# wildsonbbl/gnnepcsaft

Hardware: AMD Instinct MI355X
Metric: molecular graphs/sec (fwd+bwd) (higher is better)
Workload: dtype f32; 1 GPU; BASELINE configs[1]: PNA hidden=128 L=6 towers=1 pre=2 post=4, 4096 graphs/GPU (81920 atoms, 163840 directed bonds), fwd+loss+bwd incl. CSR packing; graphs_per_gpu=4096, parallelism=dp1, hip_graph=False, launch=auto, grad_allreduce_bytes=0, grad_exchange=none (1 rank)

## Files before the change

gnnepcsaft_amd/_lib.py:

```python
from __future__ import annotations

import ctypes as C
from pathlib import Path
from typing import Dict, Optional

import torch

_LIB_PATH = Path(__file__).resolve().parent / "libgnnepcsaft_hip.so"

ABI_VERSION = 6
GNX_OK, GNX_E_INVALID, GNX_E_HIP, GNX_E_RANGE, GNX_E_WORKSPACE = 0, -1, -2, -3, -4
OPT_GEMM_SPLIT, OPT_WGRAD_WGS, OPT_EMBED_BWD_MFMA, OPT_STD_BWD_CENTERED, OPT_GEMM_PIPE, OPT_WGRAD_PIPE, OPT_GEMM_AS, \
    OPT_GEMM_WS_FAST, OPT_GEMM_TILE_ROWS, OPT_GEMM_MID = range(10)
GEMM_RELU, GEMM_ACCUMULATE, GEMM_B_TRANS, GEMM_SPLIT_ONLY, GEMM_PRESPLIT = 1, 2, 4, 8, 16
POOL_ADD, POOL_MEAN, POOL_MAX = 0, 1, 2
K_NONE, K_PNA_AGG_FWD, K_PNA_AGG_BWD, K_GEMM_WS, K_GEMM_WGRAD, K_GINE_AGG_FWD, K_GINE_AGG_BWD, K_EDGE_COMBINE_FWD, \
    K_EDGE_COMBINE_BWD, K_BN_FWD, K_BN_BWD, K_GEMM_TILED, K_GEMM_SMALL, K_GEMM_WGRAD_BATCHED, K_KEY_SEGMENT_SUM, \
    K_EMBED, K_PNA_EDGE_FWD, K_PNA_EDGE_BWD, K_ATTN_FWD, K_ATTN_BWD, K_PCSAFT_RHO, K_PCSAFT_VP = range(22)
K_COUNT = 22
KERNEL_GROUPS = {K_PNA_AGG_FWD: "pna_aggregate_fwd", K_PNA_AGG_BWD: "pna_aggregate_bwd", K_GEMM_WS: "gemm_weights_stationary",
                 K_GEMM_WGRAD: "weight_gradient", K_GINE_AGG_FWD: "gine_aggregate_fwd", K_GINE_AGG_BWD: "gine_aggregate_bwd",
                 K_EDGE_COMBINE_FWD: "edge_combine_fwd", K_EDGE_COMBINE_BWD: "edge_combine_bwd", K_BN_FWD: "batchnorm_fwd",
                 K_BN_BWD: "batchnorm_bwd", K_GEMM_TILED: "gemm_tiled", K_GEMM_SMALL: "gemm_small",
                 K_GEMM_WGRAD_BATCHED: "weight_gradient_batched", K_KEY_SEGMENT_SUM: "key_segment_sum", K_EMBED: "embedding",
                 K_PNA_EDGE_FWD: "pna_edge_fused_fwd", K_PNA_EDGE_BWD: "pna_edge_fused_bwd",
                 K_ATTN_FWD: "transformer_attn_fwd", K_ATTN_BWD: "transformer_attn_bwd",
                 K_PCSAFT_RHO: "pcsaft_density", K_PCSAFT_VP: "pcsaft_vapor_pressure"}


class GnxError(RuntimeError):
    def __init__(self, status: int, msg: str):
        super().__init__(f"gnx status {status}: {msg}")
        self.status = status


class GemmSeg(C.Structure):
    _fields_ = [("a", C.c_void_p), ("lda", C.c_int64), ("rowscale", C.c_void_p), ("b", C.c_void_p),
                ("ldb", C.c_int64), ("k", C.c_int32), ("_pad", C.c_int32)]


class WgradProb(C.Structure):
    _fields_ = [("dC", C.c_void_p), ("lddc", C.c_int64), ("A", C.c_void_p), ("lda", C.c_int64),
                ("rowscale", C.c_void_p), ("dW", C.c_void_p), ("lddw", C.c_int64), ("dbias", C.c_void_p),
                ("M", C.c_int64), ("N", C.c_int32), ("K", C.c_int32)]


_vp, _i32, _i64, _f32, _sz = C.c_void_p, C.c_int32, C.c_int64, C.c_float, C.c_size_t

PNA_MAX_LAYERS, PNA_MAX_TOWERS = 8, 8
PNA_BWD_DEFER_SMALL, PNA_BWD_LAST_OF_PASS = 1, 2


class PnaFwdArgs(C.Structure):
    _fields_ = [("N", _i64), ("E", _i64), ("T", _i32), ("F", _i32), ("pre_layers", _i32), ("post_layers", _i32),
                ("D", _i32), ("merged", _i32),
                ("rowptr", _vp), ("src", _vp), ("dst", _vp), ("code", _vp), ("dperm", _vp), ("tiles", _vp), ("ntiles", _vp),
                ("max_tiles", _i64), ("x", _vp), ("Te", _vp), ("weff", _vp * PNA_MAX_TOWERS), ("Wm", _vp), ("bm", _vp),
                ("params", C.POINTER(_vp)), ("P", _vp), ("Q", _vp), ("A", _vp), ("hs", _vp * PNA_MAX_LAYERS),
                ("zs", _vp * PNA_MAX_LAYERS), ("ws", _vp), ("ws_bytes", _sz), ("out", _vp), ("etile_info", _vp),
                ("etile_w", _i32), ("tile_rows", _i32)]


class PnaBwdArgs(C.Structure):
    _fields_ = [("N", _i64), ("E", _i64), ("T", _i32), ("F", _i32), ("pre_layers", _i32), ("post_layers", _i32),
                ("R", _i32), ("D", _i32), ("avg_deg_log", _f32), ("merged", _i32), ("acc_first", _i32),
                ("use_side_streams", _i32), ("n_h", _i32), ("n_z", _i32),
                ("rowptr", _vp), ("colptr", _vp), ("cpos", _vp), ("code", _vp), ("code_pos", _vp), ("dperm", _vp),
                ("tiles", _vp), ("ntiles", _vp), ("chunks", _vp), ("nchunks", _vp),
                ("max_tiles", _i64), ("max_chunks", _i64),
                ("x", _vp), ("BE", _vp), ("EE", _vp), ("A", _vp),
                ("hs", _vp * PNA_MAX_LAYERS), ("zs", _vp * PNA_MAX_LAYERS), ("weff", _vp * PNA_MAX_TOWERS), ("Wm", _vp),
                ("params", C.POINTER(_vp)), ("grads", C.POINTER(_vp)), ("dout", _vp),
                ("gbuf", _vp * PNA_MAX_LAYERS), ("dA", _vp), ("gebuf", _vp * PNA_MAX_LAYERS), ("dP", _vp), ("dQ", _vp),
                ("dTe", _vp), ("dEE", _vp), ("dWm", _vp), ("dbm", _vp), ("dWeff", _vp), ("ws", _vp), ("ws_bytes", _sz),
                ("acc_buf", _vp), ("dx", _vp), ("flags", _i32), ("etile_w", _i32), ("etile_info", _vp)]


class PnaFinishArgs(C.Structure):
    _fields_ = [("L", _i32), ("T", _i32), ("F", _i32), ("pre_layers", _i32), ("post_layers", _i32), ("R", _i32), ("D", _i32),
                ("merged", _i32), ("use_side_streams", _i32), ("_pad", _i32),
                ("BE", _vp), ("acc_buf", _vp), ("ones", _vp), ("avg_deg_log", C.POINTER(_f32)),
                ("params", C.POINTER(_vp)), ("grads", C.POINTER(_vp)), ("EE", C.POINTER(_vp)), ("dTe", C.POINTER(_vp)),
                ("dEE", C.POINTER(_vp)), ("dWm", C.POINTER(_vp)), ("dbm", C.POINTER(_vp)), ("dWeff", C.POINTER(_vp))]


class SmallProb(C.Structure):
    _fields_ = [("A", _vp), ("lda", _i64), ("B", _vp), ("ldb", _i64), ("bias", _vp), ("C", _vp), ("ldc", _i64),
                ("M", _i32), ("N", _i32), ("K", _i32), ("flags", _i32)]


SB_A_TRANS, SB_B_TRANS, SB_ACCUMULATE, SB_ATOMIC, SB_RELU = 1, 2, 4, 8, 16

SIGNATURES = {
    "gnx_create": (_i32, [C.POINTER(_vp), _i32]),
    "gnx_destroy": (_i32, [_vp]),
    "gnx_set_stream": (_i32, [_vp, _vp]),
    "gnx_last_error": (C.c_char_p, []),
    "gnx_abi_version": (_i32, []),
    "gnx_set_option": (_i32, [_vp, _i32, _i32]),
    "gnx_get_option": (_i32, [_vp, _i32, C.POINTER(_i32)]),
    "gnx_prof_begin": (_i32, [_vp, C.c_uint32]),
    "gnx_prof_read": (_i32, [_vp, _i32, C.POINTER(_i64), C.POINTER(C.c_double), C.POINTER(C.c_double),
                             C.POINTER(C.c_double), C.POINTER(C.c_double)]),
    "gnx_prof_end": (_i32, [_vp]),
    "gnx_pack_csr_workspace_bytes": (_sz, [_i64, _i64]),
    "gnx_pack_csr": (_i32, [_vp, _vp, _i64, _i64, _vp, _vp, _vp, _vp, _vp, _vp, _vp, _sz]),
    "gnx_feature_code": (_i32, [_vp, _vp, _i64, _i32, C.POINTER(_i32), _vp, _vp, _vp, _sz]),
    "gnx_graph_ptr": (_i32, [_vp, _vp, _i64, _i64, _vp, _vp, _sz]),
    "gnx_degree_scalers": (_i32, [_vp, _vp, _i64, _f32, _vp, _vp]),
    "gnx_embed_sum_fwd": (_i32, [_vp, _vp, _i64, _i32, C.POINTER(_i32), _vp, _i32, _vp]),
    "gnx_table_scatter_workspace_bytes": (_sz, [_i64, _i32, _i32]),
    "gnx_embed_sum_bwd": (_i32, [_vp, _vp, _i64, _i32, C.POINTER(_i32), _i32, _vp, _i32, _vp, _vp, _sz]),
    "gnx_check_range": (_i32, [_vp]),
    "gnx_gemm_workspace_bytes": (_sz, [_vp, _i32, C.POINTER(GemmSeg), C.POINTER(_i64), _i32, _i64, _i32, _vp, _i32,
                                       _i32]),
    "gnx_gemm": (_i32, [_vp, _i32, C.POINTER(GemmSeg), _i64, _i32, _vp, _vp, _i64, _vp, _i64, _i32, _vp, _sz]),
    "gnx_gemm_wgrad": (_i32, [_vp, _vp, _i64, _vp, _i64, _vp, _i64, _i32, _i32, _vp, _i64, _vp]),
    "gnx_gemm_wgrad_batched": (_i32, [_vp, _i32, C.POINTER(WgradProb)]),
    "gnx_degree_max": (_i32, [_vp, _vp, _i64, C.POINTER(_i32)]),
    "gnx_degree_classes_workspace_bytes": (_sz, [_i64, _i32]),
    "gnx_degree_classes": (_i32, [_vp, _vp, _i64, _i32, _vp, _vp, _vp, _sz]),
    "gnx_class_tiles": (_i32, [_vp, _vp, _i32, _i32, _vp, _vp]),
    "gnx_gemm_grouped": (_i32, [_vp, _i32, C.POINTER(GemmSeg), C.POINTER(_i64), _i32, _i64, _i32, _vp, _vp, _i64, _vp,
                                _i64, _i32, _vp, _vp, _vp, _i64, _vp, _sz]),
    "gnx_gemm_tile_rows": (_i32, [_vp, _i64, _i32]),
    "gnx_gemm_grouped_rows": (_i32, [_vp, _i32, C.POINTER(GemmSeg), C.POINTER(_i64), _i32, _i64, _i32, _vp, _vp, _i64, _vp,
                                     _i64, _i32, _vp, _vp, _vp, _i64, _vp, _sz, _i32]),
    "gnx_gemm_wgrad_grouped": (_i32, [_vp, _vp, _i64, _vp, _i64, _i64, _i32, _i32, _vp, _i64, _i64, _vp, _vp, _vp,
                                      _i64]),
    "gnx_pna_weff": (_i32, [_vp, _vp, _i64, _i32, _i32, _f32, _vp]),
    "gnx_pna_weff_bwd": (_i32, [_vp, _vp, _i32, _i32, _f32, _vp, _i64]),
    "gnx_group_by_small_key": (_i32, [_vp, _vp, _i64, _i32, _vp, _vp, _vp, _sz]),
    "gnx_key_segment_sum": (_i32, [_vp, _vp, _vp, _vp, _i64, _i32, _vp]),
    "gnx_edge_combine_fwd": (_i32, [_vp, _vp, _vp, _vp, _vp, _vp, _vp, _i64, _i32, _i32, _vp]),
    "gnx_edge_combine_bwd": (_i32, [_vp, _vp, _vp, _vp, _vp, _vp, _i64, _i64, _i32, _i32, _vp, _vp, _vp, _vp, _sz]),
    "gnx_pna_aggregate_fwd": (_i32, [_vp, _vp, _vp, _i64, _i64, _i32, _i32, _vp]),
    "gnx_pna_aggregate_bwd": (_i32, [_vp, _vp, _vp, _vp, _vp, _i64, _i64, _i32, _i32, _vp]),
    "gnx_edge_tiles_count": (_i32, [_i64, _i32]),
    "gnx_edge_tiles": (_i32, [_vp, _vp, _i64, _i64, _i32, _vp]),
    "gnx_pna_edge_fwd": (_i32, [_vp, _vp, _vp, _vp, _vp, _vp, _vp, _vp, _vp, _i32, _i64, _i64, _i32, _i32, C.POINTER(_vp),
                                C.POINTER(_vp), _vp, _vp, _vp]),
    "gnx_pna_edge_bwd": (_i32, [_vp, _vp, _vp, _vp, _vp, _vp, _i32, _i64, _i64, _i32, _i32, _i32, C.POINTER(_vp), _vp, _vp,
                                _vp]),
    "gnx_gine_aggregate_fwd": (_i32, [_vp, _vp, _vp, _vp, _vp, _vp, _i64, _i64, _i32, _f32, _vp]),
    "gnx_gine_aggregate_bwd": (_i32, [_vp, _vp, _vp, _vp, _vp, _vp, _vp, _vp, _vp, _vp, _i64, _i64, _i32, _i32, _f32,
                                      _vp, _vp]),
    "gnx_gine_dle": (_i32, [_vp, _vp, _vp, _vp, _vp, _vp, _vp, _vp, _i64, _i32, _i32, _vp]),
    "gnx_transformer_attn_fwd": (_i32, [_vp, _vp, _vp, _vp, _vp, _vp, _i64, _i64, _i32, _i32, _f32, C.c_uint64,
                                        C.c_uint64, _vp, _vp, _vp]),
    "gnx_transformer_attn_bwd": (_i32, [_vp, _vp, _vp, _vp, _vp, _vp, _vp, _vp, _vp, _vp, _vp, _vp, _i64, _i64, _i32,
                                        _i32, _i32, _f32, C.c_uint64, C.c_uint64, _vp, _vp, _vp]),
    "gnx_transformer_attn_dle": (_i32, [_vp, _vp, _vp, _vp, _vp, _vp, _vp, _i64, _i32, _i32, _i32, _vp]),
    "gnx_pcsaft_density": (_i32, [_vp, _vp, _i64, _vp, _vp, _vp, _i64, _vp, _vp]),
    "gnx_pcsaft_vapor_pressure": (_i32, [_vp, _vp, _i64, _vp, _vp, _i64, _vp, _vp, _vp, _vp]),
    "gnx_segment_pool_fwd": (_i32, [_vp, _vp, _vp, _i64, _i32, _i32, _vp]),
    "gnx_segment_pool_bwd": (_i32, [_vp, _vp, _vp, _vp, _vp, _i64, _i32, _i32, _vp]),
    "gnx_batchnorm_workspace_bytes": (_sz, [_i64, _i32]),
    "gnx_batchnorm_fwd": (_i32, [_vp, _vp, _i64, _i32, _vp, _vp, _vp, _vp, _vp, _f32, _f32, _i32, _i32, _vp, _vp, _vp,
                                 _vp, _sz]),
    "gnx_batchnorm_bwd": (_i32, [_vp, _vp, _vp, _vp, _i64, _i32, _vp, _vp, _vp, _i32, _vp, _vp, _vp, _vp, _sz]),
    "gnx_dropout": (_i32, [_vp, _vp, _i64, _f32, C.c_uint64, C.c_uint64, _vp]),
    "gnx_huber_ape": (_i32, [_vp, _vp, _vp, _i64, _f32, _vp, _vp]),
    "gnx_adamw_amsgrad": (_i32, [_vp, _vp, _vp, _vp, _vp, _vp, _i64, _f32, _f32, _f32, _f32, _f32, _i64]),
    "gnx_sgd": (_i32, [_vp, _vp, _vp, _i64, _f32]),
    "gnx_pna_weight_only": (_i32, [_vp, _vp, _i32, _i32, _i32, _i32, _i32, _i32, _f32, C.POINTER(_vp), _i32, _vp, _vp,
                                   C.POINTER(_vp), _vp, _vp]),
    "gnx_pna_conv_fwd": (_i32, [_vp, C.POINTER(PnaFwdArgs)]),
    "gnx_pna_weight_only_all": (_i32, [_vp, _i32, _vp, _i32, _i32, _i32, _i32, _i32, _i32, C.POINTER(_f32), C.POINTER(_vp),
                                       _i32, C.POINTER(_vp), C.POINTER(_vp), C.POINTER(_vp), C.POINTER(_vp), C.POINTER(_vp)]),
    "gnx_pna_stack_finish": (_i32, [_vp, C.POINTER(PnaFinishArgs)]),
    "gnx_gemm_small_batched": (_i32, [_vp, _i32, C.POINTER(SmallProb)]),
    "gnx_pna_weff_batched": (_i32, [_vp, _i32, C.POINTER(_vp), _i64, _i32, _i32, C.POINTER(_f32), C.POINTER(_vp)]),
    "gnx_pna_weff_bwd_batched": (_i32, [_vp, _i32, C.POINTER(_vp), _i32, _i32, C.POINTER(_f32), C.POINTER(_vp), _i64]),
    "gnx_pna_conv_bwd_workspace_bytes": (_sz, [_i32, _i32, _i32]),
    "gnx_pna_conv_bwd": (_i32, [_vp, C.POINTER(PnaBwdArgs)]),
    "gnx_fill": (_i32, [_vp, _vp, _i64, _f32]),
    "gnx_scale": (_i32, [_vp, _vp, _i64, _f32]),
    "gnx_axpy": (_i32, [_vp, _vp, _vp, _i64, _f32]),
    "gnx_side_stream": (_i32, [_vp, C.POINTER(_vp)]),
    "gnx_side_begin": (_i32, [_vp]),
    "gnx_side_end": (_i32, [_vp]),
    "gnx_side_join": (_i32, [_vp]),
    "gnx_side_stream_n": (_i32, [_vp, _i32, C.POINTER(_vp)]),
    "gnx_side_begin_n": (_i32, [_vp, _i32]),
    "gnx_side_join_n": (_i32, [_vp, _i32]),
    "gnx_clip_rows": (_i32, [_vp, _vp, _i64, _i32, _vp, _vp, _vp]),
}

_lib: Optional[C.CDLL] = None
_handles: Dict[int, int] = {}


def lib_path() -> Path:
    return _LIB_PATH


def load() -> C.CDLL:
    global _lib
    if _lib is not None:
        return _lib
    if not _LIB_PATH.exists():
        raise ImportError(f"{_LIB_PATH} is missing: build it with `python -m gnnepcsaft_amd.build` "
                          "(hipcc --offload-arch=gfx950). There is no CPU fallback.")
    lib = C.CDLL(str(_LIB_PATH))
    for name, (res, args) in SIGNATURES.items():
        fn = getattr(lib, name)
        fn.restype = res
        fn.argtypes = args
    if lib.gnx_abi_version() != ABI_VERSION:
        raise ImportError(f"ABI version mismatch: library {lib.gnx_abi_version()} != binding {ABI_VERSION}")
    _lib = lib
    return lib


def last_error() -> str:
    return load().gnx_last_error().decode(errors="replace")


def check(status: int) -> None:
    if status != GNX_OK:
        raise GnxError(status, last_error())


_bound_stream: dict = {}
try:
    _raw_stream = torch._C._cuda_getCurrentRawStream
except AttributeError:
    def _raw_stream(idx: int) -> int:
        return torch.cuda.current_stream(idx).cuda_stream


def handle(device: torch.device) -> int:
    if device.type != "cuda":
        raise GnxError(GNX_E_INVALID, f"gnnepcsaft_amd kernels need a HIP device tensor, got {device}; there is no CPU "
                                      "fallback")
    idx = device.index if device.index is not None else torch.cuda.current_device()
    lib = load()
    h = _handles.get(idx)
    if h is None:
        out = _vp()
        check(lib.gnx_create(C.byref(out), idx))
        h = out.value
        _handles[idx] = h
    stream = _raw_stream(idx)
    if _bound_stream.get(idx) != stream:
        check(lib.gnx_set_stream(h, stream))
        _bound_stream[idx] = stream
    return h
```

gnnepcsaft_amd/csrc/gnx_norm.hip:

```cpp
#include "gnx_common.hpp"

#define BN_ROWS_PER_BLOCK 256

extern "C" size_t gnx_batchnorm_workspace_bytes(int64_t M, int32_t H) {
  if (M < 0) M = 0;
  size_t chunks = (size_t)gnx_cdiv(M > 0 ? M : 1, BN_ROWS_PER_BLOCK);
  return sizeof(float) * ((size_t)4 * H + chunks * 2 * (size_t)H) + 256;
}

__global__ void __launch_bounds__(256) k_bn_partial(const float* __restrict__ x, int64_t M, int H,
                                                    float* __restrict__ part) {
  __shared__ float s1[4][64], s2[4][64];
  const int cx = threadIdx.x & 63, ry = threadIdx.x >> 6;
  const int col = blockIdx.y * 64 + cx;
  int64_t r0 = (int64_t)blockIdx.x * BN_ROWS_PER_BLOCK;
  int64_t r1 = r0 + BN_ROWS_PER_BLOCK;
  if (r1 > M) r1 = M;
  float a1 = 0.f, a2 = 0.f;
  if (col < H) {
    const float k = x[col];
    for (int64_t r = r0 + ry; r < r1; r += 4) {
      float v = x[r * H + col] - k;
      a1 += v;
      a2 += v * v;
    }
  }
  s1[ry][cx] = a1;
  s2[ry][cx] = a2;
  __syncthreads();
  if (ry == 0 && col < H) {
    float t1 = (s1[0][cx] + s1[1][cx]) + (s1[2][cx] + s1[3][cx]);
    float t2 = (s2[0][cx] + s2[1][cx]) + (s2[2][cx] + s2[3][cx]);
    part[((int64_t)blockIdx.x * 2 + 0) * H + col] = t1;
    part[((int64_t)blockIdx.x * 2 + 1) * H + col] = t2;
  }
}


__global__ void __launch_bounds__(256) k_bn_partial_v4(const float* __restrict__ x, int64_t M, int H,
                                                       float* __restrict__ part) {
  __shared__ f32x4 s1[8][32], s2[8][32];
  const int cq = threadIdx.x & 31, ry = threadIdx.x >> 5;
  const int col = blockIdx.y * 128 + cq * 4;
  int64_t r0 = (int64_t)blockIdx.x * BN_ROWS_PER_BLOCK;
  int64_t r1 = r0 + BN_ROWS_PER_BLOCK;
  if (r1 > M) r1 = M;
  f32x4 a1 = {0.f, 0.f, 0.f, 0.f}, a2 = {0.f, 0.f, 0.f, 0.f};
  if (col < H) {
    const f32x4 k = *reinterpret_cast<const f32x4*>(x + col);
    int64_t r = r0 + ry;
    for (; r + 24 < r1; r += 32) {
      f32x4 v0 = *reinterpret_cast<const f32x4*>(x + r * H + col);
      f32x4 v1 = *reinterpret_cast<const f32x4*>(x + (r + 8) * H + col);
      f32x4 v2 = *reinterpret_cast<const f32x4*>(x + (r + 16) * H + col);
      f32x4 v3 = *reinterpret_cast<const f32x4*>(x + (r + 24) * H + col);
      v0 -= k;
      a1 += v0;
      a2 += v0 * v0;
      v1 -= k;
      a1 += v1;
      a2 += v1 * v1;
      v2 -= k;
      a1 += v2;
      a2 += v2 * v2;
      v3 -= k;
      a1 += v3;
      a2 += v3 * v3;
    }
    for (; r < r1; r += 8) {
      f32x4 v = *reinterpret_cast<const f32x4*>(x + r * H + col);
      v -= k;
      a1 += v;
      a2 += v * v;
    }
  }
  s1[ry][cq] = a1;
  s2[ry][cq] = a2;
  __syncthreads();
  if (ry == 0 && col < H) {
    f32x4 t1 = s1[0][cq], t2 = s2[0][cq];
#pragma unroll
    for (int l = 1; l < 8; ++l) {
      t1 += s1[l][cq];
      t2 += s2[l][cq];
    }
    *reinterpret_cast<f32x4*>(part + ((int64_t)blockIdx.x * 2 + 0) * H + col) = t1;
    *reinterpret_cast<f32x4*>(part + ((int64_t)blockIdx.x * 2 + 1) * H + col) = t2;
  }
}

__global__ void __launch_bounds__(256) k_bn_bwd_partial_v4(const float* __restrict__ dy, const float* __restrict__ x,
                                                           const float* __restrict__ y, int64_t M, int H,
                                                           const float* __restrict__ mean,
                                                           const float* __restrict__ rstd, int relu,
                                                           float* __restrict__ part) {
  __shared__ f32x4 s1[8][32], s2[8][32];
  const int cq = threadIdx.x & 31, ry = threadIdx.x >> 5;
  const int col = blockIdx.y * 128 + cq * 4;
  int64_t r0 = (int64_t)blockIdx.x * BN_ROWS_PER_BLOCK;
  int64_t r1 = r0 + BN_ROWS_PER_BLOCK;
  if (r1 > M) r1 = M;
  f32x4 a1 = {0.f, 0.f, 0.f, 0.f}, a2 = {0.f, 0.f, 0.f, 0.f};
  if (col < H) {
    const f32x4 mu = *reinterpret_cast<const f32x4*>(mean + col);
    const f32x4 rs = *reinterpret_cast<const f32x4*>(rstd + col);
    auto row = [&](int64_t r, f32x4& g, f32x4& xv, f32x4& yv) {
      g = *reinterpret_cast<const f32x4*>(dy + r * H + col);
      xv = *reinterpret_cast<const f32x4*>(x + r * H + col);
      yv = *reinterpret_cast<const f32x4*>((relu ? y : x) + r * H + col);
    };
    auto fold = [&](f32x4 g, const f32x4& xv, const f32x4& yv) {
      if (relu) {
        g.x = yv.x > 0.f ? g.x : 0.f;
        g.y = yv.y > 0.f ? g.y : 0.f;
        g.z = yv.z > 0.f ? g.z : 0.f;
        g.w = yv.w > 0.f ? g.w : 0.f;
      }
      a1 += g;
      a2 += g * ((xv - mu) * rs);
    };
    int64_t r = r0 + ry;
    for (; r + 8 < r1; r += 16) {
      f32x4 g0, x0, y0, g1, x1, y1;
      row(r, g0, x0, y0);
      row(r + 8, g1, x1, y1);
      fold(g0, x0, y0);
      fold(g1, x1, y1);
    }
    for (; r < r1; r += 8) {
      f32x4 g, xv, yv;
      row(r, g, xv, yv);
      fold(g, xv, yv);
    }
  }
  s1[ry][cq] = a1;
  s2[ry][cq] = a2;
  __syncthreads();
  if (ry == 0 && col < H) {
    f32x4 t1 = s1[0][cq], t2 = s2[0][cq];
#pragma unroll
    for (int l = 1; l < 8; ++l) {
      t1 += s1[l][cq];
      t2 += s2[l][cq];
    }
    *reinterpret_cast<f32x4*>(part + ((int64_t)blockIdx.x * 2 + 0) * H + col) = t1;
    *reinterpret_cast<f32x4*>(part + ((int64_t)blockIdx.x * 2 + 1) * H + col) = t2;
  }
}

template <int VEC>
__global__ void __launch_bounds__(256) k_bn_bwd_apply_v(const float* __restrict__ dy, const float* __restrict__ x,
                                                        const float* __restrict__ y, int64_t total, int H,
                                                        const float* __restrict__ mean, const float* __restrict__ rstd,
                                                        const float* __restrict__ coef, int relu,
                                                        float* __restrict__ dx) {
  int64_t i = ((int64_t)blockIdx.x * blockDim.x + threadIdx.x) * 4;
  const int64_t stride = (int64_t)gridDim.x * blockDim.x * 4;
  for (; i < total; i += stride) {
    const int c = (int)(i % H);
    f32x4 g = *reinterpret_cast<const f32x4*>(dy + i);
    const f32x4 xv = *reinterpret_cast<const f32x4*>(x + i);
    if (relu) {
      const f32x4 yv = *reinterpret_cast<const f32x4*>(y + i);
      g.x = yv.x > 0.f ? g.x : 0.f;
      g.y = yv.y > 0.f ? g.y : 0.f;
      g.z = yv.z > 0.f ? g.z : 0.f;
      g.w = yv.w > 0.f ? g.w : 0.f;
    }
    const f32x4 mu = *reinterpret_cast<const f32x4*>(mean + c), rs = *reinterpret_cast<const f32x4*>(rstd + c);
    const f32x4 k0 = *reinterpret_cast<const f32x4*>(coef + c), k1 = *reinterpret_cast<const f32x4*>(coef + H + c),
                k2 = *reinterpret_cast<const f32x4*>(coef + 2 * H + c);
    const f32x4 xh = (xv - mu) * rs;
    *reinterpret_cast<f32x4*>(dx + i) = k0 * (g - k1 - xh * k2);
  }
}

__device__ __forceinline__ void bn_fold(const float* __restrict__ part, int64_t chunks, int H, int c, float& t1,
                                        float& t2) {
  __shared__ float f1[16][17], f2[16][17];
  const int cx = threadIdx.x & 15, ly = threadIdx.x >> 4;
  float a1 = 0.f, a2 = 0.f;
  if (c < H) {
    int64_t b = ly;
    for (; b + 48 < chunks; b += 64) {
      const float p0 = part[(b * 2 + 0) * H + c], q0 = part[(b * 2 + 1) * H + c];
      const float p1 = part[((b + 16) * 2 + 0) * H + c], q1 = part[((b + 16) * 2 + 1) * H + c];
      const float p2 = part[((b + 32) * 2 + 0) * H + c], q2 = part[((b + 32) * 2 + 1) * H + c];
      const float p3 = part[((b + 48) * 2 + 0) * H + c], q3 = part[((b + 48) * 2 + 1) * H + c];
      a1 += p0;
      a2 += q0;
      a1 += p1;
      a2 += q1;
      a1 += p2;
      a2 += q2;
      a1 += p3;
      a2 += q3;
    }
    for (; b < chunks; b += 16) {
      a1 += part[(b * 2 + 0) * H + c];
      a2 += part[(b * 2 + 1) * H + c];
    }
  }
  f1[ly][cx] = a1;
  f2[ly][cx] = a2;
  __syncthreads();
  t1 = 0.f;
  t2 = 0.f;
  if (ly == 0) {
#pragma unroll
    for (int l = 0; l < 16; ++l) {
      t1 += f1[l][cx];
      t2 += f2[l][cx];
    }
  }
}

__global__ void k_bn_finalize(const float* __restrict__ x, const float* __restrict__ part, int64_t chunks, int64_t M,
                              int H, const float* __restrict__ gamma, const float* __restrict__ beta,
                              float* __restrict__ running_mean, float* __restrict__ running_var, float momentum,
                              float eps, int training, float* __restrict__ save_mean, float* __restrict__ save_rstd,
                              float* __restrict__ ab, int64_t* __restrict__ num_batches_tracked) {
  const int c = blockIdx.x * 16 + (threadIdx.x & 15);
  if (training && num_batches_tracked != nullptr && blockIdx.x == 0 && threadIdx.x == 0) num_batches_tracked[0] += 1;
  float t1 = 0.f, t2 = 0.f;
  if (training) bn_fold(part, chunks, H, c, t1, t2);
  if (c >= H || (threadIdx.x >> 4) != 0) return;
  float mean, var;
  if (training) {
    const float inv = 1.0f / (float)M;
    const float d = t1 * inv;
    mean = x[c] + d;
    var = fmaxf(t2 * inv - d * d, 0.f);
    if (running_mean) running_mean[c] = (1.f - momentum) * running_mean[c] + momentum * mean;
    if (running_var) {
      float unb = (M > 1) ? var * ((float)M / (float)(M - 1)) : var;
      running_var[c] = (1.f - momentum) * running_var[c] + momentum * unb;
    }
  } else {
    mean = running_mean[c];
    var = running_var[c];
  }
  float rstd = 1.0f / sqrtf(var + eps);
  if (save_mean) save_mean[c] = mean;
  if (save_rstd) save_rstd[c] = rstd;
  float a = rstd * (gamma ? gamma[c] : 1.f);
  ab[c] = a;
  ab[H + c] = (beta ? beta[c] : 0.f) - mean * a;
}

template <int VEC>
__global__ void __launch_bounds__(256) k_bn_apply(const float* __restrict__ x, int64_t total, int H,
                                                  const float* __restrict__ ab, int relu, float* __restrict__ y) {
  int64_t i = ((int64_t)blockIdx.x * blockDim.x + threadIdx.x) * VEC;
  int64_t stride = (int64_t)gridDim.x * blockDim.x * VEC;
  for (; i < total; i += stride) {
    int c = (int)(i % H);
    if constexpr (VEC == 4) {
      f32x4 v = *reinterpret_cast<const f32x4*>(x + i);
      f32x4 a = *reinterpret_cast<const f32x4*>(ab + c);
      f32x4 b = *reinterpret_cast<const f32x4*>(ab + H + c);
      f32x4 o = {v.x * a.x + b.x, v.y * a.y + b.y, v.z * a.z + b.z, v.w * a.w + b.w};
      if (relu) {
        o.x = fmaxf(o.x, 0.f);
        o.y = fmaxf(o.y, 0.f);
        o.z = fmaxf(o.z, 0.f);
        o.w = fmaxf(o.w, 0.f);
      }
      *reinterpret_cast<f32x4*>(y + i) = o;
    } else {
      float o = x[i] * ab[c] + ab[H + c];
      y[i] = relu ? fmaxf(o, 0.f) : o;
    }
  }
}

extern "C" int32_t gnx_batchnorm_fwd(gnx_handle* h, const float* x, int64_t M, int32_t H, const float* gamma,
                                     const float* beta, float* running_mean, float* running_var,
                                     int64_t* num_batches_tracked, float momentum, float eps, int32_t training,
                                     int32_t relu, float* y, float* save_mean, float* save_rstd, void* ws,
                                     size_t ws_bytes) {
  GNX_CHECK_ARG(h && H > 0 && M >= 0, "gnx_batchnorm_fwd: bad argument");
  if (M == 0) return GNX_OK;
  GNX_CHECK_ARG(x && y && ws, "gnx_batchnorm_fwd: NULL argument");
  GNX_CHECK_ARG(training || (running_mean && running_var), "gnx_batchnorm_fwd: eval mode needs running stats");
  if (ws_bytes < gnx_batchnorm_workspace_bytes(M, H)) {
    gnx_set_error("gnx_batchnorm_fwd: workspace %zu < %zu", ws_bytes, gnx_batchnorm_workspace_bytes(M, H));
    return GNX_E_WORKSPACE;
  }
  float* ab = reinterpret_cast<float*>(ws);
  float* part = ab + 4 * (size_t)H;
  int64_t chunks = gnx_cdiv(M, BN_ROWS_PER_BLOCK);
  gnx_prof_scope prof(h, GNX_K_BN_FWD, (training ? 12.0 : 8.0) * M * H);
  if (training) {
    if (H % 4 == 0)
      hipLaunchKernelGGL(k_bn_partial_v4, dim3((unsigned)chunks, (unsigned)gnx_cdiv(H, 128)), dim3(256), 0, h->stream, x,
                         M, (int)H, part);
    else
      hipLaunchKernelGGL(k_bn_partial, dim3((unsigned)chunks, (unsigned)gnx_cdiv(H, 64)), dim3(256), 0, h->stream, x, M,
                         (int)H, part);
    GNX_LAUNCH_CHECK();
  }
  hipLaunchKernelGGL(k_bn_finalize, dim3((unsigned)gnx_cdiv(H, 16)), dim3(256), 0, h->stream, x, part, chunks, M, (int)H,
                     gamma, beta, running_mean, running_var, momentum, eps, (int)training, save_mean, save_rstd, ab,
                     num_batches_tracked);
  GNX_LAUNCH_CHECK();
  int64_t total = M * H;
  if (H % 4 == 0) {
    int64_t blocks = gnx_cdiv(total / 4, 256);
    if (blocks > 4096) blocks = 4096;
    hipLaunchKernelGGL(k_bn_apply<4>, dim3((unsigned)blocks), dim3(256), 0, h->stream, x, total, (int)H, ab, (int)relu, y);
  } else {
    int64_t blocks = gnx_cdiv(total, 256);
    if (blocks > 4096) blocks = 4096;
    hipLaunchKernelGGL(k_bn_apply<1>, dim3((unsigned)blocks), dim3(256), 0, h->stream, x, total, (int)H, ab, (int)relu, y);
  }
  GNX_LAUNCH_CHECK();
  return GNX_OK;
}

__global__ void __launch_bounds__(256) k_bn_bwd_partial(const float* __restrict__ dy, const float* __restrict__ x,
                                                        const float* __restrict__ y, int64_t M, int H,
                                                        const float* __restrict__ mean, const float* __restrict__ rstd,
                                                        int relu, float* __restrict__ part) {
  __shared__ float s1[4][64], s2[4][64];
  const int cx = threadIdx.x & 63, ry = threadIdx.x >> 6;
  const int col = blockIdx.y * 64 + cx;
  int64_t r0 = (int64_t)blockIdx.x * BN_ROWS_PER_BLOCK;
  int64_t r1 = r0 + BN_ROWS_PER_BLOCK;
  if (r1 > M) r1 = M;
  float a1 = 0.f, a2 = 0.f;
  if (col < H) {
    const float mu = mean[col], rs = rstd[col];
    for (int64_t r = r0 + ry; r < r1; r += 4) {
      float g = dy[r * H + col];
      if (relu && !(y[r * H + col] > 0.f)) g = 0.f;
      a1 += g;
      a2 += g * ((x[r * H + col] - mu) * rs);
    }
  }
  s1[ry][cx] = a1;
  s2[ry][cx] = a2;
  __syncthreads();
  if (ry == 0 && col < H) {
    part[((int64_t)blockIdx.x * 2 + 0) * H + col] = (s1[0][cx] + s1[1][cx]) + (s1[2][cx] + s1[3][cx]);
    part[((int64_t)blockIdx.x * 2 + 1) * H + col] = (s2[0][cx] + s2[1][cx]) + (s2[2][cx] + s2[3][cx]);
  }
}

__global__ void k_bn_bwd_finalize(const float* __restrict__ part, int64_t chunks, int64_t M, int H,
                                  const float* __restrict__ gamma, const float* __restrict__ rstd,
                                  float* __restrict__ dgamma, float* __restrict__ dbeta, float* __restrict__ coef) {
  const int c = blockIdx.x * 16 + (threadIdx.x & 15);
  float t1 = 0.f, t2 = 0.f;
  bn_fold(part, chunks, H, c, t1, t2);
  if (c >= H || (threadIdx.x >> 4) != 0) return;
  if (dbeta) dbeta[c] += t1;
  if (dgamma) dgamma[c] += t2;
  const float inv = 1.0f / (float)M;
  coef[c] = (gamma ? gamma[c] : 1.f) * rstd[c];
  coef[H + c] = t1 * inv;
  coef[2 * H + c] = t2 * inv;
}

__global__ void __launch_bounds__(256) k_bn_bwd_apply(const float* __restrict__ dy, const float* __restrict__ x,
                                                      const float* __restrict__ y, int64_t total, int H,
                                                      const float* __restrict__ mean, const float* __restrict__ rstd,
                                                      const float* __restrict__ coef, int relu, float* __restrict__ dx) {
  int64_t i = (int64_t)blockIdx.x * blockDim.x + threadIdx.x;
  int64_t stride = (int64_t)gridDim.x * blockDim.x;
  for (; i < total; i += stride) {
    int c = (int)(i % H);
    float g = dy[i];
    if (relu && !(y[i] > 0.f)) g = 0.f;
    float xh = (x[i] - mean[c]) * rstd[c];
    dx[i] = coef[c] * (g - coef[H + c] - xh * coef[2 * H + c]);
  }
}

extern "C" int32_t gnx_batchnorm_bwd(gnx_handle* h, const float* dy, const float* x, const float* y, int64_t M,
                                     int32_t H, const float* gamma, const float* save_mean, const float* save_rstd,
                                     int32_t relu, float* dx, float* dgamma, float* dbeta, void* ws, size_t ws_bytes) {
  GNX_CHECK_ARG(h && H > 0 && M >= 0, "gnx_batchnorm_bwd: bad argument");
  if (M == 0) return GNX_OK;
  GNX_CHECK_ARG(dy && x && save_mean && save_rstd && dx && ws && (!relu || y), "gnx_batchnorm_bwd: NULL argument");
  if (ws_bytes < gnx_batchnorm_workspace_bytes(M, H)) {
    gnx_set_error("gnx_batchnorm_bwd: workspace %zu < %zu", ws_bytes, gnx_batchnorm_workspace_bytes(M, H));
    return GNX_E_WORKSPACE;
  }
  float* coef = reinterpret_cast<float*>(ws);
  float* part = coef + 4 * (size_t)H;
  int64_t chunks = gnx_cdiv(M, BN_ROWS_PER_BLOCK);
  gnx_prof_scope prof(h, GNX_K_BN_BWD, 28.0 * M * H);
  if (H % 4 == 0)
    hipLaunchKernelGGL(k_bn_bwd_partial_v4, dim3((unsigned)chunks, (unsigned)gnx_cdiv(H, 128)), dim3(256), 0, h->stream,
                       dy, x, y, M, (int)H, save_mean, save_rstd, (int)relu, part);
  else
    hipLaunchKernelGGL(k_bn_bwd_partial, dim3((unsigned)chunks, (unsigned)gnx_cdiv(H, 64)), dim3(256), 0, h->stream, dy,
                       x, y, M, (int)H, save_mean, save_rstd, (int)relu, part);
  GNX_LAUNCH_CHECK();
  hipLaunchKernelGGL(k_bn_bwd_finalize, dim3((unsigned)gnx_cdiv(H, 16)), dim3(256), 0, h->stream, part, chunks, M, (int)H,
                     gamma, save_rstd, dgamma, dbeta, coef);
  GNX_LAUNCH_CHECK();
  int64_t total = M * H;
  if (H % 4 == 0) {
    int64_t blocks = gnx_cdiv(total / 4, 256);
    if (blocks > 4096) blocks = 4096;
    hipLaunchKernelGGL(k_bn_bwd_apply_v<4>, dim3((unsigned)blocks), dim3(256), 0, h->stream, dy, x, y, total, (int)H,
                       save_mean, save_rstd, coef, (int)relu, dx);
  } else {
    int64_t blocks = gnx_cdiv(total, 256);
    if (blocks > 8192) blocks = 8192;
    hipLaunchKernelGGL(k_bn_bwd_apply, dim3((unsigned)blocks), dim3(256), 0, h->stream, dy, x, y, total, (int)H,
                       save_mean, save_rstd, coef, (int)relu, dx);
  }
  GNX_LAUNCH_CHECK();
  return GNX_OK;
}

#define LOSS_MAX_BLOCKS 64

__global__ void __launch_bounds__(256) k_huber_partial(const float* __restrict__ pred, const float* __restrict__ tgt,
                                                       int64_t count, float delta, float* __restrict__ part,
                                                       float* __restrict__ dpred) {
  __shared__ float sh[256], sm[256];
  float ah = 0.f, am = 0.f;
  const float inv = 1.0f / (float)count;
  int64_t i = (int64_t)blockIdx.x * blockDim.x + threadIdx.x;
  int64_t stride = (int64_t)gridDim.x * blockDim.x;
  for (; i < count; i += stride) {
    float p = pred[i], t = tgt[i];
    float a = (p - t) / t;
    float aa = fabsf(a);
    ah += (aa <= delta) ? 0.5f * a * a : delta * (aa - 0.5f * delta);
    am += fabsf(p - t) / fmaxf(fabsf(t), 1.17e-06f);
    if (dpred) {
      float da = (aa <= delta) ? a : (a > 0.f ? delta : -delta);
      dpred[i] = da * inv / t;
    }
  }
  sh[threadIdx.x] = ah;
  sm[threadIdx.x] = am;
  __syncthreads();
  for (int off = 128; off > 0; off >>= 1) {
    if (threadIdx.x < off) {
      sh[threadIdx.x] += sh[threadIdx.x + off];
      sm[threadIdx.x] += sm[threadIdx.x + off];
    }
    __syncthreads();
  }
  if (threadIdx.x == 0) {
    part[blockIdx.x * 2] = sh[0];
    part[blockIdx.x * 2 + 1] = sm[0];
  }
}

__global__ void k_huber_final(const float* __restrict__ part, int blocks, int64_t count, float* __restrict__ out2) {
  if (threadIdx.x == 0 && blockIdx.x == 0) {
    float h = 0.f, m = 0.f;
    for (int b = 0; b < blocks; ++b) {
      h += part[b * 2];
      m += part[b * 2 + 1];
    }
    out2[0] = h / (float)count;
    out2[1] = m / (float)count;
  }
}

extern "C" int32_t gnx_huber_ape(gnx_handle* h, const float* pred, const float* target, int64_t count, float delta,
                                 float* out2, float* dpred) {
  GNX_CHECK_ARG(h && pred && target && out2 && count > 0, "gnx_huber_ape: bad argument");
  int blocks = (int)(gnx_cdiv(count, 256) < LOSS_MAX_BLOCKS ? gnx_cdiv(count, 256) : LOSS_MAX_BLOCKS);
  hipLaunchKernelGGL(k_huber_partial, dim3(blocks), dim3(256), 0, h->stream, pred, target, count, delta, h->d_scratch,
                     dpred);
  GNX_LAUNCH_CHECK();
  hipLaunchKernelGGL(k_huber_final, dim3(1), dim3(64), 0, h->stream, h->d_scratch, blocks, count, out2);
  GNX_LAUNCH_CHECK();
  return GNX_OK;
}
```

gnnepcsaft_amd/csrc/gnx_pack.hip:

```cpp
#include "gnx_common.hpp"

#define SCAN_ITEMS 4
#define SCAN_BLOCK 256
#define SCAN_TILE (SCAN_ITEMS * SCAN_BLOCK)

__global__ void __launch_bounds__(SCAN_BLOCK) k_scan_tile(const int* __restrict__ in, int* __restrict__ out,
                                                          int* __restrict__ sums, int64_t n) {
  __shared__ int s[SCAN_BLOCK];
  int64_t base = (int64_t)blockIdx.x * SCAN_TILE + (int64_t)threadIdx.x * SCAN_ITEMS;
  int v[SCAN_ITEMS];
  int t = 0;
#pragma unroll
  for (int i = 0; i < SCAN_ITEMS; ++i) {
    v[i] = (base + i < n) ? in[base + i] : 0;
    t += v[i];
  }
  s[threadIdx.x] = t;
  __syncthreads();
  for (int off = 1; off < SCAN_BLOCK; off <<= 1) {
    int add = (threadIdx.x >= off) ? s[threadIdx.x - off] : 0;
    __syncthreads();
    s[threadIdx.x] += add;
    __syncthreads();
  }
  int excl = s[threadIdx.x] - t;
#pragma unroll
  for (int i = 0; i < SCAN_ITEMS; ++i) {
    if (base + i < n) out[base + i] = excl;
    excl += v[i];
  }
  if (threadIdx.x == SCAN_BLOCK - 1) sums[blockIdx.x] = s[SCAN_BLOCK - 1];
}

__global__ void k_scan_add(int* __restrict__ out, const int* __restrict__ offs, int64_t n) {
  int64_t i = (int64_t)blockIdx.x * SCAN_TILE + threadIdx.x;
  int o = offs[blockIdx.x];
  for (int k = 0; k < SCAN_ITEMS; ++k, i += SCAN_BLOCK)
    if (i < n) out[i] += o;
}

__global__ void k_set_total(int* __restrict__ out, const int* __restrict__ in, int64_t n) {
  if (threadIdx.x == 0 && blockIdx.x == 0) out[n] = (n > 0) ? out[n - 1] + in[n - 1] : 0;
}

static int32_t exclusive_scan(gnx_handle* h, const int* in, int* out, int64_t n, int* ws, bool write_total) {
  if (n > 0) {
    int64_t blocks = gnx_cdiv(n, SCAN_TILE);
    hipLaunchKernelGGL(k_scan_tile, dim3((unsigned)blocks), dim3(SCAN_BLOCK), 0, h->stream, in, out, ws, n);
    GNX_LAUNCH_CHECK();
    if (blocks > 1) {
      int* sums_scanned = ws + blocks + 1;
      int32_t st = exclusive_scan(h, ws, sums_scanned, blocks, sums_scanned + blocks + 1, false);
      if (st != GNX_OK) return st;
      hipLaunchKernelGGL(k_scan_add, dim3((unsigned)blocks), dim3(SCAN_BLOCK), 0, h->stream, out, sums_scanned, n);
      GNX_LAUNCH_CHECK();
    }
  }
  if (write_total) {
    hipLaunchKernelGGL(k_set_total, dim3(1), dim3(64), 0, h->stream, out, in, n);
    GNX_LAUNCH_CHECK();
  }
  return GNX_OK;
}

static size_t scan_ws_ints_total(int64_t n) {
  size_t tot = 0;
  int64_t m = n;
  while (m > 1) {
    int64_t b = gnx_cdiv(m, SCAN_TILE);
    tot += 2 * ((size_t)b + 1);
    m = b;
  }
  return tot + 16;
}

__global__ void k_convert_edges(const int64_t* __restrict__ ei, int64_t E, int64_t N, int* __restrict__ src0,
                                int* __restrict__ dst0, int* __restrict__ flag) {
  int64_t e = (int64_t)blockIdx.x * blockDim.x + threadIdx.x;
  if (e >= E) return;
  int64_t s = ei[e], d = ei[E + e];
  bool bad = (s < 0) | (s >= N) | (d < 0) | (d >= N);
  if (bad) {
    atomicOr(flag, 1);
    s = 0;
    d = 0;
  }
  src0[e] = (int)s;
  dst0[e] = (int)d;
}

__global__ void k_count_keys(const int* __restrict__ key, int64_t E, int* __restrict__ counts) {
  int64_t e = (int64_t)blockIdx.x * blockDim.x + threadIdx.x;
  if (e < E) atomicAdd(&counts[key[e]], 1);
}

__global__ void k_fill_groups(const int* __restrict__ key, int64_t E, const int* __restrict__ ptr,
                              int* __restrict__ cursor, int* __restrict__ items) {
  int64_t e = (int64_t)blockIdx.x * blockDim.x + threadIdx.x;
  if (e >= E) return;
  int k = key[e];
  int pos = ptr[k] + atomicAdd(&cursor[k], 1);
  items[pos] = (int)e;
}

__global__ void k_sort_groups(const int* __restrict__ ptr, int64_t N, int* __restrict__ items) {
  int64_t i = (int64_t)blockIdx.x * blockDim.x + threadIdx.x;
  if (i >= N) return;
  int b = ptr[i], e = ptr[i + 1];
  for (int a = b + 1; a < e; ++a) {
    int v = items[a];
    int c = a - 1;
    while (c >= b && items[c] > v) {
      items[c + 1] = items[c];
      --c;
    }
    items[c + 1] = v;
  }
}

__global__ void k_gather_endpoints(const int* __restrict__ perm, const int* __restrict__ src0,
                                   const int* __restrict__ dst0, int64_t E, int* __restrict__ src,
                                   int* __restrict__ dst) {
  int64_t p = (int64_t)blockIdx.x * blockDim.x + threadIdx.x;
  if (p >= E) return;
  int e = perm[p];
  src[p] = src0[e];
  dst[p] = dst0[e];
}

static int32_t group_by_key(gnx_handle* h, const int* key, int64_t E, int64_t N, int* ptr, int* items, int* cursor,
                            int* scan_ws) {
  gnx_zero_ints(h, cursor, N > 0 ? N : 1);
  if (E > 0) {
    hipLaunchKernelGGL(k_count_keys, dim3((unsigned)gnx_cdiv(E, 256)), dim3(256), 0, h->stream, key, E, cursor);
    GNX_LAUNCH_CHECK();
  }
  int32_t st = exclusive_scan(h, cursor, ptr, N, scan_ws, true);
  if (st != GNX_OK) return st;
  gnx_zero_ints(h, cursor, N > 0 ? N : 1);
  if (E > 0) {
    hipLaunchKernelGGL(k_fill_groups, dim3((unsigned)gnx_cdiv(E, 256)), dim3(256), 0, h->stream, key, E, ptr, cursor,
                       items);
    GNX_LAUNCH_CHECK();
    hipLaunchKernelGGL(k_sort_groups, dim3((unsigned)gnx_cdiv(N, 256)), dim3(256), 0, h->stream, ptr, N, items);
    GNX_LAUNCH_CHECK();
  }
  return GNX_OK;
}

extern "C" size_t gnx_pack_csr_workspace_bytes(int64_t N, int64_t E) {
  if (N < 0) N = 0;
  if (E < 0) E = 0;
  size_t ints = 2 * (size_t)E + (size_t)N + 1 + scan_ws_ints_total(N) + 64;
  return ints * sizeof(int);
}

extern "C" int32_t gnx_pack_csr(gnx_handle* h, const int64_t* edge_index, int64_t E, int64_t N, int32_t* rowptr,
                                int32_t* perm, int32_t* src, int32_t* dst, int32_t* colptr, int32_t* cpos, void* ws,
                                size_t ws_bytes) {
  GNX_CHECK_ARG(h != nullptr, "gnx_pack_csr: handle is NULL");
  GNX_CHECK_ARG(N >= 0 && E >= 0 && N < (1ll << 31) - 1 && E < (1ll << 31) - 1, "gnx_pack_csr: N=%lld E=%lld out of int32 range",
                (long long)N, (long long)E);
  GNX_CHECK_ARG(rowptr && colptr, "gnx_pack_csr: rowptr/colptr NULL");
  GNX_CHECK_ARG(E == 0 || (edge_index && perm && src && dst && cpos), "gnx_pack_csr: NULL edge array with E>0");
  if (ws_bytes < gnx_pack_csr_workspace_bytes(N, E) || (!ws && ws_bytes)) {
    gnx_set_error("gnx_pack_csr: workspace %zu < %zu", ws_bytes, gnx_pack_csr_workspace_bytes(N, E));
    return GNX_E_WORKSPACE;
  }
  GNX_CHECK_ARG(ws != nullptr, "gnx_pack_csr: workspace is NULL");
  int* w = reinterpret_cast<int*>(ws);
  int* src0 = w;
  int* dst0 = src0 + E;
  int* cursor = dst0 + E;
  int* scan_ws = cursor + N + 1;
  if (E > 0) {
    hipLaunchKernelGGL(k_convert_edges, dim3((unsigned)gnx_cdiv(E, 256)), dim3(256), 0, h->stream, edge_index, E, N,
                       src0, dst0, h->d_flag);
    GNX_LAUNCH_CHECK();
  }
  int32_t st = group_by_key(h, dst0, E, N, rowptr, perm, cursor, scan_ws);
  if (st != GNX_OK) return st;
  if (E > 0) {
    hipLaunchKernelGGL(k_gather_endpoints, dim3((unsigned)gnx_cdiv(E, 256)), dim3(256), 0, h->stream, perm, src0,
                       dst0, E, src, dst);
    GNX_LAUNCH_CHECK();
  }
  return group_by_key(h, src, E, N, colptr, cpos, cursor, scan_ws);
}

struct dims_t {
  int d[16];
};

__global__ void k_feature_code(const int64_t* __restrict__ feat, int64_t rows, int K, dims_t dims,
                               const int* __restrict__ perm, int* __restrict__ code, int* __restrict__ flag) {
  int64_t p = (int64_t)blockIdx.x * blockDim.x + threadIdx.x;
  if (p >= rows) return;
  int64_t r = perm ? perm[p] : p;
  int c = 0;
  bool bad = false;
  for (int k = 0; k < K; ++k) {
    int64_t f = feat[r * K + k];
    if (f < 0 || f >= dims.d[k]) {
      bad = true;
      f = 0;
    }
    c = c * dims.d[k] + (int)f;
  }
  if (bad) atomicOr(flag, 2);
  code[p] = c;
}

extern "C" int32_t gnx_feature_code(gnx_handle* h, const int64_t* feat, int64_t rows, int32_t K, const int32_t* dims,
                                    const int32_t* perm, int32_t* code, void* ws, size_t ws_bytes) {
  (void)ws;
  (void)ws_bytes;
  GNX_CHECK_ARG(h && dims && K > 0 && K <= 16 && rows >= 0, "gnx_feature_code: bad argument");
  GNX_CHECK_ARG(rows == 0 || (feat && code), "gnx_feature_code: NULL array with rows>0");
  dims_t d;
  int64_t prod = 1;
  for (int k = 0; k < 16; ++k) d.d[k] = (k < K) ? dims[k] : 1;
  for (int k = 0; k < K; ++k) {
    GNX_CHECK_ARG(dims[k] > 0, "gnx_feature_code: dims[%d] <= 0", k);
    prod *= dims[k];
  }
  GNX_CHECK_ARG(prod < (1ll << 31), "gnx_feature_code: code space overflows int32");
  if (rows > 0) {
    hipLaunchKernelGGL(k_feature_code, dim3((unsigned)gnx_cdiv(rows, 256)), dim3(256), 0, h->stream, feat, rows, (int)K,
                       d, perm, code, h->d_flag);
    GNX_LAUNCH_CHECK();
  }
  return GNX_OK;
}

__global__ void k_graph_ptr(const int64_t* __restrict__ batch, int64_t N, int64_t B, int* __restrict__ ptr,
                            int* __restrict__ flag) {
  int64_t n = (int64_t)blockIdx.x * blockDim.x + threadIdx.x;
  if (n > N) return;
  int64_t prev = (n == 0) ? -1 : batch[n - 1];
  int64_t cur = (n == N) ? B : batch[n];
  if (n < N && (cur < 0 || cur >= B)) {
    atomicOr(flag, 4);
    return;
  }
  if (cur < prev) {
    atomicOr(flag, 8);
    return;
  }
  for (int64_t g = prev + 1; g <= cur; ++g) ptr[g] = (int)n;
}

extern "C" int32_t gnx_graph_ptr(gnx_handle* h, const int64_t* batch, int64_t N, int64_t B, int32_t* graph_ptr,
                                 void* ws, size_t ws_bytes) {
  (void)ws;
  (void)ws_bytes;
  GNX_CHECK_ARG(h && graph_ptr && N >= 0 && B >= 0 && (batch || N == 0), "gnx_graph_ptr: bad argument");
  hipLaunchKernelGGL(k_graph_ptr, dim3((unsigned)gnx_cdiv(N + 1, 256)), dim3(256), 0, h->stream, batch, N, B,
                     graph_ptr, h->d_flag);
  GNX_LAUNCH_CHECK();
  return GNX_OK;
}

__global__ void k_degree_scalers(const int* __restrict__ rowptr, int64_t N, float avg_log, float* __restrict__ amp,
                                 float* __restrict__ att) {
  int64_t n = (int64_t)blockIdx.x * blockDim.x + threadIdx.x;
  if (n >= N) return;
  float d = (float)(rowptr[n + 1] - rowptr[n]);
  amp[n] = logf(d + 1.0f) / avg_log;
  att[n] = avg_log / logf(fmaxf(d, 1.0f) + 1.0f);
}

extern "C" int32_t gnx_degree_scalers(gnx_handle* h, const int32_t* rowptr, int64_t N, float avg_deg_log, float* amp,
                                      float* att) {
  GNX_CHECK_ARG(h && N >= 0 && (N == 0 || (rowptr && amp && att)), "gnx_degree_scalers: bad argument");
  if (N == 0) return GNX_OK;
  hipLaunchKernelGGL(k_degree_scalers, dim3((unsigned)gnx_cdiv(N, 256)), dim3(256), 0, h->stream, rowptr, N,
                     avg_deg_log, amp, att);
  GNX_LAUNCH_CHECK();
  return GNX_OK;
}

struct weff_batch_args {
  const float* W[GNX_SMALL_BATCH];
  float* out[GNX_SMALL_BATCH];
  float avg_log[GNX_SMALL_BATCH];
  int64_t ldw;
  int F, D;
};

__global__ void k_pna_weff_batched(weff_batch_args a) {
  const int b = blockIdx.y;
  const int F = a.F;
  int64_t i = (int64_t)blockIdx.x * blockDim.x + threadIdx.x;
  int64_t per = (int64_t)F * 4 * F;
  if (i >= per * a.D) return;
  int d = (int)(i / per);
  int o = (int)((i % per) / (4 * F)), j = (int)(i % (4 * F));
  float dd = (float)d;
  float amp = logf(dd + 1.0f) / a.avg_log[b];
  float att = a.avg_log[b] / logf(fmaxf(dd, 1.0f) + 1.0f);
  const float* w = a.W[b] + (int64_t)o * a.ldw;
  a.out[b][i] = w[F + j] + amp * w[5 * F + j] + att * w[9 * F + j];
}

struct weff_bwd_batch_args {
  const float* dWeff[GNX_SMALL_BATCH];
  float* dW[GNX_SMALL_BATCH];
  float avg_log[GNX_SMALL_BATCH];
  int64_t lddw;
  int F, D;
};

__global__ void k_pna_weff_bwd_batched(weff_bwd_batch_args a) {
  const int b = blockIdx.y;
  const int F = a.F;
  int64_t i = (int64_t)blockIdx.x * blockDim.x + threadIdx.x;
  int64_t per = (int64_t)F * 4 * F;
  if (i >= per) return;
  int o = (int)(i / (4 * F)), j = (int)(i % (4 * F));
  float s1 = 0.f, s2 = 0.f, s3 = 0.f;
  const float avg_log = a.avg_log[b];
  const float* dWeff = a.dWeff[b];
  for (int d = 0; d < a.D; ++d) {
    float dd = (float)d;
    float amp = logf(dd + 1.0f) / avg_log;
    float att = avg_log / logf(fmaxf(dd, 1.0f) + 1.0f);
    float v = dWeff[(int64_t)d * per + i];
    s1 += v;
    s2 += amp * v;
    s3 += att * v;
  }
  float* w = a.dW[b] + (int64_t)o * a.lddw;
  w[F + j] += s1;
  w[5 * F + j] += s2;
  w[9 * F + j] += s3;
}

extern "C" int32_t gnx_pna_weff_bwd_batched(gnx_handle* h, int32_t n, const float* const* dWeff, int32_t F, int32_t D,
                                            const float* avg_deg_log, float* const* dW, int64_t lddw) {
  GNX_CHECK_ARG(h && dWeff && dW && avg_deg_log && n >= 0 && F > 0 && D > 0 && lddw >= 13 * F,
                "gnx_pna_weff_bwd_batched: bad argument");
  const int64_t cnt = (int64_t)F * 4 * F;
  for (int32_t i0 = 0; i0 < n; i0 += GNX_SMALL_BATCH) {
    weff_bwd_batch_args a;
    const int m = n - i0 < GNX_SMALL_BATCH ? n - i0 : GNX_SMALL_BATCH;
    for (int i = 0; i < GNX_SMALL_BATCH; ++i) {
      const int k = i < m ? i0 + i : i0;
      a.dWeff[i] = dWeff[k];
      a.dW[i] = dW[k];
      a.avg_log[i] = avg_deg_log[k];
      GNX_CHECK_ARG(a.dWeff[i] && a.dW[i], "gnx_pna_weff_bwd_batched: NULL pointer at %d", k);
    }
    a.lddw = lddw;
    a.F = F;
    a.D = D;
    hipLaunchKernelGGL(k_pna_weff_bwd_batched, dim3((unsigned)gnx_cdiv(cnt, 256), (unsigned)m), dim3(256), 0, h->stream, a);
    GNX_LAUNCH_CHECK();
  }
  return GNX_OK;
}

extern "C" int32_t gnx_pna_weff_batched(gnx_handle* h, int32_t n, const float* const* W, int64_t ldw, int32_t F, int32_t D,
                                        const float* avg_deg_log, float* const* Weff) {
  GNX_CHECK_ARG(h && W && Weff && avg_deg_log && n >= 0 && F > 0 && D > 0 && ldw >= 13 * F, "gnx_pna_weff_batched: bad argument");
  const int64_t cnt = (int64_t)F * 4 * F * D;
  for (int32_t i0 = 0; i0 < n; i0 += GNX_SMALL_BATCH) {
    weff_batch_args a;
    const int m = n - i0 < GNX_SMALL_BATCH ? n - i0 : GNX_SMALL_BATCH;
    for (int i = 0; i < GNX_SMALL_BATCH; ++i) {
      const int k = i < m ? i0 + i : i0;
      a.W[i] = W[k];
      a.out[i] = Weff[k];
      a.avg_log[i] = avg_deg_log[k];
      GNX_CHECK_ARG(a.W[i] && a.out[i], "gnx_pna_weff_batched: NULL pointer at %d", k);
    }
    a.ldw = ldw;
    a.F = F;
    a.D = D;
    hipLaunchKernelGGL(k_pna_weff_batched, dim3((unsigned)gnx_cdiv(cnt, 256), (unsigned)m), dim3(256), 0, h->stream, a);
    GNX_LAUNCH_CHECK();
  }
  return GNX_OK;
}

extern "C" int32_t gnx_pna_weff(gnx_handle* h, const float* W, int64_t ldw, int32_t F, int32_t D, float avg_deg_log,
                                float* Weff) {
  GNX_CHECK_ARG(h && W && Weff && F > 0 && D > 0 && ldw >= 13 * F, "gnx_pna_weff: bad argument");
  return gnx_pna_weff_batched(h, 1, &W, ldw, F, D, &avg_deg_log, &Weff);
}

extern "C" int32_t gnx_pna_weff_bwd(gnx_handle* h, const float* dWeff, int32_t F, int32_t D, float avg_deg_log,
                                    float* dW, int64_t lddw) {
  GNX_CHECK_ARG(h && dWeff && dW && F > 0 && D > 0 && lddw >= 13 * F, "gnx_pna_weff_bwd: bad argument");
  return gnx_pna_weff_bwd_batched(h, 1, &dWeff, F, D, &avg_deg_log, &dW, lddw);
}

__global__ void k_degree_max(const int* __restrict__ rowptr, int64_t N, int* __restrict__ out) {
  int64_t n = (int64_t)blockIdx.x * blockDim.x + threadIdx.x;
  int d = (n < N) ? rowptr[n + 1] - rowptr[n] : 0;
  for (int off = 32; off > 0; off >>= 1) d = max(d, __shfl_xor(d, off));
  if ((threadIdx.x & 63) == 0) atomicMax(out, d);
}

extern "C" int32_t gnx_degree_max(gnx_handle* h, const int32_t* rowptr, int64_t N, int32_t* max_degree_host) {
  GNX_CHECK_ARG(h && max_degree_host && N >= 0 && (N == 0 || rowptr), "gnx_degree_max: bad argument");
  int* d_out = h->d_flag + 8;
  gnx_zero_ints(h, d_out, 1);
  if (N > 0) {
    hipLaunchKernelGGL(k_degree_max, dim3((unsigned)gnx_cdiv(N, 256)), dim3(256), 0, h->stream, rowptr, N, d_out);
    GNX_LAUNCH_CHECK();
  }
  int v = 0;
  GNX_HIP(hipMemcpyAsync(&v, d_out, sizeof(int), hipMemcpyDeviceToHost, h->stream));
  GNX_HIP(hipStreamSynchronize(h->stream));
  *max_degree_host = v;
  return GNX_OK;
}

#define DC_BLOCK 256
#define DC_MAX_CLASSES 64

__global__ void __launch_bounds__(DC_BLOCK) k_dc_hist(const int* __restrict__ rowptr, const int* __restrict__ keys,
                                                       int64_t N, int D, int nblocks, int* __restrict__ blockhist,
                                                       int* __restrict__ flag) {
  __shared__ int hist[DC_MAX_CLASSES];
  if (threadIdx.x < DC_MAX_CLASSES) hist[threadIdx.x] = 0;
  __syncthreads();
  int64_t n = (int64_t)blockIdx.x * DC_BLOCK + threadIdx.x;
  if (n < N) {
    int d = keys ? keys[n] : rowptr[n + 1] - rowptr[n];
    if (d < 0) d = 0;
    if (d >= D) {
      atomicOr(flag, 32);
      d = D - 1;
    }
    atomicAdd(&hist[d], 1);
  }
  __syncthreads();
  if (threadIdx.x < D) blockhist[threadIdx.x * nblocks + blockIdx.x] = hist[threadIdx.x];
}

__global__ void __launch_bounds__(DC_BLOCK) k_dc_fill(const int* __restrict__ rowptr, const int* __restrict__ keys,
                                                       int64_t N, int D, int nblocks,
                                                       const int* __restrict__ blockoff, int* __restrict__ dperm,
                                                       int* __restrict__ cls_ptr) {
  __shared__ int degs[DC_BLOCK];
  int64_t n = (int64_t)blockIdx.x * DC_BLOCK + threadIdx.x;
  int d = -1;
  if (n < N) {
    d = keys ? keys[n] : rowptr[n + 1] - rowptr[n];
    if (d < 0) d = 0;
    if (d >= D) d = D - 1;
  }
  degs[threadIdx.x] = d;
  __syncthreads();
  if (n < N) {
    int rank = 0;
    for (int t = 0; t < (int)threadIdx.x; ++t) rank += (degs[t] == d) ? 1 : 0;
    dperm[blockoff[d * nblocks + blockIdx.x] + rank] = (int)n;
  }
  if (blockIdx.x == 0 && (int)threadIdx.x <= D)
    cls_ptr[threadIdx.x] = ((int)threadIdx.x == D) ? (int)N : blockoff[threadIdx.x * nblocks];
}

extern "C" size_t gnx_degree_classes_workspace_bytes(int64_t N, int32_t D) {
  if (N < 0) N = 0;
  int64_t nblocks = gnx_cdiv(N > 0 ? N : 1, DC_BLOCK);
  size_t ints = 2 * (size_t)(D * nblocks + 1) + scan_ws_ints_total(D * nblocks) + 64;
  return ints * sizeof(int);
}

extern "C" int32_t gnx_degree_classes(gnx_handle* h, const int32_t* rowptr, int64_t N, int32_t D, int32_t* dperm,
                                      int32_t* cls_ptr, void* ws, size_t ws_bytes) {
  GNX_CHECK_ARG(h && rowptr && cls_ptr && N >= 0 && D >= 1 && D <= DC_MAX_CLASSES && (N == 0 || dperm),
                "gnx_degree_classes: bad argument (D must be in [1,%d])", DC_MAX_CLASSES);
  if (ws_bytes < gnx_degree_classes_workspace_bytes(N, D) || !ws) {
    gnx_set_error("gnx_degree_classes: workspace %zu < %zu", ws_bytes, gnx_degree_classes_workspace_bytes(N, D));
    return GNX_E_WORKSPACE;
  }
  int nblocks = (int)gnx_cdiv(N > 0 ? N : 1, DC_BLOCK);
  int* blockhist = reinterpret_cast<int*>(ws);
  int* blockoff = blockhist + (size_t)D * nblocks + 1;
  int* scan_ws = blockoff + (size_t)D * nblocks + 1;
  hipLaunchKernelGGL(k_dc_hist, dim3(nblocks), dim3(DC_BLOCK), 0, h->stream, rowptr, (const int*)nullptr, N, (int)D,
                     nblocks, blockhist, h->d_flag);
  GNX_LAUNCH_CHECK();
  int32_t st = exclusive_scan(h, blockhist, blockoff, (int64_t)D * nblocks, scan_ws, false);
  if (st != GNX_OK) return st;
  hipLaunchKernelGGL(k_dc_fill, dim3(nblocks), dim3(DC_BLOCK), 0, h->stream, rowptr, (const int*)nullptr, N, (int)D,
                     nblocks, blockoff, dperm, cls_ptr);
// ... 55 lines not shown
```

gnnepcsaft_amd/functional.py:

```python
from __future__ import annotations

from typing import Optional, Sequence

import torch

from . import ops
from .ops import GraphPack


_GRAD_IN_PLACE = False
_USE_DEGREE_CLASSES = True
_NATIVE_LAYER_BWD = True
_FUSED_EDGE = True
_BATCH_WEIGHT_ONLY = True


def set_grad_in_place(enabled: bool) -> None:
    global _GRAD_IN_PLACE
    _GRAD_IN_PLACE = bool(enabled)


def grad_in_place_enabled() -> bool:
    return _GRAD_IN_PLACE


def set_degree_classes(enabled: bool) -> None:
    global _USE_DEGREE_CLASSES
    _USE_DEGREE_CLASSES = bool(enabled)


def degree_classes_enabled() -> bool:
    return _USE_DEGREE_CLASSES


def set_native_layer_backward(enabled: bool) -> None:
    global _NATIVE_LAYER_BWD
    _NATIVE_LAYER_BWD = bool(enabled)


def set_fused_edge(enabled: bool) -> None:
    global _FUSED_EDGE
    _FUSED_EDGE = bool(enabled)


def set_batch_weight_only(enabled: bool) -> None:
    global _BATCH_WEIGHT_ONLY
    _BATCH_WEIGHT_ONLY = bool(enabled)


def batch_weight_only_enabled() -> bool:
    return _BATCH_WEIGHT_ONLY


def grad_sinks(params: Sequence[torch.Tensor]) -> tuple:
    if not _GRAD_IN_PLACE:
        return tuple(None for _ in params)
    out = []
    for p in params:
        g = p.grad
        ok = g is not None and g.dtype == torch.float32 and g.is_contiguous() and g.shape == p.shape and \
            g.device == p.device
        out.append(g if ok else None)
    return tuple(out)


def _tower_slices(T: int, F: int):
    return [None] if T == 1 else [slice(t * F, (t + 1) * F) for t in range(T)]


def _cols(t: torch.Tensor, sl_t):
    return t if sl_t is None else t[:, sl_t]


def _empty(rows: int, cols: int, like: torch.Tensor) -> torch.Tensor:
    return torch.empty(rows, cols, dtype=torch.float32, device=like.device)


def _zeros_like(t: torch.Tensor) -> torch.Tensor:
    return ops.zeros(*t.shape, device=t.device)


def adjacent_rows(tensors: Sequence[torch.Tensor]) -> Optional[torch.Tensor]:
    t0 = tensors[0]
    if t0.dim() != 2 or t0.dtype is not torch.float32 or not t0.is_contiguous():
        return None
    H = t0.size(1)
    ptr, rows = t0.data_ptr(), 0
    for t in tensors:
        if t.dim() != 2 or t.size(1) != H or t.dtype is not torch.float32 or not t.is_contiguous() or \
                t.device != t0.device or t.data_ptr() != ptr + rows * H * 4:
            return None
        rows += t.size(0)
    if t0.untyped_storage().nbytes() - t0.storage_offset() * 4 < rows * H * 4:
        return None
    return torch.as_strided(t0.detach(), (rows, H), (H, 1))


class EmbedSumFn(torch.autograd.Function):

    @staticmethod
    def forward(ctx, idx, offsets, *weights):
        table = adjacent_rows(weights)
        if table is None:
            table = torch.cat([w.detach() for w in weights], dim=0)
        ctx.save_for_backward(idx)
        ctx.offsets = tuple(offsets)
        ctx.sinks = grad_sinks(weights)
        return ops.embed_sum_fwd(idx, table, offsets)

    @staticmethod
    def backward(ctx, dout):
        (idx,) = ctx.saved_tensors
        sinks, offs = ctx.sinks, ctx.offsets
        if all(g is not None for g in sinks):
            gtable = adjacent_rows(sinks)
            if gtable is not None:
                ops.embed_sum_bwd(idx, offs, dout.contiguous(), out=gtable)
                return (None, None) + (None,) * len(sinks)
        dtable = ops.embed_sum_bwd(idx, offs, dout.contiguous())
        return (None, None) + tuple(dtable[offs[k]:offs[k + 1]] for k in range(len(sinks)))


class DropoutFn(torch.autograd.Function):

    @staticmethod
    def forward(ctx, x, p, seed, offset):
        ctx.key = (float(p), int(seed), int(offset))
        return ops.dropout(x, p, seed, offset)

    @staticmethod
    def backward(ctx, dy):
        p, seed, offset = ctx.key
        return ops.dropout(dy, p, seed, offset), None, None, None


class LinearFn(torch.autograd.Function):

    @staticmethod
    def forward(ctx, x, weight, bias):
        x = x.contiguous()
        ctx.save_for_backward(x, weight)
        ctx.has_bias = bias is not None
        ctx.sinks = grad_sinks([weight] + ([bias] if bias is not None else []))
        y = _empty(x.size(0), weight.size(0), x)
        return ops.gemm([(x, None, weight)], y, bias=bias)

    @staticmethod
    def backward(ctx, dy):
        x, weight = ctx.saved_tensors
        dy = dy.contiguous()
        sw = ctx.sinks[0]
        sb = ctx.sinks[1] if ctx.has_bias else None
        dw = sw if sw is not None else _zeros_like(weight)
        db = None
        if ctx.has_bias:
            db = sb if sb is not None else ops.zeros(weight.size(0), device=dy.device)
        ops.gemm_wgrad(dy, x, dw, dbias=db)
        dx = None
        if ctx.needs_input_grad[0]:
            dx = ops.gemm([(dy, None, weight)], _empty(x.size(0), x.size(1), x), b_trans=False)
        ops.finish_backward(dy.device, sw is not None and (sb is not None or not ctx.has_bias), ctx.sinks)
        return dx, (None if sw is not None else dw), (None if (sb is not None or not ctx.has_bias) else db)


class BatchNormFn(torch.autograd.Function):

    @staticmethod
    def forward(ctx, x, gamma, beta, running_mean, running_var, momentum, eps, training, relu, nbt=None):
        x = x.contiguous()
        y, mean, rstd = ops.batchnorm_fwd(x, gamma, beta, running_mean, running_var, momentum, eps, training, relu,
                                          num_batches_tracked=nbt)
        ctx.save_for_backward(x, y, gamma, mean, rstd)
        ctx.relu, ctx.training = relu, training
        ctx.sinks = grad_sinks([gamma, beta])
        return y

    @staticmethod
    def backward(ctx, dy):
        x, y, gamma, mean, rstd = ctx.saved_tensors
        if not ctx.training:
            raise NotImplementedError("BatchNorm backward in eval mode is not on the reference's training path")
        sg, sb = ctx.sinks
        dx, dgamma, dbeta = ops.batchnorm_bwd(dy.contiguous(), x, y, gamma, mean, rstd, ctx.relu, dgamma=sg, dbeta=sb)
        return dx, (None if sg is not None else dgamma), (None if sb is not None else dbeta), None, None, None, None, \
            None, None, None


class SegmentPoolFn(torch.autograd.Function):

    @staticmethod
    def forward(ctx, x, ptr, B, mode):
        x = x.contiguous()
        out = ops.segment_pool_fwd(x, ptr, B, mode)
        ctx.save_for_backward(x, out, ptr)
        ctx.B, ctx.mode = B, mode
        return out

    @staticmethod
    def backward(ctx, dout):
        x, out, ptr = ctx.saved_tensors
        return ops.segment_pool_bwd(dout.contiguous(), x, out, ptr, ctx.B, ctx.mode), None, None, None


class HuberAPEFn(torch.autograd.Function):

    @staticmethod
    def forward(ctx, pred, target, delta):
        out2, dpred = ops.huber_ape(pred, target, delta, need_grad=True)
        ctx.save_for_backward(dpred)
        ctx.mark_non_differentiable(out2)
        return out2[0], out2

    @staticmethod
    def backward(ctx, dloss, _):
        (dpred,) = ctx.saved_tensors
        return dpred * dloss, None, None


def _pna_weight_only(BE, T, F, pre_layers, post_layers, avg_deg_log, params, D):
    R, H = BE.size(0), T * F
    merged = post_layers > 1
    if _NATIVE_LAYER_BWD and BE.is_cuda and T <= 8:
        import ctypes as C
        from . import _lib
        EE, Te = _empty(R, F, BE), _empty(R, H, BE)
        weffs = [torch.empty(D, F, 4 * F, dtype=torch.float32, device=BE.device) for _ in range(T)] if D > 0 else []
        Wm = _empty(H, H, BE) if merged else None
        bm = torch.empty(H, dtype=torch.float32, device=BE.device) if merged else None
        n = len(params)
        parr = (C.c_void_p * n)(*[p.data_ptr() for p in params])
        warr = (C.c_void_p * max(T, 1))(*[w.data_ptr() for w in weffs]) if weffs else None
        ops.check(_lib.load().gnx_pna_weight_only(
            _lib.handle(BE.device), BE.data_ptr(), R, T, F, pre_layers, post_layers, D, float(avg_deg_log),
            C.cast(parr, C.POINTER(C.c_void_p)), int(merged), EE.data_ptr(), Te.data_ptr(),
            None if warr is None else C.cast(warr, C.POINTER(C.c_void_p)), None if Wm is None else Wm.data_ptr(),
            None if bm is None else bm.data_ptr()))
        return EE, Te, weffs, Wm, bm
    enc_w, enc_b, lin_w, lin_b = params[:4]
    per = 2 * (pre_layers + post_layers)
    sl = _tower_slices(T, F)
    EE = ops.gemm([(BE, None, enc_w)], _empty(R, F, BE), bias=enc_b)
    Te = _empty(R, H, BE)
    weffs, last = [], []
    for t in range(T):
        W0, b0 = params[4 + t * per], params[4 + t * per + 1]
        ops.gemm([(EE, None, W0[:, 2 * F:3 * F])], _cols(Te, sl[t]), bias=b0)
        Wp = params[4 + t * per + 2 * pre_layers]
        if D > 0:
            weffs.append(ops.pna_weff(Wp, F, D, avg_deg_log))
        k = 4 + t * per + 2 * (pre_layers + post_layers - 1)
        last.append((params[k], params[k + 1]))
    Wm = bm = None
    if merged:
        Wm, bm = _merge_last_post_with_lin(lin_w, lin_b, last, sl, BE)
    return EE, Te, weffs, Wm, bm


class BondGradAccumulator:

    def __init__(self, R: int, H: int, device, depth: int):
        self.buf = torch.empty(R, H, dtype=torch.float32, device=device)
        self.depth = depth
        self.encoder = None
        self.defer = False
        self.slab = None
        self.deferred = []

    def layer_slab(self, layer_index: int, R: int, H: int, F: int, T: int, D: int, device):
        per = R * H + R * F + H * H + H + T * D * F * 4 * F
        if self.slab is None:
            self.slab = ops.zeros(R * H + self.depth * per, device=device)
            self.buf = self.slab[:R * H].view(R, H)
        o = R * H + layer_index * per
        out = []
        for n in (R * H, R * F, H * H, H, T * D * F * 4 * F):
            out.append(self.slab[o:o + n])
            o += n
        return out

    def finish_deferred(self, device) -> None:
        if not self.deferred:
            return
        import ctypes as C
        from . import _lib
        d0 = self.deferred[0]
        L = len(self.deferred)
        T, F, pre, post, R, D, merged = d0["T"], d0["F"], d0["pre"], d0["post"], d0["R"], d0["D"], d0["merged"]
        np_ = 4 + T * 2 * (pre + post)
        a = _lib.PnaFinishArgs()
        a.L, a.T, a.F, a.pre_layers, a.post_layers, a.R, a.D, a.merged = L, T, F, pre, post, R, D, int(merged)
        a.use_side_streams = int(ops.wgrad_stream_enabled())
        ones = ops.ones_vector(device, max(R, 1))
        a.BE, a.acc_buf, a.ones = d0["BE"].data_ptr(), self.buf.data_ptr(), ones.data_ptr()
        avg = (C.c_float * L)(*[d["avg"] for d in self.deferred])
        vp = C.c_void_p
        params = (vp * (L * np_))(*[p.data_ptr() for d in self.deferred for p in d["params"]])
        grads = (vp * (L * np_))(*[g.data_ptr() for d in self.deferred for g in d["sinks"]])
        EE = (vp * L)(*[d["EE"].data_ptr() for d in self.deferred])
        dTe = (vp * L)(*[d["dTe"].data_ptr() for d in self.deferred])
        dEE = (vp * L)(*[d["dEE"].data_ptr() for d in self.deferred])
        dWm = (vp * L)(*[d["dWm"].data_ptr() for d in self.deferred])
        dbm = (vp * L)(*[d["dbm"].data_ptr() for d in self.deferred])
        per_w = D * F * 4 * F
        dWeff = (vp * (L * T))(*[d["dWeff"].data_ptr() + 4 * t * per_w for d in self.deferred for t in range(T)])
        a.avg_deg_log = C.cast(avg, C.POINTER(C.c_float))
        for name, arr in (("params", params), ("grads", grads), ("EE", EE), ("dTe", dTe), ("dEE", dEE), ("dWm", dWm),
                          ("dbm", dbm), ("dWeff", dWeff)):
            setattr(a, name, C.cast(arr, C.POINTER(vp)))
        ops.check(_lib.load().gnx_pna_stack_finish(_lib.handle(device), C.byref(a)))
        ops.keep_until_join(device, [self.slab, ones] + [t for d in self.deferred for t in (d["BE"], d["EE"], *d["params"], *d["sinks"])])
        self.deferred = []

    def first_in_backward(self, layer_index: int) -> bool:
        return layer_index == self.depth - 1

    def handoff(self, device) -> Optional[torch.Tensor]:
        if self.encoder is not None:
            idx, offs, weights = self.encoder
            sinks = grad_sinks(weights)
            gtable = adjacent_rows(sinks) if all(g is not None for g in sinks) else None
            if gtable is not None:
                buf = self.buf
                ops.run_on_second_side_stream(buf, [buf, idx, gtable], lambda: ops.embed_sum_bwd(idx, offs, buf, out=gtable))
                return None
        ops.join_side_stream(device, 1)
        return self.buf


class WeightOnlyAhead:

    def __init__(self, BE, T, F, pre_layers, post_layers, avg_deg_log, params, D):
        self.device = BE.device
        box = []
        ops.run_after_wgrads(BE, (), lambda: box.append(_pna_weight_only(BE, T, F, pre_layers, post_layers, avg_deg_log,
                                                                        params, D)))
        self.value = box[0]

    def wait(self):
        ops.join_side_stream(self.device)
        return self.value


class WeightOnlyAll:

    def __init__(self, BE, T, F, pre_layers, post_layers, layers, D):
        import ctypes as C
        from . import _lib
        self.device = BE.device
        L, R, H = len(layers), BE.size(0), T * F
        merged = post_layers > 1
        f32 = dict(dtype=torch.float32, device=BE.device)
        EE = torch.empty(L, R, F, **f32)
        Te = torch.empty(L, R, H, **f32)
        weff = torch.empty(L, T, D, F, 4 * F, **f32) if D > 0 else None
        Wm = torch.empty(L, H, H, **f32) if merged else None
        bm = torch.empty(L, H, **f32) if merged else None
        vp = C.c_void_p
        np_ = len(layers[0][1])
        avg = (C.c_float * L)(*[float(a_) for a_, _ in layers])
        params = (vp * (L * np_))(*[p.data_ptr() for _, ps in layers for p in ps])
        ptrs = lambda t_, n: (vp * n)(*[t_[i].data_ptr() for i in range(n)]) if t_ is not None else None
        a_EE, a_Te, a_Wm, a_bm = ptrs(EE, L), ptrs(Te, L), ptrs(Wm, L), ptrs(bm, L)
        a_weff = (vp * (L * T))(*[weff[l, t].data_ptr() for l in range(L) for t in range(T)]) if weff is not None else None
        cast = lambda arr: None if arr is None else C.cast(arr, C.POINTER(vp))

        def launch():
            ops.check(_lib.load().gnx_pna_weight_only_all(
                _lib.handle(BE.device), L, BE.data_ptr(), R, T, F, pre_layers, post_layers, D,
                C.cast(avg, C.POINTER(C.c_float)), cast(params), int(merged), cast(a_EE), cast(a_Te), cast(a_weff),
                cast(a_Wm), cast(a_bm)))

        keep = [BE, EE, Te, weff, Wm, bm] + [p for _, ps in layers for p in ps]
        ops.run_after_wgrads(BE, keep, launch)
        self.values = [(EE[l], Te[l], [weff[l, t] for t in range(T)] if weff is not None else [],
                        Wm[l] if merged else None, bm[l] if merged else None) for l in range(L)]
        self._joined = False

    def get(self, l: int):
        if not self._joined:
            ops.join_side_stream(self.device)
            self._joined = True
        return self.values[l]


def _merge_last_post_with_lin(lin_w, lin_b, last, sl, like):
    H = lin_w.size(0)
    Wm, bm = _empty(H, H, like), _empty(1, H, like)
    for t, (Wt, _) in enumerate(last):
        ops.gemm([(_cols(lin_w, sl[t]), None, Wt)], _cols(Wm, sl[t]), b_trans=False)
    for t, (_, bt) in enumerate(last):
        ops.gemm([(bt.view(1, -1), None, _cols(lin_w, sl[t]))], bm, bias=lin_b if t == 0 else None, accumulate=t > 0)
    return Wm, bm.view(-1)


def _unmerge_last_post_and_lin(dWm, dbm, lin_w, d_lin_w, d_lin_b, last, last_bias, sl):
    row, col = dbm.view(1, -1), dbm.view(-1, 1)
    for t, (Wt, dWt, dbt) in enumerate(last):
        bt = last_bias[t]
        ops.gemm([(_cols(dWm, sl[t]), None, Wt)], _cols(d_lin_w, sl[t]), accumulate=True)
        ops.gemm([(col, None, bt.view(-1, 1))], _cols(d_lin_w, sl[t]), accumulate=True)
        ops.gemm_wgrad_inline(_cols(lin_w, sl[t]), _cols(dWm, sl[t]), dWt)
        ops.gemm([(row, None, _cols(lin_w, sl[t]))], dbt.view(1, -1), b_trans=False, accumulate=True)
    ops.axpy_(d_lin_b, dbm)


def _pna_forward_native(ctx, x, BE, pack, cfg, params, dc, prep):
    import ctypes as C
    from . import _lib
    T, F, pre_layers, post_layers, avg_deg_log = cfg[:5]
    EE, Te, weffs, Wm, bm = prep
    N, H = x.shape
    E, D = pack.E, dc.D
    dev = x.device
    merged = Wm is not None
    n_z = post_layers - 1 if merged else post_layers
    f32 = dict(dtype=torch.float32, device=dev)
    PQ = torch.empty(2, N, H, **f32)
    hs_all = torch.empty(pre_layers, max(E, 1), H, **f32)
    zs_all = torch.empty(max(n_z, 1), N, H, **f32)
    A = torch.empty(N, T * 4 * F, **f32)
    out = torch.empty(N, H, **f32)
    lib = _lib.load()
    ws_bytes = lib.gnx_pna_conv_bwd_workspace_bytes(T, F, D)
    ws = torch.empty(ws_bytes, dtype=torch.uint8, device=dev)
    a = _lib.PnaFwdArgs()
    a.N, a.E, a.T, a.F, a.pre_layers, a.post_layers, a.D, a.merged = N, E, T, F, pre_layers, post_layers, D, int(merged)
    a.rowptr, a.src, a.dst, a.code = pack.rowptr.data_ptr(), pack.src.data_ptr(), pack.dst.data_ptr(), pack.code.data_ptr()
    a.dperm, a.tiles, a.ntiles, a.max_tiles = dc.dperm.data_ptr(), dc.tiles_p.data_ptr(), dc.ntiles_p.data_ptr(), dc.max_tiles_p
    a.tile_rows = dc.tile_rows_p
    a.x, a.Te = x.data_ptr(), Te.data_ptr()
    for i, w in enumerate(weffs):
        a.weff[i] = w.data_ptr()
    a.Wm, a.bm = (Wm.data_ptr(), bm.data_ptr()) if merged else (None, None)
    n = len(params)
    parr = (C.c_void_p * n)(*[p.data_ptr() for p in params])
    a.params = C.cast(parr, C.POINTER(C.c_void_p))
    a.P, a.Q, a.A = PQ[0].data_ptr(), PQ[1].data_ptr(), A.data_ptr()
    hs = [hs_all[i][:E] if E != hs_all.size(1) else hs_all[i] for i in range(pre_layers)]
    zs = [zs_all[i] for i in range(n_z)]
    for i, t_ in enumerate(hs):
        a.hs[i] = t_.data_ptr()
    for i, t_ in enumerate(zs):
        a.zs[i] = t_.data_ptr()
    a.ws, a.ws_bytes, a.out = ws.data_ptr(), ws_bytes, out.data_ptr()
    etiles = pack.edge_tiles(D - 1) if (_FUSED_EDGE and pre_layers == 2) else None
    a.etile_info, a.etile_w = (etiles[0].data_ptr(), etiles[1]) if etiles is not None else (None, 0)
    ops.check(lib.gnx_pna_conv_fwd(_lib.handle(dev), C.byref(a)))
    amp, att = pack.degree_scalers(avg_deg_log)
    ctx.pack, ctx.cfg = pack, cfg[:5]
    ctx.n_h, ctx.n_z = len(hs), len(zs)
    ctx.sinks = grad_sinks(params)
    ctx.dc, ctx.weffs, ctx.Wm = dc, weffs, Wm
    ctx.save_for_backward(x, BE, EE, A, amp, att, *hs, *zs, *params)
    return out


def _pna_backward_native(ctx, dout, x, BE, EE, A, hs, zs, params, sinks, code_pos):
    import ctypes as C
    from . import _lib
    T, F, pre_layers, post_layers, avg_deg_log = ctx.cfg
    pack, dc, acc = ctx.pack, ctx.dc, ctx.bond_acc
    N, H = x.shape
    E, R, D = pack.E, BE.size(0), dc.D
    dev = x.device
    dout = dout.contiguous()
    merged = ctx.Wm is not None
    n_g = post_layers - 1 if merged else post_layers
    f32 = dict(dtype=torch.float32, device=dev)
    gbuf = torch.empty(max(n_g, 1), N, H, **f32)
    gebuf = torch.empty(pre_layers, max(E, 1), H, **f32)
    dA = torch.empty(N, T * 4 * F, **f32)
    pq = torch.empty(2, N, H, **f32)
    defer = _BATCH_WEIGHT_ONLY and acc is not None and not ops.wgrad_done_hook_set() and \
        (acc.slab is not None or acc.first_in_backward(ctx.layer_index))
    if defer:
        dTe_t, dEE_t, dWm_t, dbm_t, dWeff_t = acc.layer_slab(ctx.layer_index, R, H, F, T, D, dev)
        small = None
    else:
        small = torch.empty(R * H + R * F + H * H + H + T * D * F * 4 * F, **f32)
    dx = torch.empty(N, H, **f32)
    lib = _lib.load()
    ws_bytes = lib.gnx_pna_conv_bwd_workspace_bytes(T, F, D)
    ws = torch.empty(ws_bytes, dtype=torch.uint8, device=dev)
    a = _lib.PnaBwdArgs()
    a.N, a.E, a.T, a.F, a.pre_layers, a.post_layers, a.R, a.D = N, E, T, F, pre_layers, post_layers, R, D
    a.avg_deg_log, a.merged = float(avg_deg_log), int(merged)
# ... 375 lines not shown
```

gnnepcsaft_amd/ops.py:

```python
from __future__ import annotations

import ctypes as C
import threading
from typing import List, Optional, Sequence, Tuple

import torch

from . import _lib
from ._lib import GemmSeg, check, handle

_I32 = C.c_int32


def _f32(t: torch.Tensor, name: str) -> torch.Tensor:
    if t.dtype != torch.float32:
        raise _lib.GnxError(_lib.GNX_E_INVALID, f"{name}: expected float32, got {t.dtype}")
    return t


def _mat(t: torch.Tensor, name: str) -> Tuple[int, int]:
    if t.dtype is not torch.float32:
        raise _lib.GnxError(_lib.GNX_E_INVALID, f"{name}: expected float32, got {t.dtype}")
    shape, strides = t.shape, t.stride()
    if len(shape) != 2 or (shape[1] > 1 and strides[1] != 1):
        raise _lib.GnxError(_lib.GNX_E_INVALID, f"{name}: need a 2-D view with unit column stride, got "
                                                f"shape {tuple(shape)} strides {strides}")
    ld = strides[0]
    return t.data_ptr(), (ld if ld > shape[1] else shape[1])


def _ptr(t: Optional[torch.Tensor]) -> Optional[int]:
    return None if t is None else t.data_ptr()


def _carr(vals: Sequence[int]):
    return (_I32 * len(vals))(*vals)


def zeros(*shape: int, device: torch.device) -> torch.Tensor:
    t = torch.empty(*shape, dtype=torch.float32, device=device)
    return zero_(t)


_ONES: dict = {}


def ones_vector(device: torch.device, n: int) -> torch.Tensor:
    key = device.index if device.index is not None else torch.cuda.current_device()
    t = _ONES.get(key)
    if t is None or t.numel() < n:
        t = torch.empty(max(n, 256), dtype=torch.float32, device=device)
        check(_lib.load().gnx_fill(handle(device), t.data_ptr(), t.numel(), 1.0))
        _ONES[key] = t
    return t


def zero_(t: torch.Tensor) -> torch.Tensor:
    if t.is_cuda and t.dtype is torch.float32 and t.is_contiguous():
        if t.numel():
            check(_lib.load().gnx_fill(handle(t.device), t.data_ptr(), t.numel(), 0.0))
        return t
    return t.zero_()


class GraphPack:

    __slots__ = ("N", "E", "B", "rowptr", "perm", "src", "dst", "colptr", "cpos", "code", "graph_ptr", "device",
                 "_scalers", "has_batch", "_classes", "_code_index", "max_degree_hint", "_edge_tiles")

    EDGE_TILE_ROWS = 64
    EDGE_TILE_MAX_DEG = 16

    def edge_tiles(self, max_degree: int) -> Optional[Tuple[torch.Tensor, int]]:
        if max_degree > GraphPack.EDGE_TILE_MAX_DEG or self.E == 0 or self.N == 0:
            return None
        w = GraphPack.EDGE_TILE_ROWS + 1 - max(int(max_degree), 1)
        hit = self._edge_tiles
        if hit is None or hit[1] != w:
            lib = _lib.load()
            count = lib.gnx_edge_tiles_count(self.E, w)
            info = torch.empty(2 * (count + 1), dtype=torch.int32, device=self.device)
            check(lib.gnx_edge_tiles(handle(self.device), self.rowptr.data_ptr(), self.N, self.E, w, info.data_ptr()))
            hit = self._edge_tiles = (info, w)
        return hit

    def code_index(self, R: int) -> Optional[torch.Tensor]:
        if R > 64:
            return None
        if self._code_index is None or self._code_index[0] != R:
            lib, h = _lib.load(), handle(self.device)
            pos = torch.empty(max(self.E, 1), dtype=torch.int32, device=self.device)
            ptr = torch.empty(R + 1, dtype=torch.int32, device=self.device)
            nbytes = lib.gnx_degree_classes_workspace_bytes(self.E, R)
            ws = torch.empty(nbytes, dtype=torch.uint8, device=self.device)
            check(lib.gnx_group_by_small_key(h, self.code.data_ptr(), self.E, R, pos.data_ptr(), ptr.data_ptr(),
                                             ws.data_ptr(), nbytes))
            self._code_index = (R, pos, ptr)
        return self._code_index[1]

    def degree_classes(self, max_degree_hint: Optional[int] = None) -> Optional["DegreeClasses"]:
        if self._classes is None:
            self._classes = DegreeClasses.build(self, max_degree_hint)
        return self._classes if self._classes.D <= DegreeClasses.MAX_D else None

    def degree_scalers(self, avg_deg_log: float) -> Tuple[torch.Tensor, torch.Tensor]:
        key = float(avg_deg_log)
        hit = self._scalers.get(key)
        if hit is None:
            amp = torch.empty(self.N, dtype=torch.float32, device=self.device)
            att = torch.empty(self.N, dtype=torch.float32, device=self.device)
            check(_lib.load().gnx_degree_scalers(handle(self.device), self.rowptr.data_ptr(), self.N, key,
                                                 amp.data_ptr(), att.data_ptr()))
            hit = (amp, att)
            self._scalers[key] = hit
        return hit


class DegreeClasses:
    MAX_D = 64
    GEMM_ROWS = 128
    WGRAD_ROWS = 1024

    __slots__ = ("D", "dperm", "cls_ptr", "tiles", "ntiles", "max_tiles", "chunks", "nchunks", "max_chunks",
                 "tiles_p", "ntiles_p", "max_tiles_p", "tile_rows_p")

    @staticmethod
    def build(g: "GraphPack", max_degree_hint: Optional[int] = None) -> "DegreeClasses":
        lib, h = _lib.load(), handle(g.device)
        dc = DegreeClasses()
        if max_degree_hint is None:
            mx = _I32(0)
            check(lib.gnx_degree_max(h, g.rowptr.data_ptr(), g.N, C.byref(mx)))
            dc.D = int(mx.value) + 1
        else:
            dc.D = int(max_degree_hint) + 1
        if dc.D > DegreeClasses.MAX_D:
            return dc
        i32 = dict(dtype=torch.int32, device=g.device)
        dc.dperm = torch.empty(max(g.N, 1), **i32)
        dc.cls_ptr = torch.empty(dc.D + 1, **i32)
        nbytes = lib.gnx_degree_classes_workspace_bytes(g.N, dc.D)
        ws = torch.empty(nbytes, dtype=torch.uint8, device=g.device)
        check(lib.gnx_degree_classes(h, g.rowptr.data_ptr(), g.N, dc.D, dc.dperm.data_ptr(), dc.cls_ptr.data_ptr(),
                                     ws.data_ptr(), nbytes))
        dc.max_tiles = g.N // DegreeClasses.GEMM_ROWS + dc.D
        dc.max_chunks = g.N // DegreeClasses.WGRAD_ROWS + dc.D
        dc.tiles = torch.empty(3 * dc.max_tiles, **i32)
        dc.chunks = torch.empty(3 * dc.max_chunks, **i32)
        dc.ntiles = torch.empty(1, **i32)
        dc.nchunks = torch.empty(1, **i32)
        check(lib.gnx_class_tiles(h, dc.cls_ptr.data_ptr(), dc.D, DegreeClasses.GEMM_ROWS, dc.tiles.data_ptr(),
                                  dc.ntiles.data_ptr()))
        check(lib.gnx_class_tiles(h, dc.cls_ptr.data_ptr(), dc.D, DegreeClasses.WGRAD_ROWS, dc.chunks.data_ptr(),
                                  dc.nchunks.data_ptr()))
        dc.tile_rows_p = int(lib.gnx_gemm_tile_rows(h, g.N, 128))
        if dc.tile_rows_p == DegreeClasses.GEMM_ROWS:
            dc.tiles_p, dc.ntiles_p, dc.max_tiles_p = dc.tiles, dc.ntiles, dc.max_tiles
        else:
            dc.max_tiles_p = g.N // dc.tile_rows_p + dc.D
            dc.tiles_p = torch.empty(3 * dc.max_tiles_p, **i32)
            dc.ntiles_p = torch.empty(1, **i32)
            check(lib.gnx_class_tiles(h, dc.cls_ptr.data_ptr(), dc.D, dc.tile_rows_p, dc.tiles_p.data_ptr(),
                                      dc.ntiles_p.data_ptr()))
        return dc


def set_option(device: torch.device, opt: int, value: int) -> int:
    lib, h = _lib.load(), handle(device)
    old = _I32(0)
    check(lib.gnx_get_option(h, opt, C.byref(old)))
    check(lib.gnx_set_option(h, opt, int(value)))
    return int(old.value)


def check_range(device: torch.device) -> None:
    check(_lib.load().gnx_check_range(handle(device)))


def pack_graph(edge_index: torch.Tensor, edge_attr: Optional[torch.Tensor], batch: Optional[torch.Tensor],
               num_nodes: int, num_graphs: Optional[int] = None, bond_dims: Sequence[int] = (5, 6, 2),
               validate: bool = True) -> GraphPack:
    dev = edge_index.device
    lib, h = _lib.load(), handle(dev)
    if edge_index.dtype != torch.int64 or edge_index.dim() != 2 or edge_index.size(0) != 2:
        raise _lib.GnxError(_lib.GNX_E_INVALID, f"edge_index must be int64[2,E], got {edge_index.dtype} "
                                                f"{tuple(edge_index.shape)}")
    edge_index = edge_index.contiguous()
    N, E = int(num_nodes), int(edge_index.size(1))
    i32 = dict(dtype=torch.int32, device=dev)
    g = GraphPack()
    g.N, g.E, g.device, g._scalers, g._classes, g._code_index = N, E, dev, {}, None, None
    g._edge_tiles = None
    g.max_degree_hint = None
    g.rowptr = torch.empty(N + 1, **i32)
    g.colptr = torch.empty(N + 1, **i32)
    g.perm = torch.empty(E, **i32)
    g.src = torch.empty(E, **i32)
    g.dst = torch.empty(E, **i32)
    g.cpos = torch.empty(E, **i32)
    ws_bytes = lib.gnx_pack_csr_workspace_bytes(N, E)
    ws = torch.empty(ws_bytes, dtype=torch.uint8, device=dev)
    check(lib.gnx_pack_csr(h, edge_index.data_ptr(), E, N, g.rowptr.data_ptr(), g.perm.data_ptr(), g.src.data_ptr(),
                           g.dst.data_ptr(), g.colptr.data_ptr(), g.cpos.data_ptr(), ws.data_ptr(), ws_bytes))
    g.code = torch.empty(E, **i32)
    if edge_attr is not None:
        if edge_attr.dtype != torch.int64 or edge_attr.dim() != 2 or edge_attr.size(0) != E or \
                edge_attr.size(1) != len(bond_dims):
            raise _lib.GnxError(_lib.GNX_E_INVALID, f"edge_attr must be int64[E,{len(bond_dims)}], got "
                                                    f"{edge_attr.dtype} {tuple(edge_attr.shape)}")
        edge_attr = edge_attr.contiguous()
        check(lib.gnx_feature_code(h, edge_attr.data_ptr(), E, len(bond_dims), _carr(list(bond_dims)),
                                   g.perm.data_ptr(), g.code.data_ptr(), None, 0))
    else:
        g.code.zero_()
    if batch is not None:
        if batch.dtype != torch.int64 or batch.dim() != 1 or batch.size(0) != N:
            raise _lib.GnxError(_lib.GNX_E_INVALID, f"batch must be int64[N], got {batch.dtype} {tuple(batch.shape)}")
        if num_graphs is None:
            num_graphs = int(batch.max()) + 1 if N > 0 else 0
        g.B = int(num_graphs)
        g.has_batch = True
        g.graph_ptr = torch.empty(g.B + 1, **i32)
        check(lib.gnx_graph_ptr(h, batch.contiguous().data_ptr(), N, g.B, g.graph_ptr.data_ptr(), None, 0))
    else:
        g.B = 1
        g.has_batch = False
        g.graph_ptr = torch.arange(2, **i32) * N
    if validate:
        check_range(dev)
    return g


def embed_sum_fwd(idx: torch.Tensor, table: torch.Tensor, offsets: Sequence[int]) -> torch.Tensor:
    K = len(offsets) - 1
    if idx.dtype != torch.int64 or idx.dim() != 2 or idx.size(1) != K:
        raise _lib.GnxError(_lib.GNX_E_INVALID, f"embedding index must be int64[N,{K}], got {idx.dtype} "
                                                f"{tuple(idx.shape)}")
    idx = idx.contiguous()
    table = _f32(table, "table").contiguous()
    N, H = idx.size(0), table.size(1)
    out = torch.empty(N, H, dtype=torch.float32, device=table.device)
    check(_lib.load().gnx_embed_sum_fwd(handle(table.device), idx.data_ptr(), N, K, _carr(list(offsets)),
                                        table.data_ptr(), H, out.data_ptr()))
    return out


def embed_sum_bwd(idx: torch.Tensor, offsets: Sequence[int], dout: torch.Tensor,
                  out: Optional[torch.Tensor] = None) -> torch.Tensor:
    K, R = len(offsets) - 1, offsets[-1]
    dout = _f32(dout, "dout").contiguous()
    idx = idx.contiguous()
    H = dout.size(1)
    if out is not None:
        if out.shape != (R, H) or not out.is_contiguous() or out.dtype is not torch.float32:
            raise _lib.GnxError(_lib.GNX_E_INVALID, f"embed_sum_bwd: out must be contiguous fp32 [{R},{H}]")
        dtable = out
    else:
        dtable = zeros(R, H, device=dout.device)
    lib = _lib.load()
    nbytes = lib.gnx_table_scatter_workspace_bytes(idx.size(0), R, H)
    ws = torch.empty(max(nbytes, 1), dtype=torch.uint8, device=dout.device)
    check(lib.gnx_embed_sum_bwd(handle(dout.device), idx.data_ptr(), idx.size(0), K, _carr(list(offsets)), R,
                                dout.data_ptr(), H, dtable.data_ptr(), ws.data_ptr(), nbytes))
    return dtable


Seg = Tuple[torch.Tensor, Optional[torch.Tensor], torch.Tensor]


class _SegArrays(threading.local):

    def __init__(self):
        self.by_len = {n: (GemmSeg * n)() for n in range(1, 5)}


_SEG_ARRAYS = _SegArrays()


def gemm(segs: Sequence[Seg], out: torch.Tensor, *, bias: Optional[torch.Tensor] = None,
         mask: Optional[torch.Tensor] = None, relu: bool = False, accumulate: bool = False,
         b_trans: bool = True) -> torch.Tensor:
    M, N = out.shape
    if M == 0:
        return out
    cptr, ldc = _mat(out, "out")
    arr = _SEG_ARRAYS.by_len[len(segs)]
    for i, (a, rs, b) in enumerate(segs):
        ap, lda = _mat(a, "A")
        bp, ldb = _mat(b, "B")
        (am, k), (b0, b1) = a.shape, b.shape
        if am != M or (b_trans and (b0 != N or b1 != k)) or (not b_trans and (b0 != k or b1 != N)):
            raise _lib.GnxError(_lib.GNX_E_INVALID, f"gemm segment {i}: A {tuple(a.shape)} B {tuple(b.shape)} "
                                                    f"out {tuple(out.shape)} b_trans={b_trans}")
        e = arr[i]
        e.a, e.lda, e.rowscale = ap, lda, (None if rs is None else rs.data_ptr())
        e.b, e.ldb, e.k = bp, ldb, k
    flags = (_lib.GEMM_RELU if relu else 0) | (_lib.GEMM_ACCUMULATE if accumulate else 0) | \
            (_lib.GEMM_B_TRANS if b_trans else 0)
    mp, ldm = (None, 0) if mask is None else _mat(mask, "mask")
    lib, h = _lib.load(), handle(out.device)
    nbytes = lib.gnx_gemm_workspace_bytes(h, len(segs), arr, None, 1, M, N, mp, flags, 0) if M >= 4096 else 0
    ws = torch.empty(nbytes, dtype=torch.uint8, device=out.device) if nbytes else None
    check(lib.gnx_gemm(h, len(segs), arr, M, N, _ptr(bias), mp, ldm, cptr, ldc, flags, _ptr(ws), nbytes))
    return out


GSeg = Tuple[torch.Tensor, Optional[torch.Tensor], torch.Tensor, int]
# ... 235 lines not shown

def pna_conv_bwd(args: "_lib.PnaBwdArgs", device: torch.device) -> None:
    check(_lib.load().gnx_pna_conv_bwd(handle(device), C.byref(args)))


def run_on_second_side_stream(ref: torch.Tensor, tensors, fn) -> None:
    _run_on_side(ref, tensors, fn, which=1)


def gemm_wgrad_inline(dC: torch.Tensor, A: torch.Tensor, dW: torch.Tensor, dbias: Optional[torch.Tensor] = None) -> None:
    _gemm_wgrad_launch(dC, A, dW, None, dbias)


def axpy_(y: torch.Tensor, x: torch.Tensor, alpha: float = 1.0) -> torch.Tensor:
    if y.numel() != x.numel() or not (y.is_contiguous() and x.is_contiguous()):
        raise _lib.GnxError(_lib.GNX_E_INVALID, "axpy_: need contiguous tensors of equal size")
    check(_lib.load().gnx_axpy(handle(y.device), _f32(y, "y").data_ptr(), _f32(x, "x").data_ptr(), y.numel(),
                               float(alpha)))
    return y


def gemm_wgrad(dC: torch.Tensor, A: torch.Tensor, dW: torch.Tensor, *, rowscale: Optional[torch.Tensor] = None,
               dbias: Optional[torch.Tensor] = None) -> None:
    if dC.size(0) == 0:
        return
    _run_on_side(dC, (dC, A, rowscale, dW, dbias), lambda: _gemm_wgrad_launch(dC, A, dW, rowscale, dbias))


def pna_post0_wgrad_classes(g: torch.Tensor, A: torch.Tensor, dc: "DegreeClasses", F: int, avg_deg_log: float,
                            dW: torch.Tensor) -> None:
    if g.size(0) == 0:
        return
    dWeff = zeros(dc.D, F, 4 * F, device=g.device)

    def run():
        gemm_wgrad_grouped(g, A, dWeff, dc)
        pna_weff_bwd(dWeff, F, dc.D, avg_deg_log, dW)

    _run_on_side(g, (g, A, dWeff, dW), run)


def _gemm_wgrad_launch(dC, A, dW, rowscale, dbias) -> None:
    M, N = dC.shape
    xp, ldx = _mat(dC, "dC")
    ap, lda = _mat(A, "A")
    wp, ldw = _mat(dW, "dW")
    K = A.size(1)
    if A.size(0) != M or dW.size(0) != N or dW.size(1) != K:
        raise _lib.GnxError(_lib.GNX_E_INVALID, f"wgrad shapes dC {tuple(dC.shape)} A {tuple(A.shape)} "
                                                f"dW {tuple(dW.shape)}")
    check(_lib.load().gnx_gemm_wgrad(handle(dW.device), xp, ldx, ap, lda, _ptr(rowscale), M, N, K, wp, ldw,
                                     _ptr(dbias)))


def edge_combine_fwd(P: torch.Tensor, Q: torch.Tensor, Te: torch.Tensor, g: GraphPack, relu: bool) -> torch.Tensor:
    H = P.size(1)
    h1 = torch.empty(g.E, H, dtype=torch.float32, device=P.device)
    check(_lib.load().gnx_edge_combine_fwd(handle(P.device), P.data_ptr(), Q.data_ptr(), Te.data_ptr(),
                                           g.src.data_ptr(), g.dst.data_ptr(), g.code.data_ptr(), g.E, H, int(relu),
                                           h1.data_ptr()))
    return h1


def edge_combine_bwd_pq(gr: torch.Tensor, g: GraphPack) -> Tuple[torch.Tensor, torch.Tensor]:
    H = gr.size(1)
    dP = torch.empty(g.N, H, dtype=torch.float32, device=gr.device)
    dQ = torch.empty(g.N, H, dtype=torch.float32, device=gr.device)
    check(_lib.load().gnx_edge_combine_bwd(handle(gr.device), gr.data_ptr(), g.rowptr.data_ptr(), g.colptr.data_ptr(),
                                           g.cpos.data_ptr(), g.code.data_ptr(), g.N, g.E, H, 0, dP.data_ptr(),
                                           dQ.data_ptr(), None, None, 0))
    return dP, dQ


def bond_table_grad(gr: torch.Tensor, g: GraphPack, R: int, pos: Optional[torch.Tensor]) -> torch.Tensor:
    H = gr.size(1)
    dTe = zeros(R, H, device=gr.device)
    lib = _lib.load()
    if g.E == 0:
        return dTe
    if pos is not None:
        check(lib.gnx_key_segment_sum(handle(gr.device), gr.data_ptr(), pos.data_ptr(), g.code.data_ptr(), g.E, H,
                                      dTe.data_ptr()))
        return dTe
    nbytes = lib.gnx_table_scatter_workspace_bytes(g.E, R, H)
    ws = torch.empty(max(nbytes, 1), dtype=torch.uint8, device=gr.device)
    tmp = torch.empty(2, g.N, H, dtype=torch.float32, device=gr.device)
    check(lib.gnx_edge_combine_bwd(handle(gr.device), gr.data_ptr(), g.rowptr.data_ptr(), g.colptr.data_ptr(),
                                   g.cpos.data_ptr(), g.code.data_ptr(), g.N, g.E, H, R, tmp[0].data_ptr(),
                                   tmp[1].data_ptr(), dTe.data_ptr(), ws.data_ptr(), nbytes))
    return dTe


def bond_code_index(g: GraphPack, R: int, H: int) -> Optional[torch.Tensor]:
    return g.code_index(R) if ((H % 4 == 0 and H <= 1024) or H <= 256) and g.E > 0 else None


def edge_combine_bwd(gr: torch.Tensor, g: GraphPack, R: int) -> Tuple[torch.Tensor, torch.Tensor, torch.Tensor]:
    dP, dQ = edge_combine_bwd_pq(gr, g)
    return dP, dQ, bond_table_grad(gr, g, R, bond_code_index(g, R, gr.size(1)))


def pna_edge_fwd(P: torch.Tensor, Q: torch.Tensor, Te: torch.Tensor, g: GraphPack, T: int, F: int,
                 weights: Sequence[torch.Tensor], biases: Sequence[torch.Tensor], max_degree: int,
                 keep: bool = True) -> Tuple[Optional[torch.Tensor], Optional[torch.Tensor], torch.Tensor]:
    H = T * F
    tiles = g.edge_tiles(max_degree)
    if tiles is None and g.E > 0:
        raise _lib.GnxError(_lib.GNX_E_INVALID, f"pna_edge_fwd: in-degree bound {max_degree} too large for edge tiles")
    dev = P.device
    h1 = torch.empty(g.E, H, dtype=torch.float32, device=dev) if keep else None
    m = torch.empty(g.E, H, dtype=torch.float32, device=dev) if keep else None
    A = torch.empty(g.N, T * 4 * F, dtype=torch.float32, device=dev)
    warr = (C.c_void_p * T)(*[_f32(w, "W1").data_ptr() for w in weights])
    barr = (C.c_void_p * T)(*[_f32(b, "b1").data_ptr() for b in biases])
    for w in weights:
        if tuple(w.shape) != (F, F) or not w.is_contiguous():
            raise _lib.GnxError(_lib.GNX_E_INVALID, f"pna_edge_fwd: pre-layer 1 weight must be contiguous [{F},{F}]")
    info, w_ = tiles if tiles is not None else (None, 1)
    check(_lib.load().gnx_pna_edge_fwd(handle(dev), P.data_ptr(), Q.data_ptr(), Te.data_ptr(), g.src.data_ptr(),
                                       g.dst.data_ptr(), g.code.data_ptr(), g.rowptr.data_ptr(), _ptr(info), w_, g.N, g.E,
                                       T, F, C.cast(warr, C.POINTER(C.c_void_p)), C.cast(barr, C.POINTER(C.c_void_p)),
                                       _ptr(h1), _ptr(m), A.data_ptr()))
    return h1, m, A


def pna_edge_bwd(ge: torch.Tensor, h1: torch.Tensor, g: GraphPack, T: int, F: int, R: int,
                 weights: Sequence[torch.Tensor], max_degree: int) -> Tuple[torch.Tensor, torch.Tensor, torch.Tensor]:
    H = T * F
    tiles = g.edge_tiles(max_degree)
    if tiles is None and g.E > 0:
        raise _lib.GnxError(_lib.GNX_E_INVALID, f"pna_edge_bwd: in-degree bound {max_degree} too large for edge tiles")
    dev = ge.device
    gh1 = torch.empty(g.E, H, dtype=torch.float32, device=dev)
    dP = torch.empty(g.N, H, dtype=torch.float32, device=dev)
    dTe = zeros(R, H, device=dev)
    warr = (C.c_void_p * T)(*[_f32(w, "W1").data_ptr() for w in weights])
    info, w_ = tiles if tiles is not None else (None, 1)
    check(_lib.load().gnx_pna_edge_bwd(handle(dev), _f32(ge, "ge").contiguous().data_ptr(), _f32(h1, "h1").contiguous().data_ptr(),
                                       g.code.data_ptr(), g.rowptr.data_ptr(), _ptr(info), w_, g.N, g.E, T, F, R,
                                       C.cast(warr, C.POINTER(C.c_void_p)), gh1.data_ptr(), dP.data_ptr(), dTe.data_ptr()))
    return gh1, dP, dTe


def pna_aggregate_fwd(m: torch.Tensor, g: GraphPack, T: int, F: int) -> torch.Tensor:
    A = torch.empty(g.N, T * 4 * F, dtype=torch.float32, device=m.device)
    check(_lib.load().gnx_pna_aggregate_fwd(handle(m.device), m.data_ptr(), g.rowptr.data_ptr(), g.N, g.E, T, F,
                                            A.data_ptr()))
    return A


def pna_aggregate_bwd(dA: torch.Tensor, m: torch.Tensor, A: torch.Tensor, g: GraphPack, T: int, F: int) -> torch.Tensor:
    dm = torch.empty_like(m)
    check(_lib.load().gnx_pna_aggregate_bwd(handle(m.device), dA.data_ptr(), m.data_ptr(), A.data_ptr(),
                                            g.rowptr.data_ptr(), g.N, g.E, T, F, dm.data_ptr()))
    return dm


def gine_aggregate_fwd(x: torch.Tensor, Le: torch.Tensor, g: GraphPack, eps: float) -> torch.Tensor:
    out = torch.empty_like(x)
    check(_lib.load().gnx_gine_aggregate_fwd(handle(x.device), x.data_ptr(), Le.data_ptr(), g.rowptr.data_ptr(),
                                             g.src.data_ptr(), g.code.data_ptr(), g.N, g.E, x.size(1), float(eps),
                                             out.data_ptr()))
    return out


def gine_aggregate_bwd(dout: torch.Tensor, x: torch.Tensor, Le: torch.Tensor, g: GraphPack,
                       eps: float, want_dle: bool = True) -> Tuple[torch.Tensor, Optional[torch.Tensor]]:
    dx = torch.empty_like(x)
    dLe = zeros(*Le.shape, device=Le.device) if want_dle else None
    pos = g.code_index(Le.size(0)) if (g.E > 0 and want_dle) else None
    check(_lib.load().gnx_gine_aggregate_bwd(handle(x.device), dout.data_ptr(), x.data_ptr(), Le.data_ptr(),
                                             g.colptr.data_ptr(), g.cpos.data_ptr(), g.src.data_ptr(),
                                             g.dst.data_ptr(), g.code.data_ptr(), _ptr(pos), g.N, g.E, x.size(1),
                                             Le.size(0), float(eps), dx.data_ptr(), _ptr(dLe)))
    return dx, dLe


def gine_dle(dout: torch.Tensor, x: torch.Tensor, Le: torch.Tensor, g: GraphPack, pos: Optional[torch.Tensor]) -> torch.Tensor:
    dLe = zeros(*Le.shape, device=Le.device)
    check(_lib.load().gnx_gine_dle(handle(x.device), dout.data_ptr(), x.data_ptr(), Le.data_ptr(), g.src.data_ptr(),
                                   g.dst.data_ptr(), g.code.data_ptr(), _ptr(pos), g.E, x.size(1), Le.size(0),
                                   dLe.data_ptr()))
    return dLe


def transformer_attn_fwd(qkvs: torch.Tensor, Le: torch.Tensor, g: GraphPack, heads: int, p: float = 0.0,
                         seed: int = 0, offset: int = 0, want_mask: bool = False
                         ) -> Tuple[torch.Tensor, torch.Tensor, Optional[torch.Tensor]]:
    qkvs = _f32(qkvs, "qkvs").contiguous()
    Le = _f32(Le, "Le").contiguous()
    N, H = qkvs.size(0), qkvs.size(1) // 4
    if qkvs.size(1) != 4 * H or Le.size(1) != H or heads <= 0 or H % heads != 0:
        raise _lib.GnxError(_lib.GNX_E_INVALID, f"transformer_attn_fwd: qkvs {tuple(qkvs.shape)} Le {tuple(Le.shape)} "
                                                f"heads {heads}")
    dev = qkvs.device
    out = torch.empty(N, H, dtype=torch.float32, device=dev)
    alpha = torch.empty(g.E, heads, dtype=torch.float32, device=dev)
    keep = torch.empty(g.E, heads, dtype=torch.uint8, device=dev) if want_mask else None
    check(_lib.load().gnx_transformer_attn_fwd(handle(dev), qkvs.data_ptr(), Le.data_ptr(), g.rowptr.data_ptr(),
                                               g.src.data_ptr(), g.code.data_ptr(), N, g.E, int(heads), H // int(heads),
                                               float(p), int(seed) & (2 ** 64 - 1), int(offset) & (2 ** 64 - 1),
                                               out.data_ptr(), alpha.data_ptr(), _ptr(keep)))
    return out, alpha, keep


def transformer_attn_bwd(dout: torch.Tensor, qkvs: torch.Tensor, Le: torch.Tensor, alpha: torch.Tensor, g: GraphPack,
                         heads: int, p: float = 0.0, seed: int = 0, offset: int = 0, want_dle: bool = True
                         ) -> Tuple[torch.Tensor, torch.Tensor, Optional[torch.Tensor]]:
    dout = _f32(dout, "dout").contiguous()
    N, H = dout.shape
    dev = dout.device
    dqkv = torch.empty(N, 3 * H, dtype=torch.float32, device=dev)
    scratch = torch.empty(2, g.E, heads, dtype=torch.float32, device=dev)
    dLe = zeros(*Le.shape, device=dev) if want_dle else None
    pos = g.code_index(Le.size(0)) if (want_dle and g.E > 0) else None
    if want_dle and g.E > 0 and pos is None:
        raise _lib.GnxError(_lib.GNX_E_INVALID, f"transformer_attn_bwd: {Le.size(0)} bond codes exceed the inverted index")
    check(_lib.load().gnx_transformer_attn_bwd(handle(dev), dout.data_ptr(), qkvs.data_ptr(), Le.data_ptr(),
                                               alpha.data_ptr(), g.rowptr.data_ptr(), g.src.data_ptr(), g.dst.data_ptr(),
                                               g.code.data_ptr(), g.colptr.data_ptr(), g.cpos.data_ptr(), _ptr(pos), N,
                                               g.E, int(heads), H // int(heads), Le.size(0), float(p),
                                               int(seed) & (2 ** 64 - 1), int(offset) & (2 ** 64 - 1), dqkv.data_ptr(),
                                               scratch.data_ptr(), _ptr(dLe)))
    return dqkv, scratch, dLe


def transformer_attn_dle(dout: torch.Tensor, qkvs: torch.Tensor, scratch: torch.Tensor, Le: torch.Tensor, g: GraphPack,
                         heads: int, pos: Optional[torch.Tensor]) -> torch.Tensor:
    R, H = Le.shape
    dLe = zeros(R, H, device=dout.device)
    if g.E == 0:
        return dLe
    if pos is None:
        raise _lib.GnxError(_lib.GNX_E_INVALID, f"transformer_attn_dle: {R} bond codes exceed the inverted index")
    check(_lib.load().gnx_transformer_attn_dle(handle(dout.device), dout.data_ptr(), qkvs.data_ptr(), scratch.data_ptr(),
                                               g.dst.data_ptr(), g.code.data_ptr(), pos.data_ptr(), g.E, int(heads),
                                               H // int(heads), R, dLe.data_ptr()))
    return dLe


def _f64_on(t: torch.Tensor, name: str, dev: torch.device) -> torch.Tensor:
    if t.dtype != torch.float64 or t.device != dev:
        raise _lib.GnxError(_lib.GNX_E_INVALID, f"{name}: expected float64 on {dev}, got {t.dtype} on {t.device}")
    return t.contiguous()


def _pcsaft_args(params: torch.Tensor, owner: torch.Tensor, T: torch.Tensor, name: str):
    dev = params.device
    params = _f64_on(params, f"{name}: params", dev)
    if params.dim() != 2 or params.size(1) != 9:
        raise _lib.GnxError(_lib.GNX_E_INVALID, f"{name}: params must be [B, 9], got {tuple(params.shape)}")
    if owner.dtype != torch.int64 or owner.device != dev or owner.dim() != 1:
        raise _lib.GnxError(_lib.GNX_E_INVALID, f"{name}: owner must be a 1-D int64 tensor on {dev}")
    T = _f64_on(T, f"{name}: T", dev)
    if T.shape != owner.shape:
        raise _lib.GnxError(_lib.GNX_E_INVALID, f"{name}: T {tuple(T.shape)} and owner {tuple(owner.shape)} differ")
    return params, owner.contiguous(), T


def pcsaft_density(params: torch.Tensor, owner: torch.Tensor, T: torch.Tensor, P: torch.Tensor
                   ) -> Tuple[torch.Tensor, torch.Tensor]:
    params, owner, T = _pcsaft_args(params, owner, T, "pcsaft_density")
    P = _f64_on(P, "pcsaft_density: P", params.device)
    if P.shape != T.shape:
        raise _lib.GnxError(_lib.GNX_E_INVALID, f"pcsaft_density: P {tuple(P.shape)} and T {tuple(T.shape)} differ")
    n, dev = T.numel(), params.device
    rho = torch.empty(n, dtype=torch.float64, device=dev)
    status = torch.empty(n, dtype=torch.int32, device=dev)
    check(_lib.load().gnx_pcsaft_density(handle(dev), params.data_ptr(), params.size(0), owner.data_ptr(),
                                         T.data_ptr(), P.data_ptr(), n, rho.data_ptr(), status.data_ptr()))
    return rho, status


def pcsaft_vapor_pressure(params: torch.Tensor, owner: torch.Tensor, T: torch.Tensor
                          ) -> Tuple[torch.Tensor, torch.Tensor, torch.Tensor, torch.Tensor]:
    params, owner, T = _pcsaft_args(params, owner, T, "pcsaft_vapor_pressure")
    n, dev = T.numel(), params.device
    out = torch.empty(3, n, dtype=torch.float64, device=dev)
    status = torch.empty(n, dtype=torch.int32, device=dev)
    check(_lib.load().gnx_pcsaft_vapor_pressure(handle(dev), params.data_ptr(), params.size(0), owner.data_ptr(),
                                                T.data_ptr(), n, out[0].data_ptr(), out[1].data_ptr(),
                                                out[2].data_ptr(), status.data_ptr()))
    return out[0], out[1], out[2], status


_POOL = {"add": _lib.POOL_ADD, "sum": _lib.POOL_ADD, "mean": _lib.POOL_MEAN, "max": _lib.POOL_MAX}


def segment_pool_fwd(x: torch.Tensor, ptr: torch.Tensor, B: int, mode: str) -> torch.Tensor:
    out = torch.empty(B, x.size(1), dtype=torch.float32, device=x.device)
    check(_lib.load().gnx_segment_pool_fwd(handle(x.device), x.data_ptr(), ptr.data_ptr(), B, x.size(1), _POOL[mode],
                                           out.data_ptr()))
    return out


def segment_pool_bwd(dout: torch.Tensor, x: torch.Tensor, out: torch.Tensor, ptr: torch.Tensor, B: int,
                     mode: str) -> torch.Tensor:
    dx = torch.empty_like(x)
    check(_lib.load().gnx_segment_pool_bwd(handle(x.device), dout.data_ptr(), x.data_ptr(), out.data_ptr(),
                                           ptr.data_ptr(), B, x.size(1), _POOL[mode], dx.data_ptr()))
    return dx


def _bn_ws(M: int, H: int, dev) -> Tuple[torch.Tensor, int]:
    nbytes = _lib.load().gnx_batchnorm_workspace_bytes(M, H)
    return torch.empty(nbytes, dtype=torch.uint8, device=dev), nbytes


def batchnorm_fwd(x, gamma, beta, running_mean, running_var, momentum: float, eps: float, training: bool, relu: bool,
                  num_batches_tracked: Optional[torch.Tensor] = None):
    M, H = x.shape
    y = torch.empty_like(x)
    mean = torch.empty(H, dtype=torch.float32, device=x.device)
    rstd = torch.empty(H, dtype=torch.float32, device=x.device)
    ws, nbytes = _bn_ws(M, H, x.device)
    check(_lib.load().gnx_batchnorm_fwd(handle(x.device), x.data_ptr(), M, H, _ptr(gamma), _ptr(beta),
                                        _ptr(running_mean), _ptr(running_var), _ptr(num_batches_tracked),
                                        float(momentum), float(eps),
                                        int(training), int(relu), y.data_ptr(), mean.data_ptr(), rstd.data_ptr(),
                                        ws.data_ptr(), nbytes))
    return y, mean, rstd


def batchnorm_bwd(dy, x, y, gamma, mean, rstd, relu: bool, dgamma=None, dbeta=None):
    M, H = x.shape
    dx = torch.empty_like(x)
    if dgamma is None:
        dgamma = zeros(H, device=x.device)
    if dbeta is None:
        dbeta = zeros(H, device=x.device)
    ws, nbytes = _bn_ws(M, H, x.device)
    check(_lib.load().gnx_batchnorm_bwd(handle(x.device), dy.data_ptr(), x.data_ptr(), y.data_ptr(), M, H, _ptr(gamma),
                                        mean.data_ptr(), rstd.data_ptr(), int(relu), dx.data_ptr(), dgamma.data_ptr(),
                                        dbeta.data_ptr(), ws.data_ptr(), nbytes))
    return dx, dgamma, dbeta


def dropout(x: torch.Tensor, p: float, seed: int, offset: int) -> torch.Tensor:
    x = _f32(x, "x").contiguous()
    y = torch.empty_like(x)
    check(_lib.load().gnx_dropout(handle(x.device), x.data_ptr(), x.numel(), float(p), int(seed) & (2 ** 64 - 1),
                                  int(offset) & (2 ** 64 - 1), y.data_ptr()))
    return y


def huber_ape(pred: torch.Tensor, target: torch.Tensor, delta: float, need_grad: bool):
    pred = _f32(pred, "pred").contiguous()
    target = _f32(target, "target").contiguous()
    if pred.shape != target.shape:
        raise _lib.GnxError(_lib.GNX_E_INVALID, f"pred {tuple(pred.shape)} vs target {tuple(target.shape)}")
    out2 = torch.empty(2, dtype=torch.float32, device=pred.device)
    dpred = torch.empty_like(pred) if need_grad else None
    check(_lib.load().gnx_huber_ape(handle(pred.device), pred.data_ptr(), target.data_ptr(), pred.numel(), float(delta),
                                    out2.data_ptr(), _ptr(dpred)))
    return out2, dpred


def clip_rows(x: torch.Tensor, lo: torch.Tensor, hi: torch.Tensor) -> torch.Tensor:
    x = _f32(x, "x").contiguous()
    y = torch.empty_like(x)
    check(_lib.load().gnx_clip_rows(handle(x.device), x.data_ptr(), x.size(0), x.size(1), lo.data_ptr(), hi.data_ptr(),
                                    y.data_ptr()))
    return y


def prof_begin(device: torch.device, kernel_ids: Sequence[int]) -> None:
    mask = 0
    for k in kernel_ids:
        mask |= 1 << k
    check(_lib.load().gnx_prof_begin(handle(device), mask))


def prof_read(device: torch.device, kernel_id: int) -> Tuple[int, float]:
    d = prof_read_work(device, kernel_id)
    return d["launches"], d["ms"]


def prof_read_work(device: torch.device, kernel_id: int) -> dict:
    n, ms = C.c_int64(0), C.c_double(0.0)
    by, fl, mf = C.c_double(0.0), C.c_double(0.0), C.c_double(0.0)
    check(_lib.load().gnx_prof_read(handle(device), kernel_id, C.byref(n), C.byref(ms), C.byref(by), C.byref(fl),
                                    C.byref(mf)))
    return {"launches": n.value, "ms": ms.value, "bytes": by.value, "flops": fl.value, "mfma_bf16_flops": mf.value}


def prof_end(device: torch.device) -> None:
    check(_lib.load().gnx_prof_end(handle(device)))
```

include/gnx.h:

```cpp
#ifndef GNX_H_
#define GNX_H_

#include <stddef.h>
#include <stdint.h>

#ifdef __cplusplus
extern "C" {
#endif

#define GNX_ABI_VERSION 6

enum {
  GNX_OK = 0,
  GNX_E_INVALID = -1,
  GNX_E_HIP = -2,
  GNX_E_RANGE = -3,
  GNX_E_WORKSPACE = -4
};

typedef struct gnx_handle gnx_handle;

int32_t gnx_create(gnx_handle** out, int32_t device);
int32_t gnx_destroy(gnx_handle* h);
int32_t gnx_set_stream(gnx_handle* h, void* hip_stream);
const char* gnx_last_error(void);
int32_t gnx_abi_version(void);

enum {
  GNX_OPT_GEMM_SPLIT = 0,
  GNX_OPT_WGRAD_WGS = 1,
  GNX_OPT_EMBED_BWD_MFMA = 2,
  GNX_OPT_STD_BWD_CENTERED = 3,
  GNX_OPT_GEMM_PIPE = 4,
  GNX_OPT_WGRAD_PIPE = 5,
  GNX_OPT_GEMM_AS = 6,
  GNX_OPT_GEMM_WS_FAST = 7,
  GNX_OPT_GEMM_TILE_ROWS = 8,
  GNX_OPT_GEMM_MID = 9,
  GNX_OPT_COUNT = 10
};
int32_t gnx_set_option(gnx_handle* h, int32_t opt, int32_t value);
int32_t gnx_get_option(gnx_handle* h, int32_t opt, int32_t* value);

enum {
  GNX_K_NONE = 0,
  GNX_K_PNA_AGG_FWD = 1,
  GNX_K_PNA_AGG_BWD = 2,
  GNX_K_GEMM_WS = 3,
  GNX_K_GEMM_WGRAD = 4,
  GNX_K_GINE_AGG_FWD = 5,
  GNX_K_GINE_AGG_BWD = 6,
  GNX_K_EDGE_COMBINE_FWD = 7,
  GNX_K_EDGE_COMBINE_BWD = 8,
  GNX_K_BN_FWD = 9,
  GNX_K_BN_BWD = 10,
  GNX_K_GEMM_TILED = 11,
  GNX_K_GEMM_SMALL = 12,
  GNX_K_GEMM_WGRAD_BATCHED = 13,
  GNX_K_KEY_SEGMENT_SUM = 14,
  GNX_K_EMBED = 15,
  GNX_K_PNA_EDGE_FWD = 16,
  GNX_K_PNA_EDGE_BWD = 17,
  GNX_K_ATTN_FWD = 18,
  GNX_K_ATTN_BWD = 19,
  GNX_K_PCSAFT_RHO = 20,
  GNX_K_PCSAFT_VP = 21,
  GNX_K_COUNT = 22
};
int32_t gnx_prof_begin(gnx_handle* h, uint32_t kernel_mask);
int32_t gnx_prof_read(gnx_handle* h, int32_t kid, int64_t* launches, double* total_ms, double* alg_bytes,
                      double* alg_flops, double* mfma_bf16_flops);
int32_t gnx_prof_end(gnx_handle* h);

size_t gnx_pack_csr_workspace_bytes(int64_t N, int64_t E);
int32_t gnx_pack_csr(gnx_handle* h, const int64_t* edge_index, int64_t E, int64_t N, int32_t* rowptr, int32_t* perm,
                     int32_t* src, int32_t* dst, int32_t* colptr, int32_t* cpos, void* ws, size_t ws_bytes);
int32_t gnx_feature_code(gnx_handle* h, const int64_t* feat, int64_t rows, int32_t K, const int32_t* dims,
                         const int32_t* perm, int32_t* code, void* ws, size_t ws_bytes);
int32_t gnx_graph_ptr(gnx_handle* h, const int64_t* batch, int64_t N, int64_t B, int32_t* graph_ptr, void* ws,
                      size_t ws_bytes);
int32_t gnx_degree_scalers(gnx_handle* h, const int32_t* rowptr, int64_t N, float avg_deg_log, float* amp, float* att);

int32_t gnx_embed_sum_fwd(gnx_handle* h, const int64_t* idx, int64_t N, int32_t K, const int32_t* offsets,
                          const float* table, int32_t H, float* out);
size_t gnx_table_scatter_workspace_bytes(int64_t rows, int32_t R, int32_t H);
int32_t gnx_embed_sum_bwd(gnx_handle* h, const int64_t* idx, int64_t N, int32_t K, const int32_t* offsets,
                          int32_t R, const float* dout, int32_t H, float* dtable, void* ws, size_t ws_bytes);
int32_t gnx_check_range(gnx_handle* h);

typedef struct {
  const float* a;
  int64_t lda;
  const float* rowscale;
  const float* b;
  int64_t ldb;
  int32_t k;
  int32_t _pad;
} gnx_gemm_seg;

enum {
  GNX_GEMM_RELU = 1,
  GNX_GEMM_ACCUMULATE = 2,
  GNX_GEMM_B_TRANS = 4,
  GNX_GEMM_SPLIT_ONLY = 8,
  GNX_GEMM_PRESPLIT = 16
};
size_t gnx_gemm_workspace_bytes(gnx_handle* h, int32_t nseg, const gnx_gemm_seg* segs, const int64_t* cls_strides,
                                int32_t num_classes, int64_t M, int32_t N, const float* mask, int32_t flags,
                                int32_t grouped);
int32_t gnx_gemm(gnx_handle* h, int32_t nseg, const gnx_gemm_seg* segs, int64_t M, int32_t N, const float* bias,
                 const float* mask, int64_t ldmask, float* C, int64_t ldc, int32_t flags, void* ws, size_t ws_bytes);
int32_t gnx_gemm_wgrad(gnx_handle* h, const float* dC, int64_t lddc, const float* A, int64_t lda,
                       const float* rowscale, int64_t M, int32_t N, int32_t K, float* dW, int64_t lddw, float* dbias);

typedef struct {
  const float* dC;
  int64_t lddc;
  const float* A;
  int64_t lda;
  const float* rowscale;
  float* dW;
  int64_t lddw;
  float* dbias;
  int64_t M;
  int32_t N, K;
} gnx_wgrad_prob;
int32_t gnx_gemm_wgrad_batched(gnx_handle* h, int32_t nprob, const gnx_wgrad_prob* probs);

enum { GNX_SB_A_TRANS = 1, GNX_SB_B_TRANS = 2, GNX_SB_ACCUMULATE = 4, GNX_SB_ATOMIC = 8, GNX_SB_RELU = 16 };
#define GNX_SMALL_BATCH 32
typedef struct {
  const float* A;
  int64_t lda;
  const float* B;
  int64_t ldb;
  const float* bias;
  float* C;
  int64_t ldc;
  int32_t M, N, K;
  int32_t flags;
} gnx_small_prob;
int32_t gnx_gemm_small_batched(gnx_handle* h, int32_t nprob, const gnx_small_prob* probs);

int32_t gnx_degree_max(gnx_handle* h, const int32_t* rowptr, int64_t N, int32_t* max_degree_host);
size_t gnx_degree_classes_workspace_bytes(int64_t N, int32_t D);
int32_t gnx_degree_classes(gnx_handle* h, const int32_t* rowptr, int64_t N, int32_t D, int32_t* dperm,
                           int32_t* cls_ptr, void* ws, size_t ws_bytes);
int32_t gnx_class_tiles(gnx_handle* h, const int32_t* cls_ptr, int32_t D, int32_t tile_rows, int32_t* tile_info,
                        int32_t* ntiles);
int32_t gnx_gemm_grouped(gnx_handle* h, int32_t nseg, const gnx_gemm_seg* segs, const int64_t* cls_strides,
                         int32_t num_classes, int64_t M, int32_t N, const float* bias, const float* mask,
                         int64_t ldmask, float* C, int64_t ldc, int32_t flags, const int32_t* row_index,
                         const int32_t* tile_info, const int32_t* ntiles, int64_t max_tiles, void* ws, size_t ws_bytes);
int32_t gnx_gemm_tile_rows(gnx_handle* h, int64_t M, int32_t N);
int32_t gnx_gemm_grouped_rows(gnx_handle* h, int32_t nseg, const gnx_gemm_seg* segs, const int64_t* cls_strides,
                              int32_t num_classes, int64_t M, int32_t N, const float* bias, const float* mask,
                              int64_t ldmask, float* C, int64_t ldc, int32_t flags, const int32_t* row_index,
                              const int32_t* tile_info, const int32_t* ntiles, int64_t max_tiles, void* ws,
                              size_t ws_bytes, int32_t tile_rows);
int32_t gnx_gemm_wgrad_grouped(gnx_handle* h, const float* dC, int64_t lddc, const float* A, int64_t lda, int64_t M,
                               int32_t N, int32_t K, float* dW_cls, int64_t lddw, int64_t dw_cls_stride,
                               const int32_t* row_index, const int32_t* chunk_info, const int32_t* nchunks,
                               int64_t max_chunks);
int32_t gnx_pna_weff(gnx_handle* h, const float* W, int64_t ldw, int32_t F, int32_t D, float avg_deg_log, float* Weff);
int32_t gnx_pna_weff_bwd(gnx_handle* h, const float* dWeff, int32_t F, int32_t D, float avg_deg_log, float* dW,
                         int64_t lddw);
int32_t gnx_pna_weff_batched(gnx_handle* h, int32_t n, const float* const* W, int64_t ldw, int32_t F, int32_t D,
                             const float* avg_deg_log, float* const* Weff);
int32_t gnx_pna_weff_bwd_batched(gnx_handle* h, int32_t n, const float* const* dWeff, int32_t F, int32_t D,
                                 const float* avg_deg_log, float* const* dW, int64_t lddw);

int32_t gnx_edge_combine_fwd(gnx_handle* h, const float* P, const float* Q, const float* Te, const int32_t* src,
                             const int32_t* dst, const int32_t* code, int64_t E, int32_t H, int32_t relu, float* h1);
int32_t gnx_edge_combine_bwd(gnx_handle* h, const float* g, const int32_t* rowptr, const int32_t* colptr,
                             const int32_t* cpos, const int32_t* code, int64_t N, int64_t E, int32_t H, int32_t R,
                             float* dP, float* dQ, float* dTe, void* ws, size_t ws_bytes);

int32_t gnx_group_by_small_key(gnx_handle* h, const int32_t* keys, int64_t E, int32_t R, int32_t* pos, int32_t* ptr,
                               void* ws, size_t ws_bytes);
int32_t gnx_key_segment_sum(gnx_handle* h, const float* g, const int32_t* pos, const int32_t* key, int64_t E, int32_t H,
                            float* dtable);

int32_t gnx_pna_aggregate_fwd(gnx_handle* h, const float* m, const int32_t* rowptr, int64_t N, int64_t E, int32_t T,
                              int32_t F, float* A);
int32_t gnx_pna_aggregate_bwd(gnx_handle* h, const float* dA, const float* m, const float* A, const int32_t* rowptr,
                              int64_t N, int64_t E, int32_t T, int32_t F, float* dm);

int32_t gnx_edge_tiles_count(int64_t E, int32_t tile_w);
int32_t gnx_edge_tiles(gnx_handle* h, const int32_t* rowptr, int64_t N, int64_t E, int32_t tile_w, int32_t* tile_info);
int32_t gnx_pna_edge_bwd(gnx_handle* h, const float* ge, const float* h1, const int32_t* code, const int32_t* rowptr,
                         const int32_t* tile_info, int32_t tile_w, int64_t N, int64_t E, int32_t T, int32_t F, int32_t R,
                         const float* const* W1, float* gh1, float* dP, float* dTe);
int32_t gnx_pna_edge_fwd(gnx_handle* h, const float* P, const float* Q, const float* Te, const int32_t* src,
                         const int32_t* dst, const int32_t* code, const int32_t* rowptr, const int32_t* tile_info,
                         int32_t tile_w, int64_t N, int64_t E, int32_t T, int32_t F, const float* const* W1,
                         const float* const* b1, float* h1, float* m, float* A);

int32_t gnx_gine_aggregate_fwd(gnx_handle* h, const float* x, const float* Le, const int32_t* rowptr,
                               const int32_t* src, const int32_t* code, int64_t N, int64_t E, int32_t H, float eps,
                               float* out);
int32_t gnx_gine_aggregate_bwd(gnx_handle* h, const float* dout, const float* x, const float* Le,
                               const int32_t* colptr, const int32_t* cpos, const int32_t* src, const int32_t* dst,
                               const int32_t* code, const int32_t* code_pos, int64_t N, int64_t E, int32_t H, int32_t R,
                               float eps, float* dx, float* dLe);

int32_t gnx_gine_dle(gnx_handle* h, const float* dout, const float* x, const float* Le, const int32_t* src,
                     const int32_t* dst, const int32_t* code, const int32_t* code_pos, int64_t E, int32_t H, int32_t R,
                     float* dLe);

int32_t gnx_transformer_attn_fwd(gnx_handle* h, const float* qkvs, const float* Le, const int32_t* rowptr,
                                 const int32_t* src, const int32_t* code, int64_t N, int64_t E, int32_t heads,
                                 int32_t C, float p, uint64_t seed, uint64_t offset, float* out, float* alpha,
                                 uint8_t* keep);
int32_t gnx_transformer_attn_bwd(gnx_handle* h, const float* dout, const float* qkvs, const float* Le,
                                 const float* alpha, const int32_t* rowptr, const int32_t* src, const int32_t* dst,
                                 const int32_t* code, const int32_t* colptr, const int32_t* cpos,
                                 const int32_t* code_pos, int64_t N, int64_t E, int32_t heads, int32_t C, int32_t R,
                                 float p, uint64_t seed, uint64_t offset, float* dqkv, float* scratch, float* dLe);
int32_t gnx_transformer_attn_dle(gnx_handle* h, const float* dout, const float* qkvs, const float* scratch,
                                 const int32_t* dst, const int32_t* code, const int32_t* code_pos, int64_t E,
                                 int32_t heads, int32_t C, int32_t R, float* dLe);

int32_t gnx_pcsaft_density(gnx_handle* h, const double* params, int64_t B, const int64_t* owner, const double* T,
                           const double* P, int64_t n, double* rho, int32_t* status);
int32_t gnx_pcsaft_vapor_pressure(gnx_handle* h, const double* params, int64_t B, const int64_t* owner, const double* T,
                                  int64_t n, double* psat, double* rho_l, double* rho_v, int32_t* status);

enum { GNX_POOL_ADD = 0, GNX_POOL_MEAN = 1, GNX_POOL_MAX = 2 };
int32_t gnx_segment_pool_fwd(gnx_handle* h, const float* x, const int32_t* ptr, int64_t B, int32_t H, int32_t mode,
                             float* out);
int32_t gnx_segment_pool_bwd(gnx_handle* h, const float* dout, const float* x, const float* out, const int32_t* ptr,
                             int64_t B, int32_t H, int32_t mode, float* dx);

size_t gnx_batchnorm_workspace_bytes(int64_t M, int32_t H);
int32_t gnx_batchnorm_fwd(gnx_handle* h, const float* x, int64_t M, int32_t H, const float* gamma, const float* beta,
                          float* running_mean, float* running_var, int64_t* num_batches_tracked, float momentum,
                          float eps, int32_t training, int32_t relu, float* y, float* save_mean, float* save_rstd,
                          void* ws, size_t ws_bytes);
int32_t gnx_batchnorm_bwd(gnx_handle* h, const float* dy, const float* x, const float* y, int64_t M, int32_t H,
                          const float* gamma, const float* save_mean, const float* save_rstd, int32_t relu,
                          float* dx, float* dgamma, float* dbeta, void* ws, size_t ws_bytes);

int32_t gnx_dropout(gnx_handle* h, const float* x, int64_t n, float p, uint64_t seed, uint64_t offset, float* y);

int32_t gnx_huber_ape(gnx_handle* h, const float* pred, const float* target, int64_t count, float delta, float* out2,
                      float* dpred);

int32_t gnx_adamw_amsgrad(gnx_handle* h, float* p, const float* g, float* m, float* v, float* vmax, int64_t n, float lr,
                          float beta1, float beta2, float eps, float weight_decay, int64_t step);
int32_t gnx_sgd(gnx_handle* h, float* p, const float* g, int64_t n, float lr);

#define GNX_PNA_MAX_LAYERS 8
#define GNX_PNA_MAX_TOWERS 8
enum {
  GNX_PNA_BWD_DEFER_SMALL = 1,
  GNX_PNA_BWD_LAST_OF_PASS = 2
};
typedef struct {
  int64_t N, E;
  int32_t T, F, pre_layers, post_layers, R, D;
  float avg_deg_log;
  int32_t merged;
  int32_t acc_first;
  int32_t use_side_streams;
  int32_t n_h, n_z;
  const int32_t *rowptr, *colptr, *cpos, *code, *code_pos, *dperm, *tiles, *ntiles, *chunks, *nchunks;
  int64_t max_tiles, max_chunks;
  const float *x, *BE, *EE, *A;
  const float* hs[GNX_PNA_MAX_LAYERS];
  const float* zs[GNX_PNA_MAX_LAYERS];
  const float* weff[GNX_PNA_MAX_TOWERS];
  const float* Wm;
  const float* const* params;
  float* const* grads;
  const float* dout;
  float* gbuf[GNX_PNA_MAX_LAYERS];
  float* dA;
  float* gebuf[GNX_PNA_MAX_LAYERS];
  float *dP, *dQ;
  float *dTe, *dEE;
  float *dWm, *dbm;
  float* dWeff;
  void* ws;
  size_t ws_bytes;
  float* acc_buf;
  float* dx;
  int32_t flags;
  int32_t etile_w;
  const int32_t* etile_info;
} gnx_pna_bwd_args;
size_t gnx_pna_conv_bwd_workspace_bytes(int32_t T, int32_t F, int32_t D);
int32_t gnx_pna_conv_bwd(gnx_handle* h, const gnx_pna_bwd_args* args);

typedef struct {
  int32_t L, T, F, pre_layers, post_layers, R, D, merged, use_side_streams, _pad;
  const float* BE;
  float* acc_buf;
  const float* ones;
  const float* avg_deg_log;
  const float* const* params;
  float* const* grads;
  const float* const* EE;
  float* const* dTe;
  float* const* dEE;
  const float* const* dWm;
  const float* const* dbm;
  const float* const* dWeff;
} gnx_pna_finish_args;
int32_t gnx_pna_stack_finish(gnx_handle* h, const gnx_pna_finish_args* args);
int32_t gnx_pna_weight_only_all(gnx_handle* h, int32_t L, const float* BE, int32_t R, int32_t T, int32_t F,
                                int32_t pre_layers, int32_t post_layers, int32_t D, const float* avg_deg_log,
                                const float* const* params, int32_t merged, float* const* EE, float* const* Te,
                                float* const* weff, float* const* Wm, float* const* bm);

int32_t gnx_pna_weight_only(gnx_handle* h, const float* BE, int32_t R, int32_t T, int32_t F, int32_t pre_layers,
                            int32_t post_layers, int32_t D, float avg_deg_log, const float* const* params, int32_t merged,
                            float* EE, float* Te, float* const* weff, float* Wm, float* bm);
typedef struct {
  int64_t N, E;
  int32_t T, F, pre_layers, post_layers, D, merged;
  const int32_t *rowptr, *src, *dst, *code, *dperm, *tiles, *ntiles;
  int64_t max_tiles;
  const float *x, *Te;
  const float* weff[GNX_PNA_MAX_TOWERS];
  const float *Wm, *bm;
  const float* const* params;
  float *P, *Q, *A;
  float* hs[GNX_PNA_MAX_LAYERS];
  float* zs[GNX_PNA_MAX_LAYERS];
  void* ws;
  size_t ws_bytes;
  float* out;
  const int32_t* etile_info;
  int32_t etile_w;
  int32_t tile_rows;
} gnx_pna_fwd_args;
int32_t gnx_pna_conv_fwd(gnx_handle* h, const gnx_pna_fwd_args* args);

int32_t gnx_fill(gnx_handle* h, float* p, int64_t n, float v);
int32_t gnx_scale(gnx_handle* h, float* p, int64_t n, float v);
int32_t gnx_axpy(gnx_handle* h, float* y, const float* x, int64_t n, float a);

int32_t gnx_side_begin(gnx_handle* h);
int32_t gnx_side_stream(gnx_handle* h, void** hip_stream);
int32_t gnx_side_end(gnx_handle* h);
int32_t gnx_side_join(gnx_handle* h);
int32_t gnx_side_stream_n(gnx_handle* h, int32_t which, void** hip_stream);
int32_t gnx_side_begin_n(gnx_handle* h, int32_t which);
int32_t gnx_side_join_n(gnx_handle* h, int32_t which);
int32_t gnx_clip_rows(gnx_handle* h, const float* x, int64_t M, int32_t P, const float* lo, const float* hi, float* y);

#ifdef __cplusplus
}
#endif
#endif
```

Before: 642,900 graphs/s.

## Fuse batchnorm finalize into partial kernel, restructure CSR packing, cache BN workspace

Batchnorm forward now folds the per-chunk partial sums and computes mean, rstd and affine coefficients inside the partial kernel, using a last-block ticket counter, so the separate finalize launch goes away. Backward takes beta, which points to it recomputing or reusing the affine output. CSR packing is rebuilt around count/scan/fill/sort kernels that count source degrees while gathering, replacing two generic group-by-key passes. The BN workspace is cached per device and stream and zero-initialized so the counters start clean; in exchange the code relies on atomic ticket counters and an in-kernel sort.

Result: slower. 606,400 graphs/s (-5.7%).

```diff
diff --git a/gnnepcsaft_amd/_lib.py b/gnnepcsaft_amd/_lib.py
--- a/gnnepcsaft_amd/_lib.py
+++ b/gnnepcsaft_amd/_lib.py
@@ -104,6 +104,8 @@
                              C.POINTER(C.c_double), C.POINTER(C.c_double)]),
     "gnx_prof_end": (_i32, [_vp]),
     "gnx_pack_csr_workspace_bytes": (_sz, [_i64, _i64]),
+    "gnx_scan_workspace_bytes": (_sz, [_i64]),
+    "gnx_exclusive_scan": (_i32, [_vp, _vp, _i64, _vp, _vp, _sz]),
     "gnx_pack_csr": (_i32, [_vp, _vp, _i64, _i64, _vp, _vp, _vp, _vp, _vp, _vp, _vp, _sz]),
     "gnx_feature_code": (_i32, [_vp, _vp, _i64, _i32, C.POINTER(_i32), _vp, _vp, _vp, _sz]),
     "gnx_graph_ptr": (_i32, [_vp, _vp, _i64, _i64, _vp, _vp, _sz]),
@@ -158,7 +160,7 @@
     "gnx_batchnorm_workspace_bytes": (_sz, [_i64, _i32]),
     "gnx_batchnorm_fwd": (_i32, [_vp, _vp, _i64, _i32, _vp, _vp, _vp, _vp, _vp, _f32, _f32, _i32, _i32, _vp, _vp, _vp,
                                  _vp, _sz]),
-    "gnx_batchnorm_bwd": (_i32, [_vp, _vp, _vp, _vp, _i64, _i32, _vp, _vp, _vp, _i32, _vp, _vp, _vp, _vp, _sz]),
+    "gnx_batchnorm_bwd": (_i32, [_vp, _vp, _vp, _vp, _i64, _i32, _vp, _vp, _vp, _vp, _i32, _vp, _vp, _vp, _vp, _sz]),
     "gnx_dropout": (_i32, [_vp, _vp, _i64, _f32, C.c_uint64, C.c_uint64, _vp]),
     "gnx_huber_ape": (_i32, [_vp, _vp, _vp, _i64, _f32, _vp, _vp]),
     "gnx_adamw_amsgrad": (_i32, [_vp, _vp, _vp, _vp, _vp, _vp, _i64, _f32, _f32, _f32, _f32, _f32, _i64]),
diff --git a/gnnepcsaft_amd/csrc/gnx_norm.hip b/gnnepcsaft_amd/csrc/gnx_norm.hip
--- a/gnnepcsaft_amd/csrc/gnx_norm.hip
+++ b/gnnepcsaft_amd/csrc/gnx_norm.hip
@@ -1,18 +1,148 @@
 #include "gnx_common.hpp"
 
 #define BN_ROWS_PER_BLOCK 256
+#define BN_COLS_V4 128
+#define BN_COLS_S 64
+
+static inline size_t bn_counter_ints(int32_t H) { return (size_t)gnx_cdiv(gnx_cdiv(H, BN_COLS_S), 64) * 64; }
 
 extern "C" size_t gnx_batchnorm_workspace_bytes(int64_t M, int32_t H) {
   if (M < 0) M = 0;
+  if (H < 1) H = 1;
   size_t chunks = (size_t)gnx_cdiv(M > 0 ? M : 1, BN_ROWS_PER_BLOCK);
-  return sizeof(float) * ((size_t)4 * H + chunks * 2 * (size_t)H) + 256;
-}
-
-__global__ void __launch_bounds__(256) k_bn_partial(const float* __restrict__ x, int64_t M, int H,
-                                                    float* __restrict__ part) {
+  return sizeof(int) * bn_counter_ints(H) + sizeof(float) * ((size_t)4 * H + chunks * 2 * (size_t)H) + 256;
+}
+
+__device__ __forceinline__ void bn_ab(float mean, float rstd, float gamma, float beta, float& a, float& b) {
+  a = rstd * gamma;
+  b = beta - mean * a;
+}
+__device__ __forceinline__ float bn_affine(float x, float a, float b) { return x * a + b; }
+
+__device__ __forceinline__ bool bn_last_ticket(int* counter, unsigned total) {
+  __shared__ int s_last;
+  __threadfence();
+  __syncthreads();
+  if (threadIdx.x == 0) {
+    const int last = atomicAdd(counter, 1) == (int)total - 1;
+    if (last) atomicExch(counter, 0);
+    s_last = last;
+  }
+  __syncthreads();
+  if (!s_last) return false;
+  __threadfence();
+  return true;
+}
+
+template <int G, bool V4>
+__device__ __forceinline__ void bn_fold_load(const float* part, int64_t row, int H, int c0, float (&v)[G]) {
+  if constexpr (V4) {
+#pragma unroll
+    for (int q = 0; q < G; q += 4) {
+      f32x4 w = {0.f, 0.f, 0.f, 0.f};
+      if (c0 + q < H) w = *reinterpret_cast<const f32x4*>(part + row * H + c0 + q);
+      v[q] = w.x;
+      v[q + 1] = w.y;
+      v[q + 2] = w.z;
+      v[q + 3] = w.w;
+    }
+  } else {
+#pragma unroll
+    for (int j = 0; j < G; ++j) v[j] = (c0 + j < H) ? part[row * H + c0 + j] : 0.f;
+  }
+}
+
+template <int G, bool V4>
+__device__ __forceinline__ void bn_fold(const float* part, int64_t chunks, int H, int col0, int& c, float& t1,
+                                        float& t2) {
+  const int ly = threadIdx.x & 15, c0 = col0 + (threadIdx.x >> 4) * G;
+  float a1[G], a2[G];
+#pragma unroll
+  for (int j = 0; j < G; ++j) a1[j] = a2[j] = 0.f;
+  int64_t b = ly;
+  for (; b + 48 < chunks; b += 64) {
+    float p[4][G], q[4][G];
+#pragma unroll
+    for (int u = 0; u < 4; ++u) {
+      bn_fold_load<G, V4>(part, (b + 16 * u) * 2 + 0, H, c0, p[u]);
+      bn_fold_load<G, V4>(part, (b + 16 * u) * 2 + 1, H, c0, q[u]);
+    }
+#pragma unroll
+    for (int u = 0; u < 4; ++u)
+#pragma unroll
+      for (int j = 0; j < G; ++j) {
+        a1[j] += p[u][j];
+        a2[j] += q[u][j];
+      }
+  }
+  for (; b < chunks; b += 16) {
+    float p[G], q[G];
+    bn_fold_load<G, V4>(part, b * 2 + 0, H, c0, p);
+    bn_fold_load<G, V4>(part, b * 2 + 1, H, c0, q);
+#pragma unroll
+    for (int j = 0; j < G; ++j) {
+      a1[j] += p[j];
+      a2[j] += q[j];
+    }
+  }
+  t1 = 0.f;
+  t2 = 0.f;
+#pragma unroll
+  for (int j = 0; j < G; ++j) {
+    float u1 = 0.f, u2 = 0.f;
+#pragma unroll
+    for (int l = 0; l < 16; ++l) {
+      u1 += __shfl(a1[j], l, 16);
+      u2 += __shfl(a2[j], l, 16);
+    }
+    if (ly == j) {
+      t1 = u1;
+      t2 = u2;
+    }
+  }
+  c = (ly < G && c0 + ly < H) ? c0 + ly : -1;
+}
+
+struct bn_fwd_fin {
+  const float *gamma, *beta;
+  float *running_mean, *running_var;
+  float momentum, eps;
+  float *save_mean, *save_rstd, *ab;
+  int64_t* num_batches_tracked;
+  int* counters;
+};
+
+template <int G, bool V4>
+__device__ __forceinline__ void bn_fwd_finalize(const bn_fwd_fin& f, const float* x, const float* part, int64_t M, int H) {
+  if (!bn_last_ticket(f.counters + blockIdx.y, gridDim.x)) return;
+  if (f.num_batches_tracked != nullptr && blockIdx.y == 0 && threadIdx.x == 0) f.num_batches_tracked[0] += 1;
+  int c;
+  float t1, t2;
+  bn_fold<G, V4>(part, gridDim.x, H, blockIdx.y * (16 * G), c, t1, t2);
+  if (c < 0) return;
+  const float inv = 1.0f / (float)M;
+  const float d = t1 * inv;
+  const float mean = x[c] + d;
+  const float var = fmaxf(t2 * inv - d * d, 0.f);
+  if (f.running_mean) f.running_mean[c] = (1.f - f.momentum) * f.running_mean[c] + f.momentum * mean;
+  if (f.running_var) {
+    float unb = (M > 1) ? var * ((float)M / (float)(M - 1)) : var;
+    f.running_var[c] = (1.f - f.momentum) * f.running_var[c] + f.momentum * unb;
+  }
+  const float rstd = 1.0f / sqrtf(var + f.eps);
+  if (f.save_mean) f.save_mean[c] = mean;
+  if (f.save_rstd) f.save_rstd[c] = rstd;
+  float a, bb;
+  bn_ab(mean, rstd, f.gamma ? f.gamma[c] : 1.f, f.beta ? f.beta[c] : 0.f, a, bb);
+  f.ab[c] = a;
+  f.ab[H + c] = bb;
+}
+
+__global__ void __launch_bounds__(256) k_bn_partial(const float* __restrict__ x, int64_t M, int H, float* part,
+                                                    bn_fwd_fin fin) {
   __shared__ float s1[4][64], s2[4][64];
   const int cx = threadIdx.x & 63, ry = threadIdx.x >> 6;
-  const int col = blockIdx.y * 64 + cx;
+  const int col = blockIdx.y * BN_COLS_S + cx;
   int64_t r0 = (int64_t)blockIdx.x * BN_ROWS_PER_BLOCK;
   int64_t r1 = r0 + BN_ROWS_PER_BLOCK;
   if (r1 > M) r1 = M;
@@ -34,14 +164,14 @@
     part[((int64_t)blockIdx.x * 2 + 0) * H + col] = t1;
     part[((int64_t)blockIdx.x * 2 + 1) * H + col] = t2;
   }
-}
-
-
-__global__ void __launch_bounds__(256) k_bn_partial_v4(const float* __restrict__ x, int64_t M, int H,
-                                                       float* __restrict__ part) {
+  bn_fwd_finalize<BN_COLS_S / 16, false>(fin, x, part, M, H);
+}
+
+__global__ void __launch_bounds__(256) k_bn_partial_v4(const float* __restrict__ x, int64_t M, int H, float* part,
+                                                       bn_fwd_fin fin) {
   __shared__ f32x4 s1[8][32], s2[8][32];
   const int cq = threadIdx.x & 31, ry = threadIdx.x >> 5;
-  const int col = blockIdx.y * 128 + cq * 4;
+  const int col = blockIdx.y * BN_COLS_V4 + cq * 4;
   int64_t r0 = (int64_t)blockIdx.x * BN_ROWS_PER_BLOCK;
   int64_t r1 = r0 + BN_ROWS_PER_BLOCK;
   if (r1 > M) r1 = M;
@@ -87,165 +217,22 @@
     *reinterpret_cast<f32x4*>(part + ((int64_t)blockIdx.x * 2 + 0) * H + col) = t1;
     *reinterpret_cast<f32x4*>(part + ((int64_t)blockIdx.x * 2 + 1) * H + col) = t2;
   }
-}
-
-__global__ void __launch_bounds__(256) k_bn_bwd_partial_v4(const float* __restrict__ dy, const float* __restrict__ x,
-                                                           const float* __restrict__ y, int64_t M, int H,
-                                                           const float* __restrict__ mean,
-                                                           const float* __restrict__ rstd, int relu,
-                                                           float* __restrict__ part) {
-  __shared__ f32x4 s1[8][32], s2[8][32];
-  const int cq = threadIdx.x & 31, ry = threadIdx.x >> 5;
-  const int col = blockIdx.y * 128 + cq * 4;
-  int64_t r0 = (int64_t)blockIdx.x * BN_ROWS_PER_BLOCK;
-  int64_t r1 = r0 + BN_ROWS_PER_BLOCK;
-  if (r1 > M) r1 = M;
-  f32x4 a1 = {0.f, 0.f, 0.f, 0.f}, a2 = {0.f, 0.f, 0.f, 0.f};
-  if (col < H) {
-    const f32x4 mu = *reinterpret_cast<const f32x4*>(mean + col);
-    const f32x4 rs = *reinterpret_cast<const f32x4*>(rstd + col);
-    auto row = [&](int64_t r, f32x4& g, f32x4& xv, f32x4& yv) {
-      g = *reinterpret_cast<const f32x4*>(dy + r * H + col);
-      xv = *reinterpret_cast<const f32x4*>(x + r * H + col);
-      yv = *reinterpret_cast<const f32x4*>((relu ? y : x) + r * H + col);
-    };
-    auto fold = [&](f32x4 g, const f32x4& xv, const f32x4& yv) {
-      if (relu) {
-        g.x = yv.x > 0.f ? g.x : 0.f;
-        g.y = yv.y > 0.f ? g.y : 0.f;
-        g.z = yv.z > 0.f ? g.z : 0.f;
-        g.w = yv.w > 0.f ? g.w : 0.f;
-      }
-      a1 += g;
-      a2 += g * ((xv - mu) * rs);
-    };
-    int64_t r = r0 + ry;
-    for (; r + 8 < r1; r += 16) {
-      f32x4 g0, x0, y0, g1, x1, y1;
-      row(r, g0, x0, y0);
-      row(r + 8, g1, x1, y1);
-      fold(g0, x0, y0);
-      fold(g1, x1, y1);
-    }
-    for (; r < r1; r += 8) {
-      f32x4 g, xv, yv;
-      row(r, g, xv, yv);
-      fold(g, xv, yv);
-    }
-  }
-  s1[ry][cq] = a1;
-  s2[ry][cq] = a2;
-  __syncthreads();
-  if (ry == 0 && col < H) {
-    f32x4 t1 = s1[0][cq], t2 = s2[0][cq];
-#pragma unroll
-    for (int l = 1; l < 8; ++l) {
-      t1 += s1[l][cq];
-      t2 += s2[l][cq];
-    }
-    *reinterpret_cast<f32x4*>(part + ((int64_t)blockIdx.x * 2 + 0) * H + col) = t1;
-    *reinterpret_cast<f32x4*>(part + ((int64_t)blockIdx.x * 2 + 1) * H + col) = t2;
-  }
-}
-
-template <int VEC>
-__global__ void __launch_bounds__(256) k_bn_bwd_apply_v(const float* __restrict__ dy, const float* __restrict__ x,
-                                                        const float* __restrict__ y, int64_t total, int H,
-                                                        const float* __restrict__ mean, const float* __restrict__ rstd,
-                                                        const float* __restrict__ coef, int relu,
-                                                        float* __restrict__ dx) {
-  int64_t i = ((int64_t)blockIdx.x * blockDim.x + threadIdx.x) * 4;
-  const int64_t stride = (int64_t)gridDim.x * blockDim.x * 4;
-  for (; i < total; i += stride) {
-    const int c = (int)(i % H);
-    f32x4 g = *reinterpret_cast<const f32x4*>(dy + i);
-    const f32x4 xv = *reinterpret_cast<const f32x4*>(x + i);
-    if (relu) {
-      const f32x4 yv = *reinterpret_cast<const f32x4*>(y + i);
-      g.x = yv.x > 0.f ? g.x : 0.f;
-      g.y = yv.y > 0.f ? g.y : 0.f;
-      g.z = yv.z > 0.f ? g.z : 0.f;
-      g.w = yv.w > 0.f ? g.w : 0.f;
-    }
-    const f32x4 mu = *reinterpret_cast<const f32x4*>(mean + c), rs = *reinterpret_cast<const f32x4*>(rstd + c);
-    const f32x4 k0 = *reinterpret_cast<const f32x4*>(coef + c), k1 = *reinterpret_cast<const f32x4*>(coef + H + c),
-                k2 = *reinterpret_cast<const f32x4*>(coef + 2 * H + c);
-    const f32x4 xh = (xv - mu) * rs;
-    *reinterpret_cast<f32x4*>(dx + i) = k0 * (g - k1 - xh * k2);
-  }
-}
-
-__device__ __forceinline__ void bn_fold(const float* __restrict__ part, int64_t chunks, int H, int c, float& t1,
-                                        float& t2) {
-  __shared__ float f1[16][17], f2[16][17];
-  const int cx = threadIdx.x & 15, ly = threadIdx.x >> 4;
-  float a1 = 0.f, a2 = 0.f;
-  if (c < H) {
-    int64_t b = ly;
-    for (; b + 48 < chunks; b += 64) {
-      const float p0 = part[(b * 2 + 0) * H + c], q0 = part[(b * 2 + 1) * H + c];
-      const float p1 = part[((b + 16) * 2 + 0) * H + c], q1 = part[((b + 16) * 2 + 1) * H + c];
-      const float p2 = part[((b + 32) * 2 + 0) * H + c], q2 = part[((b + 32) * 2 + 1) * H + c];
-      const float p3 = part[((b + 48) * 2 + 0) * H + c], q3 = part[((b + 48) * 2 + 1) * H + c];
-      a1 += p0;
-      a2 += q0;
-      a1 += p1;
-      a2 += q1;
-      a1 += p2;
-      a2 += q2;
-      a1 += p3;
-      a2 += q3;
-    }
-    for (; b < chunks; b += 16) {
-      a1 += part[(b * 2 + 0) * H + c];
-      a2 += part[(b * 2 + 1) * H + c];
-    }
-  }
-  f1[ly][cx] = a1;
-  f2[ly][cx] = a2;
-  __syncthreads();
-  t1 = 0.f;
-  t2 = 0.f;
-  if (ly == 0) {
-#pragma unroll
-    for (int l = 0; l < 16; ++l) {
-      t1 += f1[l][cx];
-      t2 += f2[l][cx];
-    }
-  }
-}
-
-__global__ void k_bn_finalize(const float* __restrict__ x, const float* __restrict__ part, int64_t chunks, int64_t M,
-                              int H, const float* __restrict__ gamma, const float* __restrict__ beta,
-                              float* __restrict__ running_mean, float* __restrict__ running_var, float momentum,
-                              float eps, int training, float* __restrict__ save_mean, float* __restrict__ save_rstd,
-                              float* __restrict__ ab, int64_t* __restrict__ num_batches_tracked) {
-  const int c = blockIdx.x * 16 + (threadIdx.x & 15);
-  if (training && num_batches_tracked != nullptr && blockIdx.x == 0 && threadIdx.x == 0) num_batches_tracked[0] += 1;
-  float t1 = 0.f, t2 = 0.f;
-  if (training) bn_fold(part, chunks, H, c, t1, t2);
-  if (c >= H || (threadIdx.x >> 4) != 0) return;
-  float mean, var;
-  if (training) {
-    const float inv = 1.0f / (float)M;
-    const float d = t1 * inv;
-    mean = x[c] + d;
-    var = fmaxf(t2 * inv - d * d, 0.f);
-    if (running_mean) running_mean[c] = (1.f - momentum) * running_mean[c] + momentum * mean;
-    if (running_var) {
-      float unb = (M > 1) ? var * ((float)M / (float)(M - 1)) : var;
-      running_var[c] = (1.f - momentum) * running_var[c] + momentum * unb;
-    }
-  } else {
-    mean = running_mean[c];
-    var = running_var[c];
-  }
-  float rstd = 1.0f / sqrtf(var + eps);
+  bn_fwd_finalize<BN_COLS_V4 / 16, true>(fin, x, part, M, H);
+}
+
+__global__ void k_bn_eval_ab(int H, const float* __restrict__ gamma, const float* __restrict__ beta,
+                             const float* __restrict__ running_mean, const float* __restrict__ running_var, float eps,
+                             float* __restrict__ save_mean, float* __restrict__ save_rstd, float* __restrict__ ab) {
+  const int c = blockIdx.x * blockDim.x + threadIdx.x;
+  if (c >= H) return;
+  const float mean = running_mean[c];
+  const float rstd = 1.0f / sqrtf(running_var[c] + eps);
   if (save_mean) save_mean[c] = mean;
   if (save_rstd) save_rstd[c] = rstd;
-  float a = rstd * (gamma ? gamma[c] : 1.f);
+  float a, b;
+  bn_ab(mean, rstd, gamma ? gamma[c] : 1.f, beta ? beta[c] : 0.f, a, b);
   ab[c] = a;
-  ab[H + c] = (beta ? beta[c] : 0.f) - mean * a;
+  ab[H + c] = b;
 }
 
 template <int VEC>
@@ -259,7 +246,8 @@
       f32x4 v = *reinterpret_cast<const f32x4*>(x + i);
       f32x4 a = *reinterpret_cast<const f32x4*>(ab + c);
       f32x4 b = *reinterpret_cast<const f32x4*>(ab + H + c);
-      f32x4 o = {v.x * a.x + b.x, v.y * a.y + b.y, v.z * a.z + b.z, v.w * a.w + b.w};
+      f32x4 o = {bn_affine(v.x, a.x, b.x), bn_affine(v.y, a.y, b.y), bn_affine(v.z, a.z, b.z),
+                 bn_affine(v.w, a.w, b.w)};
       if (relu) {
         o.x = fmaxf(o.x, 0.f);
         o.y = fmaxf(o.y, 0.f);
@@ -268,7 +256,7 @@
       }
       *reinterpret_cast<f32x4*>(y + i) = o;
     } else {
-      float o = x[i] * ab[c] + ab[H + c];
+      float o = bn_affine(x[i], ab[c], ab[H + c]);
       y[i] = relu ? fmaxf(o, 0.f) : o;
     }
   }
@@ -287,22 +275,24 @@
     gnx_set_error("gnx_batchnorm_fwd: workspace %zu < %zu", ws_bytes, gnx_batchnorm_workspace_bytes(M, H));
     return GNX_E_WORKSPACE;
   }
-  float* ab = reinterpret_cast<float*>(ws);
+  int* counters = reinterpret_cast<int*>(ws);
+  float* ab = reinterpret_cast<float*>(counters + bn_counter_ints(H));
   float* part = ab + 4 * (size_t)H;
   int64_t chunks = gnx_cdiv(M, BN_ROWS_PER_BLOCK);
   gnx_prof_scope prof(h, GNX_K_BN_FWD, (training ? 12.0 : 8.0) * M * H);
   if (training) {
+    bn_fwd_fin fin = {gamma, beta, running_mean, running_var, momentum, eps, save_mean, save_rstd, ab,
+                      num_batches_tracked, counters};
     if (H % 4 == 0)
-      hipLaunchKernelGGL(k_bn_partial_v4, dim3((unsigned)chunks, (unsigned)gnx_cdiv(H, 128)), dim3(256), 0, h->stream, x,
-                         M, (int)H, part);
+      hipLaunchKernelGGL(k_bn_partial_v4, dim3((unsigned)chunks, (unsigned)gnx_cdiv(H, BN_COLS_V4)), dim3(256), 0,
+                         h->stream, x, M, (int)H, part, fin);
     else
-      hipLaunchKernelGGL(k_bn_partial, dim3((unsigned)chunks, (unsigned)gnx_cdiv(H, 64)), dim3(256), 0, h->stream, x, M,
-                         (int)H, part);
-    GNX_LAUNCH_CHECK();
-  }
-  hipLaunchKernelGGL(k_bn_finalize, dim3((unsigned)gnx_cdiv(H, 16)), dim3(256), 0, h->stream, x, part, chunks, M, (int)H,
-                     gamma, beta, running_mean, running_var, momentum, eps, (int)training, save_mean, save_rstd, ab,
-                     num_batches_tracked);
+      hipLaunchKernelGGL(k_bn_partial, dim3((unsigned)chunks, (unsigned)gnx_cdiv(H, BN_COLS_S)), dim3(256), 0, h->stream,
+                         x, M, (int)H, part, fin);
+  } else {
+    hipLaunchKernelGGL(k_bn_eval_ab, dim3((unsigned)gnx_cdiv(H, 256)), dim3(256), 0, h->stream, (int)H, gamma, beta,
+                       running_mean, running_var, eps, save_mean, save_rstd, ab);
+  }
   GNX_LAUNCH_CHECK();
   int64_t total = M * H;
   if (H % 4 == 0) {
@@ -318,24 +308,49 @@
   return GNX_OK;
 }
 
+struct bn_bwd_fin {
+  const float *gamma, *beta, *mean, *rstd;
+  float *dgamma, *dbeta, *coef;
+  int* counters;
+};
+
+template <int G, bool V4>
+__device__ __forceinline__ void bn_bwd_finalize(const bn_bwd_fin& f, const float* part, int64_t M, int H) {
+  if (!bn_last_ticket(f.counters + blockIdx.y, gridDim.x)) return;
+  int c;
+  float t1, t2;
+  bn_fold<G, V4>(part, gridDim.x, H, blockIdx.y * (16 * G), c, t1, t2);
+  if (c < 0) return;
+  if (f.dbeta) f.dbeta[c] += t1;
+  if (f.dgamma) f.dgamma[c] += t2;
+  const float inv = 1.0f / (float)M;
+  float a, b;
+  bn_ab(f.mean[c], f.rstd[c], f.gamma ? f.gamma[c] : 1.f, f.beta ? f.beta[c] : 0.f, a, b);
+  f.coef[c] = a;
+  f.coef[H + c] = t1 * inv;
+  f.coef[2 * H + c] = t2 * inv;
+  f.coef[3 * H + c] = b;
+}
+
 __global__ void __launch_bounds__(256) k_bn_bwd_partial(const float* __restrict__ dy, const float* __restrict__ x,
-                                                        const float* __restrict__ y, int64_t M, int H,
-                                                        const float* __restrict__ mean, const float* __restrict__ rstd,
-                                                        int relu, float* __restrict__ part) {
+                                                        int64_t M, int H, int relu, float* part, bn_bwd_fin fin) {
   __shared__ float s1[4][64], s2[4][64];
   const int cx = threadIdx.x & 63, ry = threadIdx.x >> 6;
-  const int col = blockIdx.y * 64 + cx;
+  const int col = blockIdx.y * BN_COLS_S + cx;
   int64_t r0 = (int64_t)blockIdx.x * BN_ROWS_PER_BLOCK;
   int64_t r1 = r0 + BN_ROWS_PER_BLOCK;
   if (r1 > M) r1 = M;
   float a1 = 0.f, a2 = 0.f;
   if (col < H) {
-    const float mu = mean[col], rs = rstd[col];
+    const float mu = fin.mean[col], rs = fin.rstd[col];
+    float a, b;
+    bn_ab(mu, rs, fin.gamma ? fin.gamma[col] : 1.f, fin.beta ? fin.beta[col] : 0.f, a, b);
     for (int64_t r = r0 + ry; r < r1; r += 4) {
       float g = dy[r * H + col];
-      if (relu && !(y[r * H + col] > 0.f)) g = 0.f;
+      const float xv = x[r * H + col];
+      if (relu && !(bn_affine(xv, a, b) > 0.f)) g = 0.f;
       a1 += g;
-      a2 += g * ((x[r * H + col] - mu) * rs);
+      a2 += g * ((xv - mu) * rs);
     }
   }
   s1[ry][cx] = a1;
@@ -345,72 +360,146 @@
     part[((int64_t)blockIdx.x * 2 + 0) * H + col] = (s1[0][cx] + s1[1][cx]) + (s1[2][cx] + s1[3][cx]);
     part[((int64_t)blockIdx.x * 2 + 1) * H + col] = (s2[0][cx] + s2[1][cx]) + (s2[2][cx] + s2[3][cx]);
   }
-}
-
-__global__ void k_bn_bwd_finalize(const float* __restrict__ part, int64_t chunks, int64_t M, int H,
-                                  const float* __restrict__ gamma, const float* __restrict__ rstd,
-                                  float* __restrict__ dgamma, float* __restrict__ dbeta, float* __restrict__ coef) {
-  const int c = blockIdx.x * 16 + (threadIdx.x & 15);
-  float t1 = 0.f, t2 = 0.f;
-  bn_fold(part, chunks, H, c, t1, t2);
-  if (c >= H || (threadIdx.x >> 4) != 0) return;
-  if (dbeta) dbeta[c] += t1;
-  if (dgamma) dgamma[c] += t2;
-  const float inv = 1.0f / (float)M;
-  coef[c] = (gamma ? gamma[c] : 1.f) * rstd[c];
-  coef[H + c] = t1 * inv;
-  coef[2 * H + c] = t2 * inv;
-}
-
+  bn_bwd_finalize<BN_COLS_S / 16, false>(fin, part, M, H);
+}
+
+__global__ void __launch_bounds__(256) k_bn_bwd_partial_v4(const float* __restrict__ dy, const float* __restrict__ x,
+                                                           int64_t M, int H, int relu, float* part, bn_bwd_fin fin) {
+  __shared__ f32x4 s1[8][32], s2[8][32];
+  const int cq = threadIdx.x & 31, ry = threadIdx.x >> 5;
+  const int col = blockIdx.y * BN_COLS_V4 + cq * 4;
+  int64_t r0 = (int64_t)blockIdx.x * BN_ROWS_PER_BLOCK;
+  int64_t r1 = r0 + BN_ROWS_PER_BLOCK;
+  if (r1 > M) r1 = M;
+  f32x4 a1 = {0.f, 0.f, 0.f, 0.f}, a2 = {0.f, 0.f, 0.f, 0.f};
+  if (col < H) {
+    const f32x4 mu = *reinterpret_cast<const f32x4*>(fin.mean + col);
+    const f32x4 rs = *reinterpret_cast<const f32x4*>(fin.rstd + col);
+    f32x4 ga = {1.f, 1.f, 1.f, 1.f}, be = {0.f, 0.f, 0.f, 0.f};
+    if (fin.gamma) ga = *reinterpret_cast<const f32x4*>(fin.gamma + col);
+    if (fin.beta) be = *reinterpret_cast<const f32x4*>(fin.beta + col);
+    float a[4], b[4];
+    bn_ab(mu.x, rs.x, ga.x, be.x, a[0], b[0]);
+    bn_ab(mu.y, rs.y, ga.y, be.y, a[1], b[1]);
+    bn_ab(mu.z, rs.z, ga.z, be.z, a[2], b[2]);
+    bn_ab(mu.w, rs.w, ga.w, be.w, a[3], b[3]);
+    auto row = [&](int64_t r, f32x4& g, f32x4& xv) {
+      g = *reinterpret_cast<const f32x4*>(dy + r * H + col);
+      xv = *reinterpret_cast<const f32x4*>(x + r * H + col);
+    };
+    auto fold = [&](f32x4 g, const f32x4& xv) {
+      if (relu) {
+        g.x = bn_affine(xv.x, a[0], b[0]) > 0.f ? g.x : 0.f;
+        g.y = bn_affine(xv.y, a[1], b[1]) > 0.f ? g.y : 0.f;
+        g.z = bn_affine(xv.z, a[2], b[2]) > 0.f ? g.z : 0.f;
+        g.w = bn_affine(xv.w, a[3], b[3]) > 0.f ? g.w : 0.f;
+      }
+      a1 += g;
+      a2 += g * ((xv - mu) * rs);
+    };
+    int64_t r = r0 + ry;
+    for (; r + 24 < r1; r += 32) {
+      f32x4 g0, x0, g1, x1, g2, x2, g3, x3;
+      row(r, g0, x0);
+      row(r + 8, g1, x1);
+      row(r + 16, g2, x2);
+      row(r + 24, g3, x3);
+      fold(g0, x0);
+      fold(g1, x1);
+      fold(g2, x2);
+      fold(g3, x3);
+    }
+    for (; r < r1; r += 8) {
+      f32x4 g, xv;
+      row(r, g, xv);
+      fold(g, xv);
+    }
+  }
+  s1[ry][cq] = a1;
+  s2[ry][cq] = a2;
+  __syncthreads();
+  if (ry == 0 && col < H) {
+    f32x4 t1 = s1[0][cq], t2 = s2[0][cq];
+#pragma unroll
+    for (int l = 1; l < 8; ++l) {
+      t1 += s1[l][cq];
+      t2 += s2[l][cq];
+    }
+    *reinterpret_cast<f32x4*>(part + ((int64_t)blockIdx.x * 2 + 0) * H + col) = t1;
+    *reinterpret_cast<f32x4*>(part + ((int64_t)blockIdx.x * 2 + 1) * H + col) = t2;
+  }
+  bn_bwd_finalize<BN_COLS_V4 / 16, true>(fin, part, M, H);
+}
+
+template <int VEC>
 __global__ void __launch_bounds__(256) k_bn_bwd_apply(const float* __restrict__ dy, const float* __restrict__ x,
-                                                      const float* __restrict__ y, int64_t total, int H,
-                                                      const float* __restrict__ mean, const float* __restrict__ rstd,
-                                                      const float* __restrict__ coef, int relu, float* __restrict__ dx) {
-  int64_t i = (int64_t)blockIdx.x * blockDim.x + threadIdx.x;
-  int64_t stride = (int64_t)gridDim.x * blockDim.x;
+                                                      int64_t total, int H, const float* __restrict__ mean,
+                                                      const float* __restrict__ rstd, const float* __restrict__ coef,
+                                                      int relu, float* __restrict__ dx) {
+  int64_t i = ((int64_t)blockIdx.x * blockDim.x + threadIdx.x) * VEC;
+  const int64_t stride = (int64_t)gridDim.x * blockDim.x * VEC;
   for (; i < total; i += stride) {
-    int c = (int)(i % H);
-    float g = dy[i];
-    if (relu && !(y[i] > 0.f)) g = 0.f;
-    float xh = (x[i] - mean[c]) * rstd[c];
-    dx[i] = coef[c] * (g - coef[H + c] - xh * coef[2 * H + c]);
+    const int c = (int)(i % H);
+    if constexpr (VEC == 4) {
+      f32x4 g = *reinterpret_cast<const f32x4*>(dy + i);
+      const f32x4 xv = *reinterpret_cast<const f32x4*>(x + i);
+      const f32x4 mu = *reinterpret_cast<const f32x4*>(mean + c), rs = *reinterpret_cast<const f32x4*>(rstd + c);
+      const f32x4 k0 = *reinterpret_cast<const f32x4*>(coef + c), k1 = *reinterpret_cast<const f32x4*>(coef + H + c),
+                  k2 = *reinterpret_cast<const f32x4*>(coef + 2 * H + c);
+      if (relu) {
+        const f32x4 b = *reinterpret_cast<const f32x4*>(coef + 3 * H + c);
+        g.x = bn_affine(xv.x, k0.x, b.x) > 0.f ? g.x : 0.f;
+        g.y = bn_affine(xv.y, k0.y, b.y) > 0.f ? g.y : 0.f;
+        g.z = bn_affine(xv.z, k0.z, b.z) > 0.f ? g.z : 0.f;
+        g.w = bn_affine(xv.w, k0.w, b.w) > 0.f ? g.w : 0.f;
+      }
+      const f32x4 xh = (xv - mu) * rs;
+      *reinterpret_cast<f32x4*>(dx + i) = k0 * (g - k1 - xh * k2);
+    } else {
+      float g = dy[i];
+      const float xv = x[i];
+      if (relu && !(bn_affine(xv, coef[c], coef[3 * H + c]) > 0.f)) g = 0.f;
+      float xh = (xv - mean[c]) * rstd[c];
+      dx[i] = coef[c] * (g - coef[H + c] - xh * coef[2 * H + c]);
+    }
   }
 }
 
 extern "C" int32_t gnx_batchnorm_bwd(gnx_handle* h, const float* dy, const float* x, const float* y, int64_t M,
-                                     int32_t H, const float* gamma, const float* save_mean, const float* save_rstd,
-                                     int32_t relu, float* dx, float* dgamma, float* dbeta, void* ws, size_t ws_bytes) {
+                                     int32_t H, const float* gamma, const float* beta, const float* save_mean,
+                                     const float* save_rstd, int32_t relu, float* dx, float* dgamma, float* dbeta,
+                                     void* ws, size_t ws_bytes) {
+  (void)y;
   GNX_CHECK_ARG(h && H > 0 && M >= 0, "gnx_batchnorm_bwd: bad argument");
   if (M == 0) return GNX_OK;
-  GNX_CHECK_ARG(dy && x && save_mean && save_rstd && dx && ws && (!relu || y), "gnx_batchnorm_bwd: NULL argument");
+  GNX_CHECK_ARG(dy && x && save_mean && save_rstd && dx && ws, "gnx_batchnorm_bwd: NULL argument");
   if (ws_bytes < gnx_batchnorm_workspace_bytes(M, H)) {
     gnx_set_error("gnx_batchnorm_bwd: workspace %zu < %zu", ws_bytes, gnx_batchnorm_workspace_bytes(M, H));
     return GNX_E_WORKSPACE;
   }
-  float* coef = reinterpret_cast<float*>(ws);
+  int* counters = reinterpret_cast<int*>(ws);
+  float* coef = reinterpret_cast<float*>(counters + bn_counter_ints(H));
   float* part = coef + 4 * (size_t)H;
   int64_t chunks = gnx_cdiv(M, BN_ROWS_PER_BLOCK);
-  gnx_prof_scope prof(h, GNX_K_BN_BWD, 28.0 * M * H);
+  gnx_prof_scope prof(h, GNX_K_BN_BWD, 20.0 * M * H);
+  bn_bwd_fin fin = {gamma, beta, save_mean, save_rstd, dgamma, dbeta, coef, counters};
   if (H % 4 == 0)
-    hipLaunchKernelGGL(k_bn_bwd_partial_v4, dim3((unsigned)chunks, (unsigned)gnx_cdiv(H, 128)), dim3(256), 0, h->stream,
-                       dy, x, y, M, (int)H, save_mean, save_rstd, (int)relu, part);
+    hipLaunchKernelGGL(k_bn_bwd_partial_v4, dim3((unsigned)chunks, (unsigned)gnx_cdiv(H, BN_COLS_V4)), dim3(256), 0,
+                       h->stream, dy, x, M, (int)H, (int)relu, part, fin);
   else
-    hipLaunchKernelGGL(k_bn_bwd_partial, dim3((unsigned)chunks, (unsigned)gnx_cdiv(H, 64)), dim3(256), 0, h->stream, dy,
-                       x, y, M, (int)H, save_mean, save_rstd, (int)relu, part);
-  GNX_LAUNCH_CHECK();
-  hipLaunchKernelGGL(k_bn_bwd_finalize, dim3((unsigned)gnx_cdiv(H, 16)), dim3(256), 0, h->stream, part, chunks, M, (int)H,
-                     gamma, save_rstd, dgamma, dbeta, coef);
+    hipLaunchKernelGGL(k_bn_bwd_partial, dim3((unsigned)chunks, (unsigned)gnx_cdiv(H, BN_COLS_S)), dim3(256), 0,
+                       h->stream, dy, x, M, (int)H, (int)relu, part, fin);
   GNX_LAUNCH_CHECK();
   int64_t total = M * H;
   if (H % 4 == 0) {
     int64_t blocks = gnx_cdiv(total / 4, 256);
     if (blocks > 4096) blocks = 4096;
-    hipLaunchKernelGGL(k_bn_bwd_apply_v<4>, dim3((unsigned)blocks), dim3(256), 0, h->stream, dy, x, y, total, (int)H,
+    hipLaunchKernelGGL(k_bn_bwd_apply<4>, dim3((unsigned)blocks), dim3(256), 0, h->stream, dy, x, total, (int)H,
                        save_mean, save_rstd, coef, (int)relu, dx);
   } else {
     int64_t blocks = gnx_cdiv(total, 256);
     if (blocks > 8192) blocks = 8192;
-    hipLaunchKernelGGL(k_bn_bwd_apply, dim3((unsigned)blocks), dim3(256), 0, h->stream, dy, x, y, total, (int)H,
+    hipLaunchKernelGGL(k_bn_bwd_apply<1>, dim3((unsigned)blocks), dim3(256), 0, h->stream, dy, x, total, (int)H,
                        save_mean, save_rstd, coef, (int)relu, dx);
   }
   GNX_LAUNCH_CHECK();
diff --git a/gnnepcsaft_amd/csrc/gnx_pack.hip b/gnnepcsaft_amd/csrc/gnx_pack.hip
--- a/gnnepcsaft_amd/csrc/gnx_pack.hip
+++ b/gnnepcsaft_amd/csrc/gnx_pack.hip
@@ -43,24 +43,94 @@
   if (threadIdx.x == 0 && blockIdx.x == 0) out[n] = (n > 0) ? out[n - 1] + in[n - 1] : 0;
 }
 
+__device__ __forceinline__ int scan_block_sum(int v) {
+  __shared__ int w[SCAN_BLOCK / 64];
+  for (int off = 32; off > 0; off >>= 1) v += __shfl_xor(v, off);
+  if ((threadIdx.x & 63) == 0) w[threadIdx.x >> 6] = v;
+  __syncthreads();
+  int t = 0;
+#pragma unroll
+  for (int i = 0; i < SCAN_BLOCK / 64; ++i) t += w[i];
+  return t;
+}
+
+__global__ void __launch_bounds__(SCAN_BLOCK) k_scan_sums(const int* __restrict__ in, int* __restrict__ sums, int64_t n) {
+  int64_t i = (int64_t)blockIdx.x * SCAN_TILE + threadIdx.x;
+  int t = 0;
+#pragma unroll
+  for (int k = 0; k < SCAN_ITEMS; ++k, i += SCAN_BLOCK) t += (i < n) ? in[i] : 0;
+  t = scan_block_sum(t);
+  if (threadIdx.x == 0) sums[blockIdx.x] = t;
+}
+
+__global__ void __launch_bounds__(SCAN_BLOCK) k_scan_offset_tile(const int* __restrict__ in, int* __restrict__ out,
+                                                                 const int* __restrict__ sums, int64_t n,
+                                                                 int write_total) {
+  __shared__ int s[SCAN_BLOCK];
+  int off = 0;
+  for (int i = threadIdx.x; i < (int)blockIdx.x; i += SCAN_BLOCK) off += sums[i];
+  off = scan_block_sum(off);
+  int64_t base = (int64_t)blockIdx.x * SCAN_TILE + (int64_t)threadIdx.x * SCAN_ITEMS;
+  int v[SCAN_ITEMS];
+  int t = 0;
+#pragma unroll
+  for (int i = 0; i < SCAN_ITEMS; ++i) {
+    v[i] = (base + i < n) ? in[base + i] : 0;
+    t += v[i];
+  }
+  s[threadIdx.x] = t;
+  __syncthreads();
+  for (int o = 1; o < SCAN_BLOCK; o <<= 1) {
+    int add = (threadIdx.x >= o) ? s[threadIdx.x - o] : 0;
+    __syncthreads();
+    s[threadIdx.x] += add;
+    __syncthreads();
+  }
+  int excl = off + s[threadIdx.x] - t;
+#pragma unroll
+  for (int i = 0; i < SCAN_ITEMS; ++i) {
+    if (base + i < n) out[base + i] = excl;
+    excl += v[i];
+  }
+  if (write_total && blockIdx.x == gridDim.x - 1 && threadIdx.x == SCAN_BLOCK - 1) out[n] = excl;
+}
+
 static int32_t exclusive_scan(gnx_handle* h, const int* in, int* out, int64_t n, int* ws, bool write_total) {
-  if (n > 0) {
-    int64_t blocks = gnx_cdiv(n, SCAN_TILE);
-    hipLaunchKernelGGL(k_scan_tile, dim3((unsigned)blocks), dim3(SCAN_BLOCK), 0, h->stream, in, out, ws, n);
-    GNX_LAUNCH_CHECK();
+  int64_t blocks = gnx_cdiv(n, SCAN_TILE);
+  if (blocks <= SCAN_TILE) {
+    if (n == 0 && !write_total) return GNX_OK;
     if (blocks > 1) {
-      int* sums_scanned = ws + blocks + 1;
-      int32_t st = exclusive_scan(h, ws, sums_scanned, blocks, sums_scanned + blocks + 1, false);
-      if (st != GNX_OK) return st;
-      hipLaunchKernelGGL(k_scan_add, dim3((unsigned)blocks), dim3(SCAN_BLOCK), 0, h->stream, out, sums_scanned, n);
+      hipLaunchKernelGGL(k_scan_sums, dim3((unsigned)blocks), dim3(SCAN_BLOCK), 0, h->stream, in, ws, n);
       GNX_LAUNCH_CHECK();
     }
-  }
+    hipLaunchKernelGGL(k_scan_offset_tile, dim3((unsigned)(blocks > 0 ? blocks : 1)), dim3(SCAN_BLOCK), 0, h->stream, in,
+                       out, ws, n, (int)write_total);
+    GNX_LAUNCH_CHECK();
+    return GNX_OK;
+  }
+  hipLaunchKernelGGL(k_scan_tile, dim3((unsigned)blocks), dim3(SCAN_BLOCK), 0, h->stream, in, out, ws, n);
+  GNX_LAUNCH_CHECK();
+  int* sums_scanned = ws + blocks + 1;
+  int32_t st = exclusive_scan(h, ws, sums_scanned, blocks, sums_scanned + blocks + 1, false);
+  if (st != GNX_OK) return st;
+  hipLaunchKernelGGL(k_scan_add, dim3((unsigned)blocks), dim3(SCAN_BLOCK), 0, h->stream, out, sums_scanned, n);
+  GNX_LAUNCH_CHECK();
   if (write_total) {
     hipLaunchKernelGGL(k_set_total, dim3(1), dim3(64), 0, h->stream, out, in, n);
     GNX_LAUNCH_CHECK();
   }
   return GNX_OK;
+}
+
+extern "C" size_t gnx_scan_workspace_bytes(int64_t n);
+extern "C" int32_t gnx_exclusive_scan(gnx_handle* h, const int32_t* in, int64_t n, int32_t* out, void* ws,
+                                      size_t ws_bytes) {
+  GNX_CHECK_ARG(h && out && n >= 0 && n < (1ll << 31) - 1 && (n == 0 || in), "gnx_exclusive_scan: bad argument");
+  if (ws_bytes < gnx_scan_workspace_bytes(n) || !ws) {
+    gnx_set_error("gnx_exclusive_scan: workspace %zu < %zu", ws_bytes, gnx_scan_workspace_bytes(n));
+    return GNX_E_WORKSPACE;
+  }
+  return exclusive_scan(h, in, out, n, reinterpret_cast<int*>(ws), true);
 }
 
 static size_t scan_ws_ints_total(int64_t n) {
@@ -74,8 +144,10 @@
   return tot + 16;
 }
 
-__global__ void k_convert_edges(const int64_t* __restrict__ ei, int64_t E, int64_t N, int* __restrict__ src0,
-                                int* __restrict__ dst0, int* __restrict__ flag) {
+extern "C" size_t gnx_scan_workspace_bytes(int64_t n) { return scan_ws_ints_total(n < 0 ? 0 : n) * sizeof(int); }
+
+__global__ void k_convert_count(const int64_t* __restrict__ ei, int64_t E, int64_t N, int* __restrict__ src0,
+                                int* __restrict__ dst0, int* __restrict__ counts, int* __restrict__ flag) {
   int64_t e = (int64_t)blockIdx.x * blockDim.x + threadIdx.x;
   if (e >= E) return;
   int64_t s = ei[e], d = ei[E + e];
@@ -87,11 +159,7 @@
   }
   src0[e] = (int)s;
   dst0[e] = (int)d;
-}
-
-__global__ void k_count_keys(const int* __restrict__ key, int64_t E, int* __restrict__ counts) {
-  int64_t e = (int64_t)blockIdx.x * blockDim.x + threadIdx.x;
-  if (e < E) atomicAdd(&counts[key[e]], 1);
+  atomicAdd(&counts[d], 1);
 }
 
 __global__ void k_fill_groups(const int* __restrict__ key, int64_t E, const int* __restrict__ ptr,
@@ -103,10 +171,7 @@
   items[pos] = (int)e;
 }
 
-__global__ void k_sort_groups(const int* __restrict__ ptr, int64_t N, int* __restrict__ items) {
-  int64_t i = (int64_t)blockIdx.x * blockDim.x + threadIdx.x;
-  if (i >= N) return;
-  int b = ptr[i], e = ptr[i + 1];
+__device__ __forceinline__ void sort_group(int* __restrict__ items, int b, int e) {
   for (int a = b + 1; a < e; ++a) {
     int v = items[a];
     int c = a - 1;
@@ -118,40 +183,31 @@
   }
 }
 
-__global__ void k_gather_endpoints(const int* __restrict__ perm, const int* __restrict__ src0,
-                                   const int* __restrict__ dst0, int64_t E, int* __restrict__ src,
-                                   int* __restrict__ dst) {
-  int64_t p = (int64_t)blockIdx.x * blockDim.x + threadIdx.x;
-  if (p >= E) return;
-  int e = perm[p];
-  src[p] = src0[e];
-  dst[p] = dst0[e];
-}
-
-static int32_t group_by_key(gnx_handle* h, const int* key, int64_t E, int64_t N, int* ptr, int* items, int* cursor,
-                            int* scan_ws) {
-  gnx_zero_ints(h, cursor, N > 0 ? N : 1);
-  if (E > 0) {
-    hipLaunchKernelGGL(k_count_keys, dim3((unsigned)gnx_cdiv(E, 256)), dim3(256), 0, h->stream, key, E, cursor);
-    GNX_LAUNCH_CHECK();
-  }
-  int32_t st = exclusive_scan(h, cursor, ptr, N, scan_ws, true);
-  if (st != GNX_OK) return st;
-  gnx_zero_ints(h, cursor, N > 0 ? N : 1);
-  if (E > 0) {
-    hipLaunchKernelGGL(k_fill_groups, dim3((unsigned)gnx_cdiv(E, 256)), dim3(256), 0, h->stream, key, E, ptr, cursor,
-                       items);
-    GNX_LAUNCH_CHECK();
-    hipLaunchKernelGGL(k_sort_groups, dim3((unsigned)gnx_cdiv(N, 256)), dim3(256), 0, h->stream, ptr, N, items);
-    GNX_LAUNCH_CHECK();
-  }
-  return GNX_OK;
+__global__ void k_sort_groups(const int* __restrict__ ptr, int64_t N, int* __restrict__ items) {
+  int64_t i = (int64_t)blockIdx.x * blockDim.x + threadIdx.x;
+  if (i >= N) return;
+  sort_group(items, ptr[i], ptr[i + 1]);
+}
+
+__global__ void k_sort_gather_count(const int* __restrict__ rowptr, int64_t N, int* __restrict__ perm,
+                                    const int* __restrict__ src0, int* __restrict__ src, int* __restrict__ dst,
+                                    int* __restrict__ counts) {
+  int64_t i = (int64_t)blockIdx.x * blockDim.x + threadIdx.x;
+  if (i >= N) return;
+  const int b = rowptr[i], e = rowptr[i + 1];
+  sort_group(perm, b, e);
+  for (int p = b; p < e; ++p) {
+    const int s = src0[perm[p]];
+    src[p] = s;
+    dst[p] = (int)i;
+    atomicAdd(&counts[s], 1);
+  }
 }
 
 extern "C" size_t gnx_pack_csr_workspace_bytes(int64_t N, int64_t E) {
   if (N < 0) N = 0;
   if (E < 0) E = 0;
-  size_t ints = 2 * (size_t)E + (size_t)N + 1 + scan_ws_ints_total(N) + 64;
+  size_t ints = 2 * (size_t)E + 4 * ((size_t)N + 1) + scan_ws_ints_total(N) + 64;
   return ints * sizeof(int);
 }
 
@@ -161,6 +217,7 @@
   GNX_CHECK_ARG(h != nullptr, "gnx_pack_csr: handle is NULL");
   GNX_CHECK_ARG(N >= 0 && E >= 0 && N < (1ll << 31) - 1 && E < (1ll << 31) - 1, "gnx_pack_csr: N=%lld E=%lld out of int32 range",
                 (long long)N, (long long)E);
+  GNX_CHECK_ARG(E == 0 || N > 0, "gnx_pack_csr: E > 0 needs N > 0");
   GNX_CHECK_ARG(rowptr && colptr, "gnx_pack_csr: rowptr/colptr NULL");
   GNX_CHECK_ARG(E == 0 || (edge_index && perm && src && dst && cpos), "gnx_pack_csr: NULL edge array with E>0");
   if (ws_bytes < gnx_pack_csr_workspace_bytes(N, E) || (!ws && ws_bytes)) {
@@ -171,21 +228,37 @@
   int* w = reinterpret_cast<int*>(ws);
   int* src0 = w;
   int* dst0 = src0 + E;
-  int* cursor = dst0 + E;
-  int* scan_ws = cursor + N + 1;
+  int* cnt_dst = dst0 + E;
+  int* cur_dst = cnt_dst + N + 1;
+  int* cnt_src = cur_dst + N + 1;
+  int* cur_src = cnt_src + N + 1;
+  int* scan_ws = cur_src + N + 1;
+  const unsigned eb = (unsigned)gnx_cdiv(E, 256), nb = (unsigned)gnx_cdiv(N, 256);
+  int32_t st;
   if (E > 0) {
-    hipLaunchKernelGGL(k_convert_edges, dim3((unsigned)gnx_cdiv(E, 256)), dim3(256), 0, h->stream, edge_index, E, N,
-                       src0, dst0, h->d_flag);
-    GNX_LAUNCH_CHECK();
-  }
-  int32_t st = group_by_key(h, dst0, E, N, rowptr, perm, cursor, scan_ws);
-  if (st != GNX_OK) return st;
+    gnx_zero_ints(h, cnt_dst, 4 * (N + 1));
+    hipLaunchKernelGGL(k_convert_count, dim3(eb), dim3(256), 0, h->stream, edge_index, E, N, src0, dst0, cnt_dst,
+                       h->d_flag);
+    GNX_LAUNCH_CHECK();
+  } else {
+    gnx_zero_ints(h, cnt_dst, N > 0 ? N : 1);
+    cnt_src = cnt_dst;
+  }
+  if ((st = exclusive_scan(h, cnt_dst, rowptr, N, scan_ws, true)) != GNX_OK) return st;
   if (E > 0) {
-    hipLaunchKernelGGL(k_gather_endpoints, dim3((unsigned)gnx_cdiv(E, 256)), dim3(256), 0, h->stream, perm, src0,
-                       dst0, E, src, dst);
-    GNX_LAUNCH_CHECK();
-  }
-  return group_by_key(h, src, E, N, colptr, cpos, cursor, scan_ws);
+    hipLaunchKernelGGL(k_fill_groups, dim3(eb), dim3(256), 0, h->stream, dst0, E, rowptr, cur_dst, perm);
+    GNX_LAUNCH_CHECK();
+    hipLaunchKernelGGL(k_sort_gather_count, dim3(nb), dim3(256), 0, h->stream, rowptr, N, perm, src0, src, dst, cnt_src);
+    GNX_LAUNCH_CHECK();
+  }
+  if ((st = exclusive_scan(h, cnt_src, colptr, N, scan_ws, true)) != GNX_OK) return st;
+  if (E > 0) {
+    hipLaunchKernelGGL(k_fill_groups, dim3(eb), dim3(256), 0, h->stream, src, E, colptr, cur_src, cpos);
+    GNX_LAUNCH_CHECK();
+    hipLaunchKernelGGL(k_sort_groups, dim3(nb), dim3(256), 0, h->stream, colptr, N, cpos);
+    GNX_LAUNCH_CHECK();
+  }
+  return GNX_OK;
 }
 
 struct dims_t {
diff --git a/gnnepcsaft_amd/functional.py b/gnnepcsaft_amd/functional.py
--- a/gnnepcsaft_amd/functional.py
+++ b/gnnepcsaft_amd/functional.py
@@ -170,18 +170,19 @@
         x = x.contiguous()
         y, mean, rstd = ops.batchnorm_fwd(x, gamma, beta, running_mean, running_var, momentum, eps, training, relu,
                                           num_batches_tracked=nbt)
-        ctx.save_for_backward(x, y, gamma, mean, rstd)
+        ctx.save_for_backward(x, y, gamma, beta, mean, rstd)
         ctx.relu, ctx.training = relu, training
         ctx.sinks = grad_sinks([gamma, beta])
         return y
 
     @staticmethod
     def backward(ctx, dy):
-        x, y, gamma, mean, rstd = ctx.saved_tensors
+        x, y, gamma, beta, mean, rstd = ctx.saved_tensors
         if not ctx.training:
             raise NotImplementedError("BatchNorm backward in eval mode is not on the reference's training path")
         sg, sb = ctx.sinks
-        dx, dgamma, dbeta = ops.batchnorm_bwd(dy.contiguous(), x, y, gamma, mean, rstd, ctx.relu, dgamma=sg, dbeta=sb)
+        dx, dgamma, dbeta = ops.batchnorm_bwd(dy.contiguous(), x, y, gamma, mean, rstd, ctx.relu, dgamma=sg, dbeta=sb,
+                                              beta=beta)
         return dx, (None if sg is not None else dgamma), (None if sb is not None else dbeta), None, None, None, None, \
             None, None, None
 
diff --git a/gnnepcsaft_amd/ops.py b/gnnepcsaft_amd/ops.py
--- a/gnnepcsaft_amd/ops.py
+++ b/gnnepcsaft_amd/ops.py
@@ -2,7 +2,7 @@
 
 import ctypes as C
 import threading
-from typing import List, Optional, Sequence, Tuple
+from typing import Dict, List, Optional, Sequence, Tuple
 
 import torch
 
@@ -844,9 +844,18 @@
     return dx
 
 
+_BN_WS: Dict[Tuple[int, int], torch.Tensor] = {}
+
+
 def _bn_ws(M: int, H: int, dev) -> Tuple[torch.Tensor, int]:
     nbytes = _lib.load().gnx_batchnorm_workspace_bytes(M, H)
-    return torch.empty(nbytes, dtype=torch.uint8, device=dev), nbytes
+    dev = torch.device(dev)
+    idx = dev.index if dev.index is not None else torch.cuda.current_device()
+    key = (idx, _lib._raw_stream(idx))
+    ws = _BN_WS.get(key)
+    if ws is None or ws.numel() < nbytes:
+        ws = _BN_WS[key] = torch.zeros(max(nbytes, 1 << 20), dtype=torch.uint8, device=dev)
+    return ws, nbytes
 
 
 def batchnorm_fwd(x, gamma, beta, running_mean, running_var, momentum: float, eps: float, training: bool, relu: bool,
@@ -864,7 +873,7 @@
     return y, mean, rstd
 
 
-def batchnorm_bwd(dy, x, y, gamma, mean, rstd, relu: bool, dgamma=None, dbeta=None):
+def batchnorm_bwd(dy, x, y, gamma, mean, rstd, relu: bool, dgamma=None, dbeta=None, beta=None):
     M, H = x.shape
     dx = torch.empty_like(x)
     if dgamma is None:
@@ -872,8 +881,8 @@
     if dbeta is None:
         dbeta = zeros(H, device=x.device)
     ws, nbytes = _bn_ws(M, H, x.device)
-    check(_lib.load().gnx_batchnorm_bwd(handle(x.device), dy.data_ptr(), x.data_ptr(), y.data_ptr(), M, H, _ptr(gamma),
-                                        mean.data_ptr(), rstd.data_ptr(), int(relu), dx.data_ptr(), dgamma.data_ptr(),
+    check(_lib.load().gnx_batchnorm_bwd(handle(x.device), dy.data_ptr(), x.data_ptr(), _ptr(y), M, H, _ptr(gamma),
+                                        _ptr(beta), mean.data_ptr(), rstd.data_ptr(), int(relu), dx.data_ptr(), dgamma.data_ptr(),
                                         dbeta.data_ptr(), ws.data_ptr(), nbytes))
     return dx, dgamma, dbeta
 
diff --git a/include/gnx.h b/include/gnx.h
--- a/include/gnx.h
+++ b/include/gnx.h
@@ -75,6 +75,8 @@
 size_t gnx_pack_csr_workspace_bytes(int64_t N, int64_t E);
 int32_t gnx_pack_csr(gnx_handle* h, const int64_t* edge_index, int64_t E, int64_t N, int32_t* rowptr, int32_t* perm,
                      int32_t* src, int32_t* dst, int32_t* colptr, int32_t* cpos, void* ws, size_t ws_bytes);
+size_t gnx_scan_workspace_bytes(int64_t n);
+int32_t gnx_exclusive_scan(gnx_handle* h, const int32_t* in, int64_t n, int32_t* out, void* ws, size_t ws_bytes);
 int32_t gnx_feature_code(gnx_handle* h, const int64_t* feat, int64_t rows, int32_t K, const int32_t* dims,
                          const int32_t* perm, int32_t* code, void* ws, size_t ws_bytes);
 int32_t gnx_graph_ptr(gnx_handle* h, const int64_t* batch, int64_t N, int64_t B, int32_t* graph_ptr, void* ws,
@@ -238,8 +240,8 @@
                           float eps, int32_t training, int32_t relu, float* y, float* save_mean, float* save_rstd,
                           void* ws, size_t ws_bytes);
 int32_t gnx_batchnorm_bwd(gnx_handle* h, const float* dy, const float* x, const float* y, int64_t M, int32_t H,
-                          const float* gamma, const float* save_mean, const float* save_rstd, int32_t relu,
-                          float* dx, float* dgamma, float* dbeta, void* ws, size_t ws_bytes);
+                          const float* gamma, const float* beta, const float* save_mean, const float* save_rstd,
+                          int32_t relu, float* dx, float* dgamma, float* dbeta, void* ws, size_t ws_bytes);
 
 int32_t gnx_dropout(gnx_handle* h, const float* x, int64_t n, float p, uint64_t seed, uint64_t offset, float* y);
 
```
